# ed-fish/data-efficient-video-transformers

Measured on AMD Instinct MI355X. Metric: clips/sec fwd+bwd, B=8 T=32 3x224x224 bf16, higher is better.
Workload: dtype bf16; 1 GPU; ViViT metric shape (SURVEY 8 'M'; BASELINE configs[2]/[3] transformer): B=8/GPU, T=32, 3x224x224, patch 16, d=512, ...; global_batch=8, parallelism=dp1

## Files before the change

### data-efficient-video-transformers_amd/csrc/layernorm.hip

```cpp
#include "common.h"
#include "ln_reduce.h"

namespace {

constexpr int kLnBlock = 256;
constexpr int kLnBwdBlock = 256;
constexpr int kLnBwdMaxBlocks = 1024;

template <typename TX, typename TY, int VPL>
__global__ __launch_bounds__(kLnBlock) void ln_fwd_kernel(
    const TX* __restrict__ x, const float* __restrict__ gamma, const float* __restrict__ beta,
    TY* __restrict__ y, float* __restrict__ mean, float* __restrict__ rstd, int64_t rows, int64_t n1,
    int d, int64_t xs0, int64_t xs1, int64_t ys0, int64_t ys1, float eps) {
  const int lane = threadIdx.x & 63;
  const int64_t wave = (int64_t)blockIdx.x * (kLnBlock / 64) + (threadIdx.x >> 6);
  const int64_t nwaves = (int64_t)gridDim.x * (kLnBlock / 64);
  const float inv_d = 1.0f / (float)d;

  float g[VPL][8], b[VPL][8];
#pragma unroll
  for (int i = 0; i < VPL; ++i) {
    const int c = (lane + 64 * i) * 8;
    if (c < d) {
      load8<float>(gamma + c, g[i]);
      load8<float>(beta + c, b[i]);
    }
  }

  for (int64_t r = wave; r < rows; r += nwaves) {
    const int64_t i0 = r / n1, i1 = r - i0 * n1;
    const TX* xr = x + i0 * xs0 + i1 * xs1;
    TY* yr = y + i0 * ys0 + i1 * ys1;
    float v[VPL][8];
    float s = 0.f;
#pragma unroll
    for (int i = 0; i < VPL; ++i) {
      const int c = (lane + 64 * i) * 8;
      if (c < d) {
        load8<TX>(xr + c, v[i]);
#pragma unroll
        for (int k = 0; k < 8; ++k) s += v[i][k];
      }
    }
    const float mu = wave_sum_dpp(s) * inv_d;
    float q = 0.f;
#pragma unroll
    for (int i = 0; i < VPL; ++i) {
      const int c = (lane + 64 * i) * 8;
      if (c < d) {
#pragma unroll
        for (int k = 0; k < 8; ++k) {
          v[i][k] -= mu;
          q = fmaf(v[i][k], v[i][k], q);
        }
      }
    }
    const float rs = rsqrtf(wave_sum_dpp(q) * inv_d + eps);
#pragma unroll
    for (int i = 0; i < VPL; ++i) {
      const int c = (lane + 64 * i) * 8;
      if (c < d) {
        float o[8];
#pragma unroll
        for (int k = 0; k < 8; ++k) o[k] = fmaf(v[i][k] * rs, g[i][k], b[i][k]);
        store8<TY>(yr + c, o);
      }
    }
    if (lane == 0) {
      mean[r] = mu;
      rstd[r] = rs;
    }
  }
}

template <typename TDY, typename TX, typename TDX, typename TL, int VPL>
__global__ __launch_bounds__(kLnBwdBlock) void ln_bwd_kernel(
    const TDY* __restrict__ dy, const TX* __restrict__ x, const float* __restrict__ gamma,
    const float* __restrict__ mean, const float* __restrict__ rstd, const TDX* dx_add,
    TDX* dx, TL* __restrict__ dx_lp, float* __restrict__ partial , int64_t rows, int64_t n1, int d,
    int64_t xs0, int64_t xs1, int64_t ys0, int64_t ys1,
    const TDY* __restrict__ dy_first, int64_t dyf_s, const TDX* __restrict__ dx_first, int64_t dxf_s) {
  extern __shared__ __attribute__((aligned(16))) float lds[];
  const int lane = threadIdx.x & 63;
  const int wid = threadIdx.x >> 6;
  const int64_t wave = (int64_t)blockIdx.x * (kLnBwdBlock / 64) + wid;
  const int64_t nwaves = (int64_t)gridDim.x * (kLnBwdBlock / 64);
  const float inv_d = 1.0f / (float)d;

  float g[VPL][8], dg[VPL][8], db[VPL][8];
#pragma unroll
  for (int i = 0; i < VPL; ++i) {
    const int c = (lane + 64 * i) * 8;
    if (c < d) load8<float>(gamma + c, g[i]);
#pragma unroll
    for (int k = 0; k < 8; ++k) { dg[i][k] = 0.f; db[i][k] = 0.f; }
  }

  for (int64_t r = wave; r < rows; r += nwaves) {
    const int64_t i0 = r / n1, i1 = r - i0 * n1;
    const TX* xr = x + i0 * xs0 + i1 * xs1;
    const TDY* dyr = dy + i0 * ys0 + i1 * ys1;
    const int64_t xoff = i0 * xs0 + i1 * xs1;
    TDX* dxr = dx + xoff;
    const float mu = mean[r], rs = rstd[r];
    float xh[VPL][8], gg[VPL][8];
    float s1 = 0.f, s2 = 0.f;
#pragma unroll
    for (int i = 0; i < VPL; ++i) {
      const int c = (lane + 64 * i) * 8;
      if (c < d) {
        float xv[8], dv[8];
        load8<TX>(xr + c, xv);
        load8<TDY>(dyr + c, dv);
        if (dy_first && i1 == 0) {
          float fv[8];
          load8<TDY>(dy_first + i0 * dyf_s + c, fv);
#pragma unroll
          for (int k = 0; k < 8; ++k) dv[k] += fv[k];
        }
#pragma unroll
        for (int k = 0; k < 8; ++k) {
          xh[i][k] = (xv[k] - mu) * rs;
          gg[i][k] = dv[k] * g[i][k];
          s1 += gg[i][k];
          s2 = fmaf(gg[i][k], xh[i][k], s2);
          dg[i][k] = fmaf(dv[k], xh[i][k], dg[i][k]);
          db[i][k] += dv[k];
        }
      }
    }
    const float c1 = wave_sum_dpp(s1) * inv_d;
    const float c2 = wave_sum_dpp(s2) * inv_d;
#pragma unroll
    for (int i = 0; i < VPL; ++i) {
      const int c = (lane + 64 * i) * 8;
      if (c < d) {
        float o[8];
#pragma unroll
        for (int k = 0; k < 8; ++k) o[k] = rs * (gg[i][k] - c1 - xh[i][k] * c2);
        if (dx_add) {
          float a[8];
          load8<TDX>(dx_add + xoff + c, a);
#pragma unroll
          for (int k = 0; k < 8; ++k) o[k] += a[k];
        }
        if (dx_first && i1 == 0) {
          float a[8];
          load8<TDX>(dx_first + i0 * dxf_s + c, a);
#pragma unroll
          for (int k = 0; k < 8; ++k) o[k] += a[k];
        }
        store8<TDX>(dxr + c, o);
        if (dx_lp) store8<TL>(dx_lp + xoff + c, o);
      }
    }
  }

  for (int w = 0; w < kLnBwdBlock / 64; ++w) {
    if (wid == w) {
#pragma unroll
      for (int i = 0; i < VPL; ++i) {
        const int c = (lane + 64 * i) * 8;
        if (c < d) {
#pragma unroll
          for (int k = 0; k < 8; ++k) {
            if (w == 0) { lds[c + k] = dg[i][k]; lds[d + c + k] = db[i][k]; }
            else { lds[c + k] += dg[i][k]; lds[d + c + k] += db[i][k]; }
          }
        }
      }
    }
    __syncthreads();
  }
  float* out = partial + (int64_t)blockIdx.x * 2 * d;
  for (int c = threadIdx.x; c < 2 * d; c += kLnBwdBlock) out[c] = lds[c];
}

int ln_check(const char* name, const void* a, const void* b, int64_t n0, int64_t n1, int64_t d,
             int64_t xs0, int64_t xs1, int64_t ys0, int64_t ys1) {
  DVT_REQUIRE(a && b, "%s: null pointer", name);
  DVT_REQUIRE(n0 >= 0 && n1 >= 1 && d >= 8, "%s: bad sizes", name);
  DVT_REQUIRE(d % 8 == 0, "%s: d = %lld must be a multiple of 8", name, (long long)d);
  if (d > 8 * 64 * 8) DVT_UNSUPPORTED("%s: d = %lld > 4096 not supported", name, (long long)d);
  DVT_REQUIRE(xs0 % 8 == 0 && xs1 % 8 == 0 && ys0 % 8 == 0 && ys1 % 8 == 0,
              "%s: row strides must be multiples of 8 elements", name);
  DVT_REQUIRE(dvt_aligned16(a) && dvt_aligned16(b), "%s: buffers must be 16-byte aligned", name);
  return DVT_OK;
}

}

#define DVT_LN_VPL_SWITCH(vpl, ...)                    \
  switch (vpl) {                                       \
    case 1: { constexpr int VPL = 1; __VA_ARGS__; break; } \
    case 2: { constexpr int VPL = 2; __VA_ARGS__; break; } \
    case 3: { constexpr int VPL = 3; __VA_ARGS__; break; } \
    case 4: { constexpr int VPL = 4; __VA_ARGS__; break; } \
    default: { constexpr int VPL = 8; __VA_ARGS__; break; } \
  }

#define DVT_LN_FWD_LAUNCH(TX, TY)                                                                                          \
  DVT_LN_VPL_SWITCH(vpl, hipLaunchKernelGGL((ln_fwd_kernel<TX, TY, VPL>), dim3((unsigned)blocks), dim3(kLnBlock), 0, st,    \
                                            (const TX*)x, gamma, beta, (TY*)y, mean, rstd, rows, n1, (int)d, xs0, xs1, ys0, \
                                            ys1, eps))

#define DVT_LN_BWD_LAUNCH(TDY, TX, TDX, TL)                                                                                \
  DVT_LN_VPL_SWITCH(vpl, hipLaunchKernelGGL((ln_bwd_kernel<TDY, TX, TDX, TL, VPL>), dim3((unsigned)blocks),                 \
                                            dim3(kLnBwdBlock), lds, st, (const TDY*)q->dy, (const TX*)q->x, q->gamma,       \
                                            q->mean, q->rstd, (const TDX*)q->dx_add, (TDX*)q->dx, (TL*)q->dx_lp, partial,   \
                                            rows, q->n1, (int)q->d, q->xs0, q->xs1, q->ys0, q->ys1, (const TDY*)q->dy_first, \
                                            q->dy_first_stride, (const TDX*)q->dx_first, q->dx_first_stride))

namespace {

constexpr int kLnGroup = 32;
struct LnGroup { dvt_ln_pending e[kLnGroup]; };

__global__ __launch_bounds__(1024) void ln_bwd_reduce_group_kernel(const LnGroup grp) {
  const dvt_ln_pending& q = grp.e[blockIdx.y];
  constexpr int PL = 32;
  __shared__ float red[PL][33];
  const int cl = threadIdx.x & 31, pl = threadIdx.x >> 5;
  const int c = blockIdx.x * 32 + cl;
  const int d = q.d;
  if (blockIdx.x * 32 >= 2 * d) return;
  const int64_t ld = 2 * (int64_t)d;
  float a0 = 0.f, a1 = 0.f, a2 = 0.f, a3 = 0.f;
  if (c < 2 * d) {
    int p = pl;
    for (; p + 3 * PL < q.nparts; p += 4 * PL) {
      a0 += q.partial[(int64_t)p * ld + c];
      a1 += q.partial[(int64_t)(p + PL) * ld + c];
      a2 += q.partial[(int64_t)(p + 2 * PL) * ld + c];
      a3 += q.partial[(int64_t)(p + 3 * PL) * ld + c];
    }
    for (; p < q.nparts; p += PL) a0 += q.partial[(int64_t)p * ld + c];
  }
  red[pl][cl] = (a0 + a1) + (a2 + a3);
  __syncthreads();
  if (pl < 4) {
    float t = 0.f;
#pragma unroll
    for (int i = 0; i < PL / 4; ++i) t += red[pl * (PL / 4) + i][cl];
    red[pl * (PL / 4)][cl] = t;
  }
  __syncthreads();
  if (pl == 0 && c < 2 * d) {
    const float t = (red[0][cl] + red[PL / 4][cl]) + (red[2 * (PL / 4)][cl] + red[3 * (PL / 4)][cl]);
    float* o = c < d ? q.dgamma + c : q.dbeta + (c - d);
    const bool acc = c < d ? (q.accumulate & 1) : (q.accumulate & 2);
    *o = acc ? *o + t : t;
  }
}

}

extern "C" {

int dvt_layernorm_fwd_mixed(const void* x, int x_dtype, const float* gamma, const float* beta, void* y, int y_dtype, float* mean,
                            float* rstd, int64_t n0, int64_t n1, int64_t d, int64_t xs0, int64_t xs1,
                            int64_t ys0, int64_t ys1, float eps, dvt_stream_t stream) {
  int rc = ln_check("dvt_layernorm_fwd", x, y, n0, n1, d, xs0, xs1, ys0, ys1);
  if (rc) return rc;
  DVT_REQUIRE(gamma && beta && mean && rstd, "dvt_layernorm_fwd: null parameter/statistics pointer");
  DVT_REQUIRE(dvt_aligned16(gamma) && dvt_aligned16(beta), "dvt_layernorm_fwd: gamma/beta misaligned");
  const int64_t rows = n0 * n1;
  if (rows == 0) return DVT_OK;
  hipStream_t st = (hipStream_t)stream;
  int64_t blocks = dvt_cdiv(rows, kLnBlock / 64);
  const int64_t cap = (int64_t)dvt_num_cus() * 8;
  if (blocks > cap) blocks = cap;
  const int vpl = (int)dvt_cdiv(d, 8 * 64);
  if (x_dtype == y_dtype) {
    DVT_DISPATCH_DTYPE(x_dtype, T, DVT_LN_FWD_LAUNCH(T, T));
  } else if (x_dtype == DVT_F32 && dvt_is_16bit(y_dtype)) {
    DVT_DISPATCH_16BIT(y_dtype, E, DVT_LN_FWD_LAUNCH(float, E));
  } else if (y_dtype == DVT_F32 && dvt_is_16bit(x_dtype)) {
    DVT_DISPATCH_16BIT(x_dtype, E, DVT_LN_FWD_LAUNCH(E, float));
  } else {
    DVT_UNSUPPORTED("dvt_layernorm_fwd: x dtype %d -> y dtype %d (equal types, or fp32 on one side)", x_dtype, y_dtype);
  }
  DVT_LAUNCH_CHECK("dvt_layernorm_fwd");
  return DVT_OK;
}

int dvt_layernorm_fwd(const void* x, const float* gamma, const float* beta, void* y, float* mean,
                      float* rstd, int64_t n0, int64_t n1, int64_t d, int64_t xs0, int64_t xs1,
                      int64_t ys0, int64_t ys1, float eps, int dtype, dvt_stream_t stream) {
  return dvt_layernorm_fwd_mixed(x, dtype, gamma, beta, y, dtype, mean, rstd, n0, n1, d, xs0, xs1, ys0, ys1, eps, stream);
}

size_t dvt_layernorm_bwd_workspace_bytes(int64_t d) {
  return (size_t)kLnBwdMaxBlocks * 2 * (size_t)(d > 0 ? d : 0) * sizeof(float);
}

size_t dvt_layernorm_bwd_partial_bytes(int64_t rows, int64_t d) {
  int64_t blocks = dvt_cdiv(rows > 0 ? rows : 1, kLnBwdBlock / 64);
  if (blocks > kLnBwdMaxBlocks) blocks = kLnBwdMaxBlocks;
  return (size_t)blocks * 2 * (size_t)(d > 0 ? d : 0) * sizeof(float);
}

int dvt_layernorm_bwd_ex(const dvt_ln_bwd_desc* q, dvt_stream_t stream) {
  DVT_REQUIRE(q, "dvt_layernorm_bwd: null descriptor");
  int rc = ln_check("dvt_layernorm_bwd", q->x, q->dy, q->n0, q->n1, q->d, q->xs0, q->xs1, q->ys0, q->ys1);
  if (rc) return rc;
  DVT_REQUIRE(q->gamma && q->mean && q->rstd && q->dx && q->dgamma && q->dbeta && q->workspace, "dvt_layernorm_bwd: null pointer");
  DVT_REQUIRE(dvt_aligned16(q->dx) && dvt_aligned16(q->gamma) && dvt_aligned16(q->workspace) && dvt_aligned16(q->dx_add) &&
                  dvt_aligned16(q->dy_first) && dvt_aligned16(q->dx_first) && dvt_aligned16(q->dx_lp),
              "dvt_layernorm_bwd: buffers must be 16-byte aligned");
  DVT_REQUIRE(q->dy_first_stride % 8 == 0 && q->dx_first_stride % 8 == 0,
              "dvt_layernorm_bwd: first-row strides must be multiples of 8 elements");
  DVT_REQUIRE(!q->defer_reduce || q->pending, "dvt_layernorm_bwd: defer_reduce needs a pending descriptor to fill");
  const int64_t rows = q->n0 * q->n1;
  DVT_REQUIRE(rows > 0, "dvt_layernorm_bwd: no rows");
  hipStream_t st = (hipStream_t)stream;
  int64_t blocks = dvt_cdiv(rows, kLnBwdBlock / 64);
  if (blocks > kLnBwdMaxBlocks) blocks = kLnBwdMaxBlocks;
  const int64_t d = q->d;
  const int vpl = (int)dvt_cdiv(d, 8 * 64);
  const size_t lds = 2 * (size_t)d * sizeof(float);
  float* partial = (float*)q->workspace;
  const int dyt = q->dy_dtype, xt = q->x_dtype, dxt = q->dx_dtype;
  if (dyt == xt && xt == dxt && !q->dx_lp) {
    DVT_DISPATCH_DTYPE(xt, T, DVT_LN_BWD_LAUNCH(T, T, T, T));
  } else if (dvt_is_16bit(dyt) && xt == DVT_F32 && dxt == DVT_F32 && (!q->dx_lp || q->dx_lp_dtype == dyt)) {
    DVT_DISPATCH_16BIT(dyt, E, DVT_LN_BWD_LAUNCH(E, float, float, E));
  } else if (dyt == DVT_F32 && dvt_is_16bit(xt) && dxt == xt && !q->dx_lp) {
    DVT_DISPATCH_16BIT(xt, E, DVT_LN_BWD_LAUNCH(float, E, E, E));
  } else {
    DVT_UNSUPPORTED("dvt_layernorm_bwd: dtype combination (dy %d, x %d, dx %d, dx_lp %d) not instantiated", dyt, xt, dxt,
                    q->dx_lp ? q->dx_lp_dtype : -1);
  }
  DVT_LAUNCH_CHECK("dvt_layernorm_bwd");
  if (q->defer_reduce) {
    dvt_ln_pending* pn = q->pending;
    pn->partial = partial; pn->nparts = (int)blocks; pn->d = (int)d; pn->dgamma = q->dgamma; pn->dbeta = q->dbeta;
    pn->accumulate = (q->accumulate_gamma ? 1 : 0) | (q->accumulate_beta ? 2 : 0); pn->valid = 1;
    return DVT_OK;
  }
  dvt_ln_partials_reduce(partial, (int)blocks, (int)d, q->dgamma, q->dbeta, q->accumulate_gamma, q->accumulate_beta, st);
  DVT_LAUNCH_CHECK("dvt_layernorm_bwd(reduce)");
  return DVT_OK;
}

int dvt_layernorm_reduce_group(const dvt_ln_pending* list, int count, dvt_stream_t stream) {
  DVT_REQUIRE(count >= 0 && (count == 0 || list), "dvt_layernorm_reduce_group: bad arguments");
  hipStream_t st = (hipStream_t)stream;
  for (int i = 0; i < count;) {
    LnGroup grp{};
    int n = 0, dmax = 0;
    for (; i < count && n < kLnGroup; ++i) {
      if (!list[i].valid) continue;
      DVT_REQUIRE(list[i].partial && list[i].dgamma && list[i].dbeta && list[i].nparts > 0 && list[i].d > 0,
                  "dvt_layernorm_reduce_group: bad entry");
      grp.e[n++] = list[i];
      if (list[i].d > dmax) dmax = list[i].d;
    }
    if (n == 0) continue;
    hipLaunchKernelGGL(ln_bwd_reduce_group_kernel, dim3((unsigned)dvt_cdiv(2 * dmax, 32), (unsigned)n), dim3(1024), 0, st, grp);
    DVT_LAUNCH_CHECK("dvt_layernorm_reduce_group");
  }
  return DVT_OK;
}

int dvt_layernorm_bwd_first(const void* dy, const void* x, const float* gamma, const float* mean,
                            const float* rstd, const void* dx_add, void* dx, float* dgamma, float* dbeta,
                            void* workspace,
                            int64_t n0, int64_t n1, int64_t d, int64_t xs0, int64_t xs1, int64_t ys0,
                            int64_t ys1, const void* dy_first, int64_t dy_first_stride,
                            const void* dx_first, int64_t dx_first_stride, int dtype,
                            int accumulate_gamma, int accumulate_beta, dvt_stream_t stream) {
  dvt_ln_bwd_desc q{};
  q.dy = dy; q.dy_dtype = dtype; q.x = x; q.x_dtype = dtype; q.gamma = gamma; q.mean = mean; q.rstd = rstd;
  q.dx_add = dx_add; q.dx = dx; q.dx_dtype = dtype; q.dgamma = dgamma; q.dbeta = dbeta; q.workspace = workspace;
  q.n0 = n0; q.n1 = n1; q.d = d; q.xs0 = xs0; q.xs1 = xs1; q.ys0 = ys0; q.ys1 = ys1;
  q.dy_first = dy_first; q.dy_first_stride = dy_first_stride; q.dx_first = dx_first; q.dx_first_stride = dx_first_stride;
  q.accumulate_gamma = accumulate_gamma; q.accumulate_beta = accumulate_beta;
  return dvt_layernorm_bwd_ex(&q, stream);
}

int dvt_layernorm_bwd(const void* dy, const void* x, const float* gamma, const float* mean,
                      const float* rstd, const void* dx_add, void* dx, float* dgamma, float* dbeta,
                      void* workspace,
                      int64_t n0, int64_t n1, int64_t d, int64_t xs0, int64_t xs1, int64_t ys0,
                      int64_t ys1, int dtype, int accumulate, dvt_stream_t stream) {
  return dvt_layernorm_bwd_first(dy, x, gamma, mean, rstd, dx_add, dx, dgamma, dbeta, workspace, n0, n1, d, xs0,
                                 xs1, ys0, ys1, nullptr, 0, nullptr, 0, dtype, accumulate, accumulate, stream);
}

}
```

### data-efficient-video-transformers_amd/functional.py

```python
from __future__ import annotations

import contextlib
from collections import namedtuple
from typing import Optional

import torch

from . import _lib as L
from . import ops

Tensor = torch.Tensor


def _wc(w: Optional[Tensor], dtype: torch.dtype) -> Optional[Tensor]:
    if w is None:
        return None
    c = getattr(w, "_dvt_compute", None)
    if c is not None and c.dtype == dtype and w._dvt_sink.owner.compute_valid:
        return c
    w = w.detach()
    if w.dtype == dtype:
        return w.contiguous()
    return ops.cast(w, dtype)


def _sink(p):
    return None if p is None else getattr(p, "_dvt_sink", None)


def _emit_wgrad(sink, dy2: Tensor, x2: Tensor):
    if sink is None:
        return ops.linear_wgrad(dy2, x2)
    ops.linear_wgrad(dy2, x2, out=sink.buf.view(dy2.shape[1], x2.shape[1]), accumulate=not sink.fresh)
    sink.mark_written()
    return None


def _emit_wgrad_bias(sink_w, sink_b, dy2: Tensor, x2: Tensor, has_bias: bool, defer: bool = False):
    N, K = dy2.shape[1], x2.shape[1]
    w_out = sink_w.buf.view(N, K) if sink_w is not None else None
    b_out, b_acc = None, False
    if has_bias:
        if sink_b is not None:
            b_out, b_acc = sink_b.buf.view(-1), not sink_b.fresh
        else:
            b_out = torch.empty((N,), dtype=torch.float32, device=dy2.device)
    r = ops.linear_wgrad(dy2, x2, out=w_out, accumulate=(not sink_w.fresh) if sink_w is not None else False,
                         bias_out=b_out, bias_accumulate=b_acc, defer_reduce=defer)
    dw, pending = r if defer else (r, None)

    def finish():
        if sink_w is not None:
            sink_w.mark_written()
        if has_bias and sink_b is not None:
            sink_b.mark_written()

    dw_ret = None if sink_w is not None else dw
    db_ret = None if (not has_bias or sink_b is not None) else b_out
    if defer:
        return dw_ret, db_ret, pending, finish
    finish()
    return dw_ret, db_ret


def _linear_bwd(sink_w, sink_b, dy2: Tensor, x2: Tensor, w: Tensor, has_bias: bool, *, epilogue: int = L.EPI_NONE,
                aux: Optional[Tensor] = None):
    N, K = dy2.shape[1], x2.shape[1]
    w_out = sink_w.buf.view(N, K) if sink_w is not None else None
    b_out, b_acc = None, False
    if has_bias:
        if sink_b is not None:
            b_out, b_acc = sink_b.buf.view(-1), not sink_b.fresh
        else:
            b_out = torch.empty((N,), dtype=torch.float32, device=dy2.device)
    dw, dx = ops.linear_backward(dy2, x2, w, out=w_out, accumulate=(not sink_w.fresh) if sink_w is not None else False,
                                 bias_out=b_out, bias_accumulate=b_acc, epilogue=epilogue, aux=aux)
    if sink_w is not None:
        sink_w.mark_written()
    if has_bias and sink_b is not None:
        sink_b.mark_written()
    return (None if sink_w is not None else dw), (None if (not has_bias or sink_b is not None) else b_out), dx


def _emit_colsum(sink, dy2: Tensor):
    if sink is None:
        return ops.colsum(dy2)
    ops.colsum(dy2, out=sink.buf.view(-1), accumulate=not sink.fresh)
    sink.mark_written()
    return None


LN_DEFER = True
_ln_pending_sinks = set()


def ln_flush(end_of_step: bool = False):
    ops.layernorm_flush()
    _ln_pending_sinks.clear()
    if end_of_step:
        _lp_hand.clear()


def _ln_bwd(dy, x, g, mean, rstd, sg, sb, **kw):
    if sg is None or sb is None:
        return ops.layernorm_bwd(dy, x, g, mean, rstd, **kw)
    defer = None
    if LN_DEFER:
        if id(sg) in _ln_pending_sinks or id(sb) in _ln_pending_sinks:
            ln_flush()
        if sg.fresh and sb.fresh:
            _ln_pending_sinks.update((id(sg), id(sb)))

            def defer():
                sg.mark_written()
                sb.mark_written()
    r = ops.layernorm_bwd(dy, x, g, mean, rstd, dg=sg.buf.view(-1), db=sb.buf.view(-1),
                          accumulate=not sg.fresh, accumulate_beta=not sb.fresh, defer=defer, **kw)
    if defer is None:
        sg.mark_written()
        sb.mark_written()
    return (r[0], None, None) + tuple(r[3:])


def _emit_into(sink, t: Tensor):
    ops.axpby_f32_(sink.buf.view(-1), t.reshape(-1).contiguous(), 1.0, 0.0 if sink.fresh else 1.0)
    sink.mark_written()


_lp_hand = {}


def lp_clear() -> None:
    _lp_hand.clear()


def _lp_put(t32: Tensor, lp: Tensor) -> None:
    _lp_hand[t32.data_ptr()] = (t32, t32._version, lp)


def _lp_take(t32: Tensor, T: torch.dtype) -> Tensor:
    e = _lp_hand.pop(t32.data_ptr(), None)
    if (e is not None and e[0].shape == t32.shape and e[0].stride() == t32.stride() and e[0].dtype == t32.dtype
            and t32._version == e[1] and e[2].dtype == T):
        return e[2]
    return ops.cast(t32, T)


def _f32(t: Optional[Tensor]) -> Optional[Tensor]:
    if t is None:
        return None
    t = t.detach()
    return t.contiguous() if t.dtype == torch.float32 else ops.cast(t, torch.float32)


def _same_layout(a: Tensor, b: Tensor) -> bool:
    return a.shape == b.shape and all(sa == sb for sa, sb, n in zip(a.stride(), b.stride(), a.shape) if n > 1)


def _as(t: Tensor, dtype: torch.dtype) -> Tensor:
    return t if t.dtype == dtype else ops.cast(t, dtype)


class _Linear(torch.autograd.Function):
    @staticmethod
    def forward(ctx, x, w, b, out_f32):
        shp = x.shape
        x2 = x.reshape(-1, shp[-1])
        if not x2.is_contiguous():
            x2 = x2.contiguous()
        wc = _wc(w, x.dtype)
        M, K = x2.shape
        N = wc.shape[0]
        out_dtype = torch.float32 if out_f32 else x.dtype
        y = ops.gemm(x2, wc, M, N, K, a_kmajor=True, b_kmajor=True, lda=x2.stride(0), ldb=K,
                     out_dtype=out_dtype, bias=_f32(b))
        ctx.save_for_backward(x2, wc)
        ctx.has_bias = b is not None
        ctx.xshape = shp
        ctx.sinks = (_sink(w), _sink(b))
        return y.view(*shp[:-1], N)

    @staticmethod
    def backward(ctx, dy):
        x2, wc = ctx.saved_tensors
        dy2 = _as(dy.reshape(-1, dy.shape[-1]).contiguous(), x2.dtype)
        dx = dw = db = None
        if ctx.needs_input_grad[0]:
            dx = ops.linear_dgrad(dy2, wc).view(ctx.xshape)
        if ctx.needs_input_grad[1]:
            dw, db = _emit_wgrad_bias(ctx.sinks[0], ctx.sinks[1], dy2, x2, ctx.has_bias and ctx.needs_input_grad[2])
        elif ctx.has_bias and ctx.needs_input_grad[2]:
            db = _emit_colsum(ctx.sinks[1], dy2)
        return dx, dw, db, None


def linear(x: Tensor, w: Tensor, b: Optional[Tensor] = None, out_f32: bool = False) -> Tensor:
    return _Linear.apply(x, w, b, out_f32)


class _Act(torch.autograd.Function):
    @staticmethod
    def forward(ctx, x, act):
        ctx.save_for_backward(x)
        ctx.act = act
        return ops.act_fwd(x, act)

    @staticmethod
    def backward(ctx, dy):
        (x,) = ctx.saved_tensors
        return ops.act_bwd(_as(dy, x.dtype), x, ctx.act), None


def gelu(x: Tensor) -> Tensor:
    return _Act.apply(x, ops.ACT_GELU)


def relu(x: Tensor) -> Tensor:
    return _Act.apply(x, ops.ACT_RELU)


class _Add(torch.autograd.Function):
    @staticmethod
    def forward(ctx, a, b):
        return ops.add(a, b)

    @staticmethod
    def backward(ctx, dy):
        return dy, dy


def add(a: Tensor, b: Tensor) -> Tensor:
    return _Add.apply(a, b)


class _Fork(torch.autograd.Function):

    @staticmethod
    def forward(ctx, x):
        return x.view(x.shape), x.view(x.shape)

    @staticmethod
    def backward(ctx, da, db):
        if da is None or db is None:
            return da if db is None else db
        if da.dtype != db.dtype:
            db = _as(db.contiguous(), da.dtype)
        return ops.add(da.contiguous(), db.contiguous())


def fork(x: Tensor):
    if not (torch.is_grad_enabled() and x.requires_grad):
        return x, x
    return _Fork.apply(x)


class _Cast(torch.autograd.Function):

    @staticmethod
    def forward(ctx, x, dtype):
        ctx.src = x.dtype
        return _as(x, dtype)

    @staticmethod
    def backward(ctx, dy):
        return _as(dy.contiguous(), ctx.src), None


def cast(x: Tensor, dtype: torch.dtype) -> Tensor:
    return x if x.dtype == dtype else _Cast.apply(x, dtype)


class _LayerNorm(torch.autograd.Function):
    @staticmethod
    def forward(ctx, x, w, b, eps):
        xc = x.contiguous()
        g, bb = _f32(w), _f32(b)
        y, mean, rstd = ops.layernorm_fwd(xc, g, bb, eps)
        ctx.save_for_backward(xc, g, mean, rstd)
        ctx.sinks = (_sink(w), _sink(b))
        return y

    @staticmethod
    def backward(ctx, dy):
        xc, g, mean, rstd = ctx.saved_tensors
        dx, dg, db = _ln_bwd(_as(dy.contiguous(), xc.dtype), xc, g, mean, rstd, *ctx.sinks)
        return dx, dg, db, None


def layernorm(x: Tensor, w: Tensor, b: Tensor, eps: float = 1e-5) -> Tensor:
    return _LayerNorm.apply(x, w, b, eps)


class _PatchEmbed(torch.autograd.Function):

    @staticmethod
    def forward(ctx, clip, w, b, patch, dtype, tubelet):
        if tubelet == 1:
            patches = ops.patchify(clip, patch, dtype)
        else:
            patches = ops.tubelet_patchify(clip, patch, tubelet, dtype)
        wc = _wc(w, dtype)
        emb = ops.linear_fwd(patches, wc, _f32(b))
        ctx.save_for_backward(patches, wc)
        ctx.clip_shape, ctx.clip_dtype, ctx.patch, ctx.tubelet = tuple(clip.shape), clip.dtype, patch, tubelet
        ctx.sinks = (_sink(w), _sink(b))
        return emb

    @staticmethod
    def backward(ctx, demb):
        patches, wc = ctx.saved_tensors
        demb = demb.contiguous()
        dclip = None
        if ctx.needs_input_grad[0]:
            dpatch = ops.linear_dgrad(demb, wc)
            if ctx.tubelet == 1:
                dclip = ops.patchify_bwd(dpatch, ctx.clip_shape, ctx.patch, ctx.clip_dtype)
            else:
                dclip = ops.tubelet_patchify_bwd(dpatch, ctx.clip_shape, ctx.patch, ctx.tubelet, ctx.clip_dtype)
        dw, db = _emit_wgrad_bias(ctx.sinks[0], ctx.sinks[1], demb, patches, True)
        return dclip, dw, db, None, None, None


def patch_embed(clip: Tensor, w: Tensor, b: Tensor, patch: int, dtype: torch.dtype, tubelet: int = 1) -> Tensor:
    return _PatchEmbed.apply(clip, w, b, patch, dtype, tubelet)


class _Tokens(torch.autograd.Function):
    @staticmethod
    def forward(ctx, emb, cls, pos, S, T, n):
        cls32 = _f32(cls).reshape(-1)
        pos32 = _f32(pos)
        pos32 = pos32.reshape(T, pos32.shape[-2], pos32.shape[-1])
        ctx.T, ctx.pos_rows = T, pos32.shape[1]
        ctx.cls_shape, ctx.pos_shape = tuple(cls.shape), tuple(pos.shape)
        ctx.sinks = (_sink(cls), _sink(pos))
        return ops.tokens_assemble_fwd(emb.contiguous(), cls32, pos32, S, T, n)

    @staticmethod
    def backward(ctx, dout):
        sc, sp = ctx.sinks
        if sc is not None and sp is not None and sc.fresh != sp.fresh:
            demb, dcls, dpos = ops.tokens_assemble_bwd(dout, ctx.T, ctx.pos_rows)
            _emit_into(sc, dcls)
            _emit_into(sp, dpos)
            return demb, None, None, None, None, None
        if sc is not None and sp is not None:
            demb, _, _ = ops.tokens_assemble_bwd(dout, ctx.T, ctx.pos_rows, dcls=sc.buf.view(-1),
                                                 dpos=sp.buf.view(ctx.T, ctx.pos_rows, -1),
                                                 accumulate=not sc.fresh)
            sc.mark_written()
            sp.mark_written()
            return demb, None, None, None, None, None
        demb, dcls, dpos = ops.tokens_assemble_bwd(dout, ctx.T, ctx.pos_rows)
        return demb, dcls.view(ctx.cls_shape), dpos.view(ctx.pos_shape), None, None, None


def tokens_assemble(emb: Tensor, cls: Tensor, pos: Tensor, S: int, T: int, n: int) -> Tensor:
    return _Tokens.apply(emb, cls, pos, S, T, n)


class _ClsNormConcat(torch.autograd.Function):

    @staticmethod
    def forward(ctx, x, w, b, tok, B, T, eps, out_dtype=None):
        S, N, d = x.shape
        xc = x.contiguous()
        g, bb = _f32(w), _f32(b)
        rows = (S, 1, N * d, 0)
        cls_rows, mean, rstd = ops.layernorm_fwd(xc, g, bb, eps, rows=rows, out_dtype=out_dtype)
        tok32 = _f32(tok).reshape(-1) if tok is not None else None
        seq = ops.rows_gather_fwd(cls_rows, d, tok32, B, T, d)
        ctx.save_for_backward(xc, g, mean, rstd)
        ctx.dims = (B, T, S, N, d)
        ctx.seq_dtype = seq.dtype
        ctx.tok_shape = tuple(tok.shape) if tok is not None else None
        ctx.sinks = (_sink(w), _sink(b), _sink(tok))
        return seq

    @staticmethod
    def backward(ctx, dseq):
        xc, g, mean, rstd = ctx.saved_tensors
        B, T, S, N, d = ctx.dims
        gdt = ctx.seq_dtype
        dseq = _as(dseq.contiguous(), gdt)
        drows = torch.empty((S, d), dtype=gdt, device=xc.device)
        sg, sb, st = ctx.sinks
        if st is not None:
            ops.rows_gather_bwd(dseq, drows, d, True, B, T, d, dtok=st.buf.view(-1), accumulate=not st.fresh)
            st.mark_written()
            dtok = None
        else:
            dtok = ops.rows_gather_bwd(dseq, drows, d, ctx.tok_shape is not None, B, T, d)
        dx = ops.zeros(xc.shape, xc.dtype, xc.device) if N > 1 else torch.empty_like(xc)
        _, dg, db = _ln_bwd(drows, xc, g, mean, rstd, sg, sb, rows=(S, 1, N * d, 0), dy_rows=(d, 0), dx=dx)
        if dtok is not None:
            dtok = dtok.view(ctx.tok_shape)
        return dx, dg, db, dtok, None, None, None, None


def cls_norm_concat(x: Tensor, w: Tensor, b: Tensor, tok: Optional[Tensor], B: int, T: int,
                    eps: float = 1e-5, out_dtype: Optional[torch.dtype] = None) -> Tensor:
    return _ClsNormConcat.apply(x, w, b, tok, B, T, eps, out_dtype)


class _RowsSelect(torch.autograd.Function):

    @staticmethod
    def forward(ctx, x):
        B, Ln, d = x.shape
        xc = x.contiguous()
        ctx.shape = (B, Ln, d)
        return ops.rows_gather_fwd(xc, Ln * d, None, B, 1, d).view(B, d)

    @staticmethod
    def backward(ctx, dy):
        B, Ln, d = ctx.shape
        dx = ops.zeros((B, Ln, d), dy.dtype, dy.device)
        ops.rows_gather_bwd(dy.contiguous().view(B, 1, d), dx, Ln * d, False, B, 1, d)
        return dx


def select_first_row(x: Tensor) -> Tensor:
    return _RowsSelect.apply(x)


class _AttentionCore(torch.autograd.Function):

    @staticmethod
    def forward(ctx, q, k, v, scale):
        B, H, Lq, dh = q.shape
        o_mem = torch.empty((B, Lq, H, dh), dtype=q.dtype, device=q.device)
        o = o_mem.permute(0, 2, 1, 3)
        lse = ops.attention_fwd(q, k, v, o, scale)
        ctx.save_for_backward(q, k, v, o, lse)
        ctx.scale = scale
        return o

    @staticmethod
    def backward(ctx, do):
        q, k, v, o, lse = ctx.saved_tensors
        B, H, Lq, dh = q.shape
        Lk = k.shape[2]
        if _same_layout(do, o) and do.dtype == q.dtype:
            do_v = do.as_strided(o.shape, o.stride())
        else:
            do_c = _as(do.permute(0, 2, 1, 3).contiguous(), q.dtype)
            do_v = do_c.permute(0, 2, 1, 3).as_strided(o.shape, o.stride())
        dq = torch.empty_strided(q.shape, q.stride(), dtype=q.dtype, device=q.device)
        dk = torch.empty_strided(k.shape, k.stride(), dtype=k.dtype, device=k.device)
        dv = torch.empty_strided(v.shape, v.stride(), dtype=v.dtype, device=v.device)
        ops.attention_bwd(q, k, v, o, lse, do_v, dq, dk, dv, ctx.scale)
        return dq, dk, dv, None


def attention_core(q: Tensor, k: Tensor, v: Tensor, scale: float) -> Tensor:
    return _AttentionCore.apply(q, k, v, scale)


AttnTap = namedtuple("AttnTap", "kind q k lse heads dh seq_first packed P")
_attn_tap = None


@contextlib.contextmanager
def attention_tap():
    global _attn_tap
    outer, layers = _attn_tap, []
    _attn_tap = layers
    try:
        yield layers
    finally:
        _attn_tap = outer


def _split_qkv(qkv: Tensor, S: int, N: int, heads: int, dh: int, seq_first: bool):
    if seq_first:
        q5 = qkv.view(N, S, 3, heads, dh)
        return tuple(q5[:, :, i].permute(1, 2, 0, 3) for i in range(3))
    q5 = qkv.view(S, N, 3, heads, dh)
    return tuple(q5[:, :, i].permute(0, 2, 1, 3) for i in range(3))


def _heads_view(o_mem: Tensor, seq_first: bool) -> Tensor:
    return o_mem.permute(1, 2, 0, 3) if seq_first else o_mem.permute(0, 2, 1, 3)


class _AttnBlock(torch.autograd.Function):

    @staticmethod
    def forward(ctx, x, ln_w, ln_b, w_qkv, w_out, b_out, heads, prenorm, residual, eps, b_qkv=None,
                seq_first=False, attn_dropout=0.0, cdt=None):
        shp = x.shape
        d = shp[-1]
        if seq_first:
            N, S = shp[0], shp[1]
        else:
            S, N = (shp[0], shp[1]) if x.dim() == 3 else (1, shp[0])
        x2 = x.reshape(-1, d)
        if not x2.is_contiguous():
            x2 = x2.contiguous()
        M = x2.shape[0]
        T = x.dtype if cdt is None else cdt
        ctx.mixed = mixed = T != x.dtype
        if mixed and not (x.dtype == torch.float32 and prenorm and residual and w_out is not None and attn_dropout == 0.0):
            raise ValueError("the fp32 stream form is the pre-norm residual block with an output projection")
        if prenorm:
            g, bb = _f32(ln_w), _f32(ln_b)
            xn, mean, rstd = ops.layernorm_fwd(x2, g, bb, eps, out_dtype=T)
        else:
            g = mean = rstd = None
            xn = x2
        wq = _wc(w_qkv, T)
        inner = wq.shape[0] // 3
        dh = inner // heads
        qkv = ops.linear_fwd(xn, wq, _f32(b_qkv))
        q, k, v = _split_qkv(qkv, S, N, heads, dh, seq_first)
        o_mem = torch.empty((N, S, heads, dh) if seq_first else (S, N, heads, dh), dtype=T, device=x.device)
        drop = None
        if attn_dropout > 0.0:
            drop = (attn_dropout, _rng.tensor(x.device), _rng.take(S * heads * N * N))
        lse = ops.attention_fwd(q, k, v, _heads_view(o_mem, seq_first), dh ** -0.5, drop)
        if _attn_tap is not None:
            _attn_tap.append(AttnTap("dense", q, k, lse, heads, dh, seq_first, qkv, None))
        ctx.drop = drop
        o2 = o_mem.view(M, inner)
        if w_out is not None:
            wo = _wc(w_out, T)
            if residual:
                y = ops.linear_fwd(o2, wo, _f32(b_out), epilogue=L.EPI_RESIDUAL, residual=x2,
                                   out_dtype=torch.float32 if mixed else None)
            else:
                y = ops.linear_fwd(o2, wo, _f32(b_out))
        else:
            wo = None
            y = ops.add(o2, x2) if residual else o2
        ctx.save_for_backward(x2, g, mean, rstd, xn if prenorm else None, wq, wo, qkv, o_mem, lse)
        ctx.cfg = (S, N, heads, dh, inner, prenorm, residual, w_out is not None, b_out is not None,
                   b_qkv is not None, seq_first)
        ctx.xshape = shp
        ctx.sinks = tuple(_sink(t) for t in (ln_w, ln_b, w_qkv, w_out, b_out, b_qkv))
        return y.view(*shp[:-1], y.shape[-1])

    @staticmethod
    def backward(ctx, dy):
        x2, g, mean, rstd, xn, wq, wo, qkv, o_mem, lse = ctx.saved_tensors
        S, N, heads, dh, inner, prenorm, residual, has_out, has_bias, has_qkv_bias, seq_first = ctx.cfg
        M = x2.shape[0]
        T = qkv.dtype
        if xn is None:
            xn = x2
        if ctx.mixed:
            dy32 = dy.reshape(M, -1).contiguous()
            dy2 = _lp_take(dy32, T)
        else:
            dy2 = _as(dy.reshape(M, -1).contiguous(), T)
        dwo = dbo = None
        if has_out:
            dwo, dbo, do2 = _linear_bwd(ctx.sinks[3], ctx.sinks[4], dy2, o_mem.view(M, inner), wo, has_bias)
        else:
            do2 = dy2
        q, k, v = _split_qkv(qkv, S, N, heads, dh, seq_first)
        dqkv = torch.empty_like(qkv)
        dq, dk, dv = _split_qkv(dqkv, S, N, heads, dh, seq_first)
        ops.attention_bwd(q, k, v, _heads_view(o_mem, seq_first), lse,
                          _heads_view(do2.view(o_mem.shape), seq_first), dq, dk, dv, dh ** -0.5, ctx.drop)
        dwq, dbq, dxn = _linear_bwd(ctx.sinks[2], ctx.sinks[5], dqkv, xn, wq, has_qkv_bias)
        dg = db = None
        if ctx.mixed:
            dx, dg, db, dx_lp = _ln_bwd(dxn, x2, g, mean, rstd, ctx.sinks[0], ctx.sinks[1], dx_add=dy32,
                                        dx_dtype=torch.float32, dx_lp=T)
            _lp_put(dx, dx_lp)
        elif prenorm:
            dx, dg, db = _ln_bwd(dxn, x2, g, mean, rstd, ctx.sinks[0], ctx.sinks[1],
                                 dx_add=dy2 if residual else None)
        else:
            dx = ops.add(dxn, dy2) if residual else dxn
        if M >= 4096:
            ln_flush()
        return dx.view(ctx.xshape), dg, db, dwq, dwo, dbo, None, None, None, None, dbq, None, None, None


def attn_block(x, ln_w, ln_b, w_qkv, w_out, b_out, heads, *, prenorm=True, residual=True, eps=1e-5,
               b_qkv=None, seq_first=False, attn_dropout=0.0, cdt=None):
    return _AttnBlock.apply(x, ln_w, ln_b, w_qkv, w_out, b_out, heads, prenorm, residual, eps, b_qkv, seq_first,
                            float(attn_dropout), cdt)


class _AttnBlockCls(torch.autograd.Function):

    @staticmethod
    def forward(ctx, x, ln_w, ln_b, w_qkv, w_out, b_out, heads, eps, cdt=None):
        S, N, d = x.shape
        T = x.dtype if cdt is None else cdt
        ctx.mixed = mixed = T != x.dtype
        x2 = x.reshape(S * N, d)
        if not x2.is_contiguous():
            x2 = x2.contiguous()
        g, bb = _f32(ln_w), _f32(ln_b)
        wqkv = _wc(w_qkv, T)
        inner = wqkv.shape[0] // 3
        dh = inner // heads
        wo = _wc(w_out, T)
        ctx.cfg = (S, N, d, heads, dh, inner, b_out is not None, eps)
        ctx.sinks = tuple(_sink(t) for t in (ln_w, ln_b, w_qkv, w_out, b_out))
        x3 = x2.view(S, N, d)
        ctx.folded = (not mixed) and cls_fold_taken(x3, heads, dh)
        if ctx.folded:
            xn0, mean0, rstd0 = ops.layernorm_fwd(x2, g, bb, eps, rows=(S, 1, N * d, 0))
            q = ops.linear_fwd(xn0, wqkv[:inner])
            R = ops.heads_expand(q, wqkv[inner:2 * inner], heads, dh ** -0.5)
            A, lse, P, mean, rstd = ops.attn_cls_fwd(x3, g, bb, eps, R)
            if _attn_tap is not None:
                _attn_tap.append(AttnTap("folded", None, None, None, heads, dh, False, None, P))
            o = ops.heads_contract(A, wqkv[2 * inner:], 1.0, g, bb)
            y = ops.linear_fwd(o, wo, _f32(b_out), epilogue=L.EPI_RESIDUAL, residual=x3[:, 0])
            ctx.save_for_backward(x2, g, bb, mean0, rstd0, xn0, wqkv, wo, q, o, R, A, lse, P, mean, rstd)
            return y
        xn, mean, rstd = ops.layernorm_fwd(x2, g, bb, eps, out_dtype=T)
        w_q, w_kv = wqkv[:inner], wqkv[inner:]
        kv = ops.linear_fwd(xn, w_kv)
        xn0 = xn.view(S, N, d)[:, 0]
        q = ops.linear_fwd(xn0, w_q)
        kv5 = kv.view(S, N, 2, heads, dh)
        k4, v4 = kv5[:, :, 0].permute(0, 2, 1, 3), kv5[:, :, 1].permute(0, 2, 1, 3)
        o = torch.empty((S, inner), dtype=T, device=x.device)
        lse = ops.attention_fwd(q.view(S, 1, heads, dh).permute(0, 2, 1, 3), k4, v4,
                                o.view(S, 1, heads, dh).permute(0, 2, 1, 3), dh ** -0.5)
        if _attn_tap is not None:
            _attn_tap.append(AttnTap("cls", q.view(S, 1, heads, dh).permute(0, 2, 1, 3), k4, lse, heads, dh, False, kv, None))
        y = ops.linear_fwd(o, wo, _f32(b_out), epilogue=L.EPI_RESIDUAL, residual=x3[:, 0],
                           out_dtype=torch.float32 if mixed else None)
        ctx.save_for_backward(x2, g, mean, rstd, xn, wqkv, wo, q, kv, o, lse)
        return y

    @staticmethod
    def _backward_folded(ctx, dy):
        x2, g, bb, mean0, rstd0, xn0, wqkv, wo, q, o, R, A, lse, P, mean, rstd = ctx.saved_tensors
        S, N, d, heads, dh, inner, has_bias, eps = ctx.cfg
        T = x2.dtype
        s_g, s_b, s_qkv, s_o, s_bo = ctx.sinks
        scale = dh ** -0.5
        dy2 = _as(dy.reshape(S, d).contiguous(), T)
        dwo, dbo, do = _linear_bwd(s_o, s_bo, dy2, o, wo, has_bias)
        if s_qkv is not None:
            buf, acc = s_qkv.buf.view(3 * inner, d), not s_qkv.fresh
            dwqkv = None
        else:
            buf, acc = torch.empty((3 * inner, d), dtype=torch.float32, device=x2.device), False
            dwqkv = buf
        w_q, w_k, w_v = wqkv[:inner], wqkv[inner:2 * inner], wqkv[2 * inner:]
        dM = ops.heads_expand_outer(do, w_v, heads, A, buf[2 * inner:], gamma=g, beta=bb, accumulate=acc)
        if s_g is not None and s_b is not None:
            dx2, G, _, _ = ops.attn_cls_bwd(x2.view(S, N, d), g, bb, eps, R, A, lse, P, mean, rstd, dM, dg=s_g.buf.view(-1),
                                            db=s_b.buf.view(-1), accumulate=not s_g.fresh, accumulate_beta=not s_b.fresh)
            dg, db = s_g.buf.view(-1), s_b.buf.view(-1)
        else:
            dx2, G, dg, db = ops.attn_cls_bwd(x2.view(S, N, d), g, bb, eps, R, A, lse, P, mean, rstd, dM)
        dq = ops.heads_contract_outer(G, g, w_k, q, buf[inner:2 * inner], alpha_out=scale, alpha_dw=scale, accumulate=acc)
        _, dxn0 = ops.linear_backward(dq, xn0, w_q, out=buf[:inner], accumulate=acc)
        if s_qkv is not None:
            s_qkv.mark_written()
        dxf = dx2.view(S * N, d)
        ops.layernorm_bwd(dxn0, x2, g, mean0, rstd0, rows=(S, 1, N * d, 0), dx=dxf, dx_add=dxf, dx_first=dy2,
                          dg=dg, db=db, accumulate=True)
        if s_g is not None and s_b is not None:
            s_g.mark_written()
            s_b.mark_written()
            dg = db = None
        return dx2.view(S, N, d), dg, db, dwqkv, dwo, dbo, None, None, None

    @staticmethod
    def backward(ctx, dy):
        if ctx.folded:
            return _AttnBlockCls._backward_folded(ctx, dy)
        x2, g, mean, rstd, xn, wqkv, wo, q, kv, o, lse = ctx.saved_tensors
        S, N, d, heads, dh, inner, has_bias, _ = ctx.cfg
        T = kv.dtype
        s_g, s_b, s_qkv, s_o, s_bo = ctx.sinks
        dy_s = dy.reshape(S, d).contiguous()
        dy2 = _lp_take(dy_s, T) if ctx.mixed else _as(dy_s, T)
        dwo, dbo, do = _linear_bwd(s_o, s_bo, dy2, o, wo, has_bias)
        kv5 = kv.view(S, N, 2, heads, dh)
        k4, v4 = kv5[:, :, 0].permute(0, 2, 1, 3), kv5[:, :, 1].permute(0, 2, 1, 3)
        dq = torch.empty_like(q)
        dkv = torch.empty_like(kv)
        dkv5 = dkv.view(S, N, 2, heads, dh)
        one = lambda t: t.view(S, 1, heads, dh).permute(0, 2, 1, 3)
        ops.attention_bwd(one(q), k4, v4, one(o), lse, one(do), one(dq),
                          dkv5[:, :, 0].permute(0, 2, 1, 3), dkv5[:, :, 1].permute(0, 2, 1, 3), dh ** -0.5)
        xn0 = xn.view(S, N, d)[:, 0]
        w_q, w_kv = wqkv[:inner], wqkv[inner:]
        if s_qkv is not None:
            buf, acc = s_qkv.buf.view(3 * inner, d), not s_qkv.fresh
            dwqkv = None
        else:
            buf, acc = torch.empty((3 * inner, d), dtype=torch.float32, device=x2.device), False
            dwqkv = buf
        ops.linear_wgrad(dq, xn0, out=buf[:inner], accumulate=acc)
        _, pend = ops.linear_wgrad(dkv, xn, out=buf[inner:], accumulate=acc, defer_reduce=True)
        dxn = ops.linear_dgrad(dkv, w_kv, carry=pend)
        if s_qkv is not None:
            s_qkv.mark_written()
        dxn0 = ops.linear_dgrad(dq, w_q)
        if ctx.mixed:
            dx, dg, db, dx_lp = _ln_bwd(dxn, x2, g, mean, rstd, s_g, s_b, rows=(S, N, N * d, d), dy_first=dxn0,
                                        dx_first=dy_s, dx_dtype=torch.float32, dx_lp=T)
            _lp_put(dx.view(S * N, d), dx_lp.view(S * N, d))
        else:
            dx, dg, db = _ln_bwd(dxn, x2, g, mean, rstd, s_g, s_b, rows=(S, N, N * d, d),
                                 dy_first=dxn0, dx_first=dy2)
        return dx.view(S, N, d), dg, db, dwqkv, dwo, dbo, None, None, None


CLS_FOLD_MIN_ROWS = 4096


def cls_fold_taken(x3: Tensor, heads: int, dh: int) -> bool:
    S, N, _ = x3.shape
    return S * N >= CLS_FOLD_MIN_ROWS and ops.attn_cls_supported(x3, heads, dh)


def attn_block_cls(x, ln_w, ln_b, w_qkv, w_out, b_out, heads, *, eps=1e-5, cdt=None):
    return _AttnBlockCls.apply(x, ln_w, ln_b, w_qkv, w_out, b_out, heads, eps, cdt)


class _CrossAttnBlock(torch.autograd.Function):

    @staticmethod
    def forward(ctx, x, c, lnq_w, lnq_b, lnk_w, lnk_b, w_q, w_kv, w_out, b_out, heads, eps):
        B, Lq, d = x.shape
        Lk = c.shape[1]
        T = x.dtype
        x2 = x.reshape(B * Lq, d).contiguous()
        c2 = _as(c.reshape(B * Lk, c.shape[-1]).contiguous(), T)
        gq, bq, gk, bk = _f32(lnq_w), _f32(lnq_b), _f32(lnk_w), _f32(lnk_b)
        xn, mq, rq = ops.layernorm_fwd(x2, gq, bq, eps)
        cn, mk, rk = ops.layernorm_fwd(c2, gk, bk, eps)
        wq, wkv, wo = _wc(w_q, T), _wc(w_kv, T), _wc(w_out, T)
        inner = wq.shape[0]
        dh = inner // heads
        q = ops.linear_fwd(xn, wq)
        kv = ops.linear_fwd(cn, wkv)
        q4 = q.view(B, Lq, heads, dh).permute(0, 2, 1, 3)
        kv5 = kv.view(B, Lk, 2, heads, dh)
        k4, v4 = kv5[:, :, 0].permute(0, 2, 1, 3), kv5[:, :, 1].permute(0, 2, 1, 3)
        o_mem = torch.empty((B, Lq, heads, dh), dtype=T, device=x.device)
        lse = ops.attention_fwd(q4, k4, v4, o_mem.permute(0, 2, 1, 3), dh ** -0.5)
        y = ops.linear_fwd(o_mem.view(B * Lq, inner), wo, _f32(b_out), epilogue=L.EPI_RESIDUAL, residual=x2)
        ctx.save_for_backward(x2, c2, gq, gk, mq, rq, mk, rk, xn, cn, wq, wkv, wo, q, kv, o_mem, lse)
        ctx.cfg = (B, Lq, Lk, heads, dh, inner, tuple(x.shape), tuple(c.shape), c.dtype)
        ctx.sinks = tuple(_sink(t) for t in (lnq_w, lnq_b, lnk_w, lnk_b, w_q, w_kv, w_out, b_out))
        return y.view(B, Lq, d)

    @staticmethod
    def backward(ctx, dy):
        x2, c2, gq, gk, mq, rq, mk, rk, xn, cn, wq, wkv, wo, q, kv, o_mem, lse = ctx.saved_tensors
        B, Lq, Lk, heads, dh, inner, xshape, cshape, cdt = ctx.cfg
        s = ctx.sinks
        T = x2.dtype
        dy2 = _as(dy.reshape(B * Lq, -1).contiguous(), T)
        do2 = ops.linear_dgrad(dy2, wo)
        dwo, dbo = _emit_wgrad_bias(s[6], s[7], dy2, o_mem.view(B * Lq, inner), True)
        q4 = q.view(B, Lq, heads, dh).permute(0, 2, 1, 3)
        kv5 = kv.view(B, Lk, 2, heads, dh)
        k4, v4 = kv5[:, :, 0].permute(0, 2, 1, 3), kv5[:, :, 1].permute(0, 2, 1, 3)
        dq = torch.empty_like(q)
        dkv = torch.empty_like(kv)
        dkv5 = dkv.view(B, Lk, 2, heads, dh)
        ops.attention_bwd(q4, k4, v4, o_mem.permute(0, 2, 1, 3), lse, do2.view(o_mem.shape).permute(0, 2, 1, 3),
                          dq.view(B, Lq, heads, dh).permute(0, 2, 1, 3), dkv5[:, :, 0].permute(0, 2, 1, 3),
                          dkv5[:, :, 1].permute(0, 2, 1, 3), dh ** -0.5)
        dwq = _emit_wgrad(s[4], dq, xn)
        dwkv = _emit_wgrad(s[5], dkv, cn)
        dx, dgq, dbq = _ln_bwd(ops.linear_dgrad(dq, wq), x2, gq, mq, rq, s[0], s[1], dx_add=dy2)
        dc = dgk = dbk = None
        if ctx.needs_input_grad[1] or ctx.needs_input_grad[4]:
            dc, dgk, dbk = _ln_bwd(ops.linear_dgrad(dkv, wkv), c2, gk, mk, rk, s[2], s[3])
            dc = _as(dc, cdt).view(cshape)
        return dx.view(xshape), dc, dgq, dbq, dgk, dbk, dwq, dwkv, dwo, dbo, None, None


def cross_attn_block(x, c, lnq_w, lnq_b, lnk_w, lnk_b, w_q, w_kv, w_out, b_out, heads, eps=1e-5):
    return _CrossAttnBlock.apply(x, c, lnq_w, lnq_b, lnk_w, lnk_b, w_q, w_kv, w_out, b_out, heads, eps)


class _MlpBlock(torch.autograd.Function):

    @staticmethod
    def forward(ctx, x, ln_w, ln_b, w1, b1, w2, b2, act, prenorm, residual, eps, cdt=None):
        shp = x.shape
        d = shp[-1]
        x2 = x.reshape(-1, d)
        if not x2.is_contiguous():
            x2 = x2.contiguous()
        T = x.dtype if cdt is None else cdt
        ctx.mixed = mixed = T != x.dtype
        if mixed and not (x.dtype == torch.float32 and prenorm and residual):
            raise ValueError("the fp32 stream form is the pre-norm residual block")
        if prenorm:
            g, bb = _f32(ln_w), _f32(ln_b)
            xn, mean, rstd = ops.layernorm_fwd(x2, g, bb, eps, out_dtype=T)
        else:
            g = mean = rstd = None
            xn = x2
        w1c, w2c = _wc(w1, T), _wc(w2, T)
        M = x2.shape[0]
        if act == "gelu":
            u = torch.empty((M, w1c.shape[0]), dtype=T, device=x.device)
            h = ops.linear_fwd(xn, w1c, _f32(b1), epilogue=L.EPI_GELU, aux=u)
        else:
            u = None
            h = ops.linear_fwd(xn, w1c, _f32(b1), epilogue=L.EPI_RELU)
        if residual:
            y = ops.linear_fwd(h, w2c, _f32(b2), epilogue=L.EPI_RESIDUAL, residual=x2,
                               out_dtype=torch.float32 if mixed else None)
        else:
            y = ops.linear_fwd(h, w2c, _f32(b2))
        ctx.save_for_backward(x2, g, mean, rstd, xn if prenorm else None, w1c, w2c, u, h)
        ctx.cfg = (act, prenorm, residual, b1 is not None, b2 is not None)
        ctx.xshape = shp
        ctx.sinks = tuple(_sink(t) for t in (ln_w, ln_b, w1, b1, w2, b2))
        return y.view(shp)

    @staticmethod
    def backward(ctx, dy):
        x2, g, mean, rstd, xn, w1c, w2c, u, h = ctx.saved_tensors
        act, prenorm, residual, has_b1, has_b2 = ctx.cfg
        T = h.dtype
        if xn is None:
            xn = x2
        if ctx.mixed:
            dy32 = dy.reshape(x2.shape).contiguous()
            dy2 = _lp_take(dy32, T)
        else:
            dy2 = _as(dy.reshape(x2.shape).contiguous(), T)
        sk = ctx.sinks
        if act == "gelu":
            dw2, db2, du = _linear_bwd(sk[4], sk[5], dy2, h, w2c, has_b2, epilogue=L.EPI_DGELU, aux=u)
        else:
            dw2, db2, du = _linear_bwd(sk[4], sk[5], dy2, h, w2c, has_b2, epilogue=L.EPI_DRELU, aux=h)
        dw1, db1, dxn = _linear_bwd(sk[2], sk[3], du, xn, w1c, has_b1)
        dg = db = None
        if ctx.mixed:
            dx, dg, db, dx_lp = _ln_bwd(dxn, x2, g, mean, rstd, sk[0], sk[1], dx_add=dy32, dx_dtype=torch.float32, dx_lp=T)
            _lp_put(dx, dx_lp)
        elif prenorm:
            dx, dg, db = _ln_bwd(dxn, x2, g, mean, rstd, sk[0], sk[1], dx_add=dy2 if residual else None)
        else:
            dx = ops.add(dxn, dy2) if residual else dxn
        return dx.view(ctx.xshape), dg, db, dw1, db1, dw2, db2, None, None, None, None, None


def mlp_block(x, ln_w, ln_b, w1, b1, w2, b2, *, act="gelu", prenorm=True, residual=True, eps=1e-5, cdt=None):
    return _MlpBlock.apply(x, ln_w, ln_b, w1, b1, w2, b2, act, prenorm, residual, eps, cdt)


class _BceLogits(torch.autograd.Function):
    @staticmethod
    def forward(ctx, z, target):
        zc = z.contiguous()
        t32 = _f32(target)
        ctx.save_for_backward(zc, t32)
        return ops.bce_logits_fwd(zc, t32).view(())

    @staticmethod
    def backward(ctx, gloss):
        zc, t32 = ctx.saved_tensors
        g = _f32(gloss).reshape(1)
        return ops.bce_logits_bwd(zc, t32, g), None


def bce_with_logits(z: Tensor, target: Tensor) -> Tensor:
    return _BceLogits.apply(z, target)


class _HeadBce(torch.autograd.Function):

    @staticmethod
    def forward(ctx, x, g1, b1, g2, b2, w, c, target, eps1, eps2, lp_dtype):
        x2 = x.contiguous()
        loss, logits, grads = ops.head_bce_fwd(x2, _f32(g1), _f32(b1), eps1, _f32(g2), _f32(b2), eps2, _f32(w), _f32(c),
                                               _f32(target))
        ctx.grads = grads
        ctx.sinks = tuple(_sink(p) for p in (g1, b1, g2, b2, w, c))
        ctx.shapes = tuple(None if p is None else tuple(p.shape) for p in (g1, b1, g2, b2, w, c))
        ctx.x_dtype, ctx.lp_dtype = x.dtype, lp_dtype
        ctx.mark_non_differentiable(logits)
        ctx.set_materialize_grads(False)
# ... 523 lines not shown
        if fork == "alias":
            return (y, x.view(x.shape)) + tail
        return (y, ops.im2col(xc, False, N, Cin, H, W, 1, int(fork), 0, Cin, xc.dtype)) + tail

    @staticmethod
    def backward(ctx, dy, *more):
        if _ln_pending_sinks:
            ln_flush()
        dshort = more[0] if (ctx.fork is not None and more) else None
        if dy is None or (ctx.fork is not None and dshort is None):
            raise RuntimeError("_ConvBnAct.backward: an output of a deferred-BatchNorm layer received no gradient")
        xc, wp, z, y, mean, invstd, g32, col, b32, pidx, rmask = ctx.saved_tensors
        geom, Cout, ld, direct, relu, training, has_res, wshape, dtype = ctx.cfg
        N, Cin, H, W, k, stride, pad, nchw = geom
        Cout_l, Cin_l, padded = ctx.logical
        sw, sg, sb = ctx.sinks
        dy = _as(dy.contiguous(), z.dtype)
        Ho, Wo = ops.conv_out_hw(H, W, k, stride, pad)

        cval = Cout_l if Cout != Cout_l else 0

        def bn_backward(**kw):
            if pidx is not None:
                dz_, dg_, db_ = ops.bn_bwd_pooled(dy, pidx, z, mean, invstd, g32, b32, N, Ho, Wo - ctx.trim, relu, training, **kw)
                return dz_, None, dg_, db_
            return ops.bn_bwd(dy, z, y, mean, invstd, g32, relu, training, has_res, beta=b32, mask=rmask, c_valid=cval, **kw)

        if ctx.link is not None and ctx.link.get("done"):
            dz, dres = dy, None
            dgam, dbet = ctx.link["grads"]
            ctx.link["done"] = False
        elif sg is not None and sb is not None and sg.fresh != sb.fresh:
            dz, dres, dgam, dbet = bn_backward()
            _emit_into(sg, dgam); _emit_into(sb, dbet)
            dgam = dbet = None
        elif sg is not None and sb is not None:
            dz, dres, _, _ = bn_backward(dgamma=sg.buf.view(-1), dbeta=sb.buf.view(-1), accumulate=not sg.fresh)
            sg.mark_written(); sb.mark_written()
            dgam = dbet = None
        else:
            dz, dres, dgam, dbet = bn_backward()
        (kh, kw) = ops._pair(k)
        w4 = (Cout, Cin, kh, kw)
        wg = _wgrad_route(ctx, xc, dz, geom, Cout)
        direct_dw = wg in ("halo", "window", "implicit_bn", "implicit")
        if direct_dw:
            dw_master = sw.buf.view(wshape) if sw is not None else torch.empty(wshape, dtype=torch.float32, device=dz.device)
            acc_w = (not sw.fresh) if sw is not None else False
            if wg == "halo":
                pend = ops.conv3x3_c64_wgrad(xc, dz, N, H, W, dw_master, accumulate=acc_w, defer_reduce=True, Cout=Cout)
            elif wg == "window":
                pend = ops.conv3x1_wgrad(xc, dz, N, H, W, dw_master, accumulate=acc_w, defer_reduce=True, affine=ctx.in_affine)
            else:
                xw = xc
                if wg == "implicit_bn":
                    am, ai, ag, ab, acv, arelu = ctx.in_affine[:6]
                    xw = ops.bn_apply_fwd(xc.contiguous(), am, ai, ag, ab, None, bool(arelu), c_valid=int(acv))
                _, pend = ops.conv2d_implicit_wgrad(xw, dz, N, Cin, H, W, Cout, k, stride, pad, ctx.trim, defer_reduce=True,
                                                    master=dw_master, accumulate=acc_w, logical=(Cout_l, Cin_l))
        elif wg == "implicit_packed":
            dwt, pend = ops.conv2d_implicit_wgrad(xc, dz, N, Cin, H, W, Cout, k, stride, pad, ctx.trim,
                                                  defer_reduce=True)
            unpack, dwp = ops.conv_weight_unpack_grad_t, dwt
        else:
            if col is None:
                col = xc if direct else ops.im2col(xc, nchw, N, Cin, H, W, k, stride, pad, ld, dtype)
            dwp, pend = ops.linear_wgrad(dz, col, defer_reduce=True)
            unpack = ops.conv_weight_unpack_grad
        dx = None
        (sh_, sw_), (ph_, pw_) = ops._pair(stride), ops._pair(pad)
        joined = [dshort is None or not ctx.x_needs]
        if dshort is not None:
            dshort = _as(dshort.contiguous(), dz.dtype)

        def join_alias():
            if joined[0] or ctx.fork != "alias":
                return None
            joined[0] = True
            return dshort.view(N * H * W, Cin)
        wd = None
        pd = (kh - 1 - ph_, kw - 1 - pw_)
        if ctx.x_needs and ctx.implicit and ctx.geom0 is None and sh_ == 1 and sw_ == 1 and min(pd) >= 0:
            if ctx.w_ref is not None:
                wd = _packed_weight(ctx.w_ref, 1, Cout_l, Cin_l, kh, kw, Cout, Cin, 0, dtype)
            else:
                wd = ops.conv_weight_pack_dgrad(ctx.w4, dtype)
        dg, classes = _dgrad_route(ctx, dz, wd, geom, Cout, pd, not joined[0] and ctx.fork == "alias")
        if dg == "halo":
            dx = ops.conv3x3_c64(dz, wd, N, Ho, Wo, residual=join_alias())
        elif dg == "stream":
            dx = ops.conv3x3_stream(dz, wd, N, Ho, Wo, Cout, Cin, residual=join_alias())
        elif dg == "stream3x1_bn":
            lk = ctx.in_affine[6]
            sgm, sbm = lk["sinks"]
            if sgm is not None and sbm is not None and sgm.fresh == sbm.fresh:
                dx, _, _ = ops.conv3x1_stream_bn_bwd(dz, wd, xc, ctx.in_affine[:6], N, Ho, Wo, lk["training"],
                                                     dgamma=sgm.buf.view(-1), dbeta=sbm.buf.view(-1), accumulate=not sgm.fresh)
                sgm.mark_written(); sbm.mark_written()
                lk["grads"] = (None, None)
            else:
                dx, dgm, dbm = ops.conv3x1_stream_bn_bwd(dz, wd, xc, ctx.in_affine[:6], N, Ho, Wo, lk["training"])
                if sgm is not None and sbm is not None:
                    _emit_into(sgm, dgm); _emit_into(sbm, dbm)
                    dgm = dbm = None
                lk["grads"] = (dgm, dbm)
            lk["done"] = True
        elif dg == "stream3x1":
            dx = ops.conv3x1_stream(dz, wd, N, Ho, Wo, Cout, Cin)
        elif dg == "window":
            dx = ops.conv3x1_fwd(dz, wd, N, Ho, Wo)
        elif dg == "implicit":
            dx = ops.conv2d_implicit(dz, wd, N, Cout, Ho, Wo, Cin, k, 1, pd, carry=pend,
                                     residual=join_alias())
        elif dg == "strided":
            full = compact = None
            if not joined[0]:
                if ctx.fork == "alias":
                    full = dshort.view(N * H * W, Cin)
                elif (int(ctx.fork), int(ctx.fork)) == (sh_, sw_):
                    compact = dshort.view(-1, Cin)
                joined[0] = full is not None or compact is not None
            dx = torch.empty((N * H * W, Cin), dtype=dz.dtype, device=dz.device)
            order = sorted(classes, key=lambda c: c[2][0] * c[2][1])
            for i, (a, b, nt, pq, (rh, rw), hq) in enumerate(order):
                wc = _packed_class_weight(ctx.w_ref, Cout_l, Cin_l, kh, kw, Cout, Cin, (sh_, sw_, rh, rw), dtype)
                res, rc = (full, False) if full is not None else ((compact, True) if (compact is not None and a == 0 and b == 0)
                                                                  else (None, False))
                ops.conv2d_implicit(dz, wc, N, Cout, Ho, Wo, Cin, nt, 1, pq, out=dx, out_hw=hq,
                                    out_rows=ops.strided_class_rows(N, H, W, sh_, sw_, a, b, dz.device), residual=res,
                                    residual_compact=rc, carry=pend if i == len(order) - 1 else None)
        elif dg == "frames":
            if ctx.geom0 is not None:
                N0, C0, H0, W0, k0, s0, p0 = ctx.geom0
                (kh0, kw0) = ops._pair(k0)
                wq = _packed_weight(ctx.w_stem, 0, Cout_l, Cin_l, kh0, kw0, Cout, C0, _kpad(kh0 * kw0 * C0, dtype), dtype)
            else:
                (N0, C0, H0, W0, k0, s0, p0), wq = (N, Cin, H, W, k, stride, pad), wp
            Ho0, Wo0 = ops.conv_out_hw(H0, W0, k0, s0, p0)
            dx = ops.zeros(ctx.x_shape, ctx.x_dtype, dz.device).view(N0, C0, H0, W0)
            hw = Ho0 * Wo0
            for f0, cnt in ctx.dx_frames:
                dcol = ops.linear_dgrad(dz[f0 * hw:(f0 + cnt) * hw], wq)
                ops.copy_(dx[f0:f0 + cnt], ops.col2im_nchw(dcol, cnt, C0, H0, W0, k0, s0, p0, ctx.x_dtype))
            dx = dx.view(ctx.x_shape)
        elif dg == "gemm":
            dcol = ops.linear_dgrad(dz, wp, carry=pend)
            if direct:
                dx = dcol
            elif nchw:
                dx = ops.col2im_nchw(dcol, N, Cin, H, W, k, stride, pad, ctx.x_dtype).view(ctx.x_shape)
            elif not joined[0] and Cin % 8 == 0 and ld % 8 == 0:
                joined[0] = True
                if ctx.fork == "alias":
                    dx = ops.col2im(dcol, N, Cin, H, W, k, stride, pad, add=dshort.view(N * H * W, Cin))
                else:
                    dx = ops.col2im(dcol, N, Cin, H, W, k, stride, pad, add=dshort, add_stride=int(ctx.fork))
            else:
                dx = ops.col2im(dcol, N, Cin, H, W, k, stride, pad)
        if not joined[0]:
            dfull = dshort.view(dx.shape) if ctx.fork == "alias" else ops.col2im(dshort, N, Cin, H, W, 1, int(ctx.fork), 0)
            dx = ops.add(dx.contiguous(), dfull.view(dx.shape))
        ops.splitk_reduce_pending(pend)
        into = dict(out=sw.buf, accumulate=not sw.fresh) if sw is not None else {}
        if direct_dw:
            dw = dw_master
        elif ctx.pair is not None:
            kh_o, kw_o, pw_o, kwp = ctx.pair
            dw_pairs = unpack(dwp, w4)
            if sw is not None and Cout == Cout_l:
                dw = ops.conv_weight_pairs_bwd(dw_pairs, Cout, Cin_l, kh_o, kw_o, pw_o, kwp, **into)
            else:
                dwo = ops.conv_weight_pairs_bwd(dw_pairs, Cout, Cin_l, kh_o, kw_o, pw_o, kwp)
                dw = ops.unpad3_f32(dwo, Cout_l, Cin_l, kh_o * kw_o, Cin_l, **into)
        elif padded:
            dw = ops.unpad3_f32(unpack(dwp, w4), Cout_l, Cin_l, kh * kw, Cin, **into)
        else:
            dw = unpack(dwp, w4, **into)
        if sw is not None:
            sw.mark_written()
        dw = None if sw is not None else dw.view(wshape)
        return dx, dw, dgam, dbet, dres, None, None, None, None, None, None, None, None, None, None, None, None, None, None, None


def conv_bn_act(x, conv: torch.nn.Conv2d, bn: torch.nn.BatchNorm2d, geom, *, relu: bool, residual=None,
                dtype=torch.bfloat16, pool: bool = False, fork=None, stride=None):
    N, Cin, H, W, nchw = geom
    assert conv.bias is None and conv.groups == 1
    return conv_bn_act_raw(x, conv.weight, bn, geom, tuple(conv.kernel_size), tuple(conv.stride) if stride is None else stride,
                           tuple(conv.padding), relu=relu, residual=residual, dtype=dtype, pool=pool, fork=fork)


def conv_bn_act_raw(x, weight, bn, geom, k, stride, pad, *, relu: bool, residual=None, dtype=torch.bfloat16,
                    cpad: int = 0, dx_frames=None, pool: bool = False, fork=None, in_affine=None, defer_apply: bool = False):
    N, Cin, H, W, nchw = geom
    training = bn.training or bn.running_mean is None
    momentum = 0.1 if bn.momentum is None else bn.momentum
    joins = fork is not None and torch.is_grad_enabled() and x.requires_grad
    link = {} if defer_apply else None
    outs = _ConvBnAct.apply(x, weight, bn.weight, bn.bias, residual, bn.running_mean, bn.running_var,
                            (N, Cin, H, W, k, stride, pad, nchw), relu, training, momentum, bn.eps, dtype, cpad, dx_frames, pool,
                            fork if joins else None, in_affine, bool(defer_apply), link)
    if defer_apply:
        (mean, invstd), cout_l = outs[-2:], weight.shape[0]
        affine = (mean, invstd, _f32(bn.weight), _f32(bn.bias), cout_l if outs[0].shape[1] != cout_l else 0, relu, link)
    y = outs[0] if (joins or defer_apply) else outs
    if fork is not None:
        y = (y, outs[1] if joins else (x if fork == "alias" else subsample_nhwc(x, N, Cin, H, W, int(fork))))
    return (y, affine) if defer_apply else y

class _Subsample(torch.autograd.Function):

    @staticmethod
    def forward(ctx, x, geom):
        N, Cc, H, W, stride = geom
        ctx.geom = geom
        return ops.im2col(x.contiguous(), False, N, Cc, H, W, 1, stride, 0, Cc, x.dtype)

    @staticmethod
    def backward(ctx, dy):
        N, Cc, H, W, stride = ctx.geom
        return ops.col2im(dy.contiguous(), N, Cc, H, W, 1, stride, 0), None


def subsample_nhwc(x, N, Cc, H, W, stride):
    return _Subsample.apply(x, (N, Cc, H, W, stride))


class _Im2Col(torch.autograd.Function):

    @staticmethod
    def forward(ctx, x, geom):
        N, Cc, H, W, k, stride, pad = geom
        ctx.geom = geom
        (kh, kw) = ops._pair(k)
        return ops.im2col(x.contiguous(), False, N, Cc, H, W, k, stride, pad, kh * kw * Cc, x.dtype)

    @staticmethod
    def backward(ctx, dy):
        N, Cc, H, W, k, stride, pad = ctx.geom
        return ops.col2im(dy.contiguous(), N, Cc, H, W, k, stride, pad), None


def im2col_nhwc(x, N, Cc, H, W, k, stride, pad):
    return _Im2Col.apply(x, (N, Cc, H, W, k, stride, pad))


class _Col2Im(torch.autograd.Function):

    @staticmethod
    def forward(ctx, col, geom):
        N, Cc, H, W, k, stride, pad = geom
        ctx.geom = geom
        return ops.col2im(col.contiguous(), N, Cc, H, W, k, stride, pad)

    @staticmethod
    def backward(ctx, dy):
        N, Cc, H, W, k, stride, pad = ctx.geom
        (kh, kw) = ops._pair(k)
        return ops.im2col(dy.contiguous(), False, N, Cc, H, W, k, stride, pad, kh * kw * Cc, dy.dtype), None


def col2im_nhwc(col, N, Cc, H, W, k, stride, pad):
    return _Col2Im.apply(col, (N, Cc, H, W, k, stride, pad))


class _MaxPool(torch.autograd.Function):
    @staticmethod
    def forward(ctx, x, geom):
        N, Cc, H, W, k, stride, pad = geom
        y, idx = ops.maxpool_fwd(x.contiguous(), N, Cc, H, W, k, stride, pad)
        ctx.save_for_backward(idx)
        ctx.geom = geom
        return y

    @staticmethod
    def backward(ctx, dy):
        (idx,) = ctx.saved_tensors
        N, Cc, H, W, k, stride, pad = ctx.geom
        return ops.maxpool_bwd(dy.contiguous(), idx, N, Cc, H, W, k, stride, pad), None


def maxpool_nhwc(x, N, Cc, H, W, k, stride, pad):
    return _MaxPool.apply(x, (N, Cc, H, W, k, stride, pad))


class _Transpose12(torch.autograd.Function):

    @staticmethod
    def forward(ctx, x):
        return ops.transpose_last2(x)

    @staticmethod
    def backward(ctx, dy):
        return ops.transpose_last2(dy)


def transpose_last2(x):
    return _Transpose12.apply(x)


class _Checkpoint(torch.autograd.Function):

    @staticmethod
    def forward(ctx, fn, x, *params):
        ctx.fn = fn
        ctx.save_for_backward(x)
        ctx.site = _rng.site
        with torch.no_grad():
            return fn(x)

    @staticmethod
    def backward(ctx, dy):
        (x,) = ctx.saved_tensors
        xin = x.detach().requires_grad_(True)
        site_now, _rng.site = _rng.site, ctx.site
        with torch.enable_grad():
            y = ctx.fn(xin)
        _rng.site = site_now
        torch.autograd.backward(y, dy)
        return (None, xin.grad) + (None,) * (len(ctx.needs_input_grad) - 2)


def checkpoint(fn, x: Tensor, params=()) -> Tensor:
    if not torch.is_grad_enabled():
        return fn(x)
    return _Checkpoint.apply(fn, x, *params)


class _L2Normalize(torch.autograd.Function):
    @staticmethod
    def forward(ctx, x, eps):
        y, inv = ops.l2norm_rows_fwd(x.reshape(-1, x.shape[-1]), eps)
        ctx.save_for_backward(y, inv)
        ctx.eps, ctx.shape = eps, tuple(x.shape)
        return y.view(x.shape)

    @staticmethod
    def backward(ctx, dy):
        y, inv = ctx.saved_tensors
        return ops.l2norm_rows_bwd(_as(dy.reshape(y.shape), y.dtype), y, inv, ctx.eps).view(ctx.shape), None


def l2_normalize(x: Tensor, eps: float = 1e-12) -> Tensor:
    return _L2Normalize.apply(x, eps)


class _Gate(torch.autograd.Function):
    @staticmethod
    def forward(ctx, a, b):
        a, b = a.contiguous(), b.contiguous()
        ctx.save_for_backward(a, b)
        return ops.gate_fwd(a, b)

    @staticmethod
    def backward(ctx, dy):
        a, b = ctx.saved_tensors
        return ops.gate_bwd(_as(dy, a.dtype), a, b)


def gate(a: Tensor, b: Tensor) -> Tensor:
    return _Gate.apply(a, b)


class _Contrastive(torch.autograd.Function):

    @staticmethod
    def forward(ctx, reps, temperature):
        r32 = _as(reps.contiguous(), torch.float32)
        zn, inv = ops.l2norm_rows_fwd(r32, 1e-8)
        M, D = zn.shape
        sim = ops.gemm(zn, zn, M, M, D, a_kmajor=True, b_kmajor=True, lda=D, ldb=D, out_dtype=torch.float32)
        loss, lse = ops.contrastive_fwd(sim, temperature)
        ctx.save_for_backward(zn, inv, sim, lse)
        ctx.t, ctx.dtype = temperature, reps.dtype
        return loss

    @staticmethod
    def backward(ctx, gloss):
        zn, inv, sim, lse = ctx.saved_tensors
        M, D = zn.shape
        g = _as(gloss.contiguous().reshape(1), torch.float32)
        dsim = ops.contrastive_bwd(sim, lse, ctx.t, g)
        dzn = ops.gemm(dsim, zn, M, D, M, a_kmajor=True, b_kmajor=False, lda=M, ldb=D, out_dtype=torch.float32)
        ops.gemm(dsim, zn, M, D, M, a_kmajor=False, b_kmajor=False, lda=M, ldb=D, out=dzn, out_dtype=torch.float32,
                 accumulate=True)
        return _as(ops.l2norm_rows_bwd(dzn, zn, inv, 1e-8), ctx.dtype), None


def contrastive_loss(z_i: Tensor, z_j: Tensor, temperature: float) -> Tensor:
    return _Contrastive.apply(concat_rows(z_i, z_j), temperature)


class DropoutRng:

    def __init__(self):
        self.state = None
        self.site = 0
        self.seed = 1130

    def tensor(self, device) -> Tensor:
        if self.state is None or self.state.device != device:
            self.state = torch.tensor([self.seed, 0], dtype=torch.int64, device=device)
        return self.state

    def take(self, n: int) -> int:
        off = self.site
        self.site += (n + 3) // 4
        return off


_rng = DropoutRng()


def manual_seed(seed: int) -> None:
    _rng.seed, _rng.state, _rng.site = int(seed), None, 0


def next_step() -> None:
    if _rng.state is not None and _rng.site:
        ops.rng_advance_(_rng.state, _rng.site)
    _rng.site = 0


class _Dropout(torch.autograd.Function):
    @staticmethod
    def forward(ctx, x, p):
        st = _rng.tensor(x.device)
        ctx.p, ctx.off, ctx.state = p, _rng.take(x.numel()), st
        return ops.dropout(x, p, st, ctx.off)

    @staticmethod
    def backward(ctx, dy):
        return ops.dropout(dy.contiguous(), ctx.p, ctx.state, ctx.off), None


class _DropoutAdd(torch.autograd.Function):

    @staticmethod
    def forward(ctx, x, res, p):
        st = _rng.tensor(x.device)
        ctx.p, ctx.off, ctx.state = p, _rng.take(x.numel()), st
        return ops.dropout_fused(x, p, st, ctx.off, residual=res.contiguous())

    @staticmethod
    def backward(ctx, dy):
        dy = dy.contiguous()
        return ops.dropout(dy, ctx.p, ctx.state, ctx.off), dy, None


class _ReluDropout(torch.autograd.Function):

    @staticmethod
    def forward(ctx, x, p):
        st = _rng.tensor(x.device)
        y = ops.dropout_fused(x, p, st, _rng.take(x.numel()), relu=True)
        ctx.p = p
        ctx.save_for_backward(y)
        return y

    @staticmethod
    def backward(ctx, dy):
        (y,) = ctx.saved_tensors
        return ops.dropout_fused(dy.contiguous(), ctx.p, None, 0, gate=y), None


def dropout_add(x: Tensor, res: Tensor, p: float, training: bool) -> Tensor:
    if not training or p <= 0.0:
        return add(res, x)
    if p >= 1.0:
        raise ValueError("dropout p must be < 1")
    return _DropoutAdd.apply(x, res, float(p))


def relu_dropout(x: Tensor, p: float, training: bool) -> Tensor:
    if not training or p <= 0.0:
        return relu(x)
    if p >= 1.0:
        raise ValueError("dropout p must be < 1")
    return _ReluDropout.apply(x, float(p))


def dropout(x: Tensor, p: float, training: bool) -> Tensor:
    if not training or p <= 0.0:
        return x
    if p >= 1.0:
        raise ValueError("dropout p must be < 1")
    return _Dropout.apply(x, float(p))


class _LstmLayer(torch.autograd.Function):

    @staticmethod
    def forward(ctx, x, w_ih, w_hh, b_ih, b_hh):
        ctx.set_materialize_grads(False)
        B, T, Fdim = x.shape
        x2 = x.reshape(B * T, Fdim)
        if not x2.is_contiguous():
            x2 = x2.contiguous()
        wih, whh = _wc(w_ih, x.dtype), _wc(w_hh, x.dtype)
        G = ops.linear_fwd(x2, wih)
        h_out, h_prev, gates, c, h_last = ops.lstm_seq_fwd(G, whh, _f32(b_ih), _f32(b_hh), B, T, want_last=True)
        ctx.save_for_backward(x2, wih, whh, h_prev, gates, c)
        ctx.xshape = x.shape
        return h_out, h_last

    @staticmethod
    def backward(ctx, dh_seq, dh_last):
        x2, wih, whh, h_prev, gates, c = ctx.saved_tensors
        if dh_seq is None and dh_last is None:
            return None, None, None, None, None
        if dh_seq is not None:
            dh_seq = _as(dh_seq.contiguous(), whh.dtype)
        if dh_last is not None:
            dh_last = _as(dh_last.contiguous(), whh.dtype)
        dG = ops.lstm_seq_bwd(whh, gates, c, dh_seq, dh_last)
        H4 = dG.shape[1]
        db = torch.empty((H4,), dtype=torch.float32, device=dG.device)
        dx = None
        if ctx.needs_input_grad[0]:
            dw_ih, dx2 = ops.linear_backward(dG, x2, wih, bias_out=db)
            dx = dx2.view(ctx.xshape)
        else:
            dw_ih = ops.linear_wgrad(dG, x2, bias_out=db)
        dw_hh = ops.linear_wgrad(dG, h_prev.view(-1, h_prev.shape[-1]))
        db_hh = ops.copy_(torch.empty_like(db), db)
        return dx, dw_ih, dw_hh, db, db_hh


def lstm_layer(x: Tensor, w_ih: Tensor, w_hh: Tensor, b_ih: Optional[Tensor], b_hh: Optional[Tensor]):
    return _LstmLayer.apply(x, w_ih, w_hh, b_ih, b_hh)


class _SigmoidBce(torch.autograd.Function):
    @staticmethod
    def forward(ctx, z, target):
        zc = z.contiguous()
        t32 = _f32(target)
        ctx.save_for_backward(zc, t32)
        return ops.sigmoid_bce_fwd(zc, t32).view(())

    @staticmethod
    def backward(ctx, gloss):
        zc, t32 = ctx.saved_tensors
        return ops.sigmoid_bce_bwd(zc, t32, _f32(gloss).reshape(1)), None


def sigmoid_bce(z: Tensor, target: Tensor) -> Tensor:
    return _SigmoidBce.apply(z, target)


def _conv3d_pack(conv: torch.nn.Conv3d, bn, Cp: int, dtype: torch.dtype, K: int, Cop: Optional[int] = None):
    ts = [conv.weight] + ([bn.weight, bn.bias, bn.running_mean, bn.running_var] if bn is not None else [])
    stamp = tuple((t.data_ptr(), t._version) for t in ts if t is not None) + ((bn.eps,) if bn is not None else ())
    cache = conv.__dict__.setdefault("_dvt_conv3d_cache", {})
    Cout = conv.out_channels
    Cop = Cout if Cop is None else Cop
    key = (dtype, Cp, K) if Cop == Cout else (dtype, Cp, K, Cop)
    hit = cache.get(key)
    if hit is not None and hit[0] == stamp:
        return hit[1]
    wsrc = conv.weight
    if Cop != Cout:
        wsrc = torch.zeros((Cop,) + tuple(conv.weight.shape[1:]), dtype=torch.float32, device=conv.weight.device)
        wsrc[:Cout] = conv.weight.detach()
    w = ops.conv3d_weight_pack(wsrc, Cp, K, dtype)
    scale = shift = None
    if bn is not None:
        scale, shift = ops.bn_fold(bn.weight, bn.bias, bn.running_mean, bn.running_var, bn.eps)
        if Cop != Cout:
            scale = torch.cat((scale, scale.new_zeros(Cop - Cout)))
            shift = torch.cat((shift, shift.new_zeros(Cop - Cout)))
    cache.clear()
    cache[key] = (stamp, (w, scale, shift))
    return w, scale, shift


CONV3D_ROUTES = ("implicit", "l1")


def conv3d_bn_act(x: Tensor, conv: torch.nn.Conv3d, bn, geom, *, relu: bool, residual: Optional[Tensor] = None,
                  dtype: torch.dtype = torch.bfloat16, cout_multiple: int = 1, route: str = "implicit"):
    if torch.is_grad_enabled() and (x.requires_grad or any(p.requires_grad for p in conv.parameters())
                                    or (bn is not None and any(p.requires_grad for p in bn.parameters()))):
        raise RuntimeError("conv3d_bn_act is inference-only (no backward): call it under torch.no_grad() / "
                           "torch.inference_mode()")
    if bn is not None and (bn.training or bn.running_mean is None):
        raise RuntimeError("conv3d_bn_act folds an eval-mode BatchNorm (running statistics): put the module in eval()")
    assert conv.groups == 1 and conv.bias is None and tuple(conv.dilation) == (1, 1, 1)
    if x.dtype != dtype:
        raise TypeError(f"conv3d_bn_act: map is {x.dtype}, compute dtype {dtype}")
    k, s, p = tuple(conv.kernel_size), tuple(conv.stride), tuple(conv.padding)
    Cout = -(-conv.out_channels // cout_multiple) * cout_multiple
    K = ops.conv3d_implicit_k(x, geom, Cout, k, s, p)
    w, scale, shift = _conv3d_pack(conv, bn, x.shape[1], dtype, K, Cout)
    if route == "l1":
        y = ops.conv2p1d_l1(x, w, geom, Cout, k, s, p, scale=scale, shift=shift, residual=residual, relu=relu)
    elif route == "implicit":
        y = ops.conv3d_implicit(x, w, geom, Cout, k, s, p, scale=scale, shift=shift, residual=residual, relu=relu)
    else:
        raise ValueError(f"conv3d_bn_act: route {route!r} not in {CONV3D_ROUTES}")
    return (y,) + ops.conv3d_out(geom, k, s, p)


def _bn_grad_targets(bn_w: Tensor, bn_b: Tensor):
    sg, sb = _sink(bn_w), _sink(bn_b)
    C = bn_w.shape[0]
    if sg is not None and sb is not None and sg.fresh == sb.fresh:
        def finish():
            sg.mark_written()
            sb.mark_written()
            return None, None
        return sg.buf.view(-1), sb.buf.view(-1), not sg.fresh, finish
    dg = torch.empty(C, dtype=torch.float32, device=bn_w.device)
    db = torch.empty(C, dtype=torch.float32, device=bn_w.device)

    def finish_tmp():
        if sg is None and sb is None:
            return dg, db
        for s, t in ((sg, dg), (sb, db)):
            if s is not None:
                _emit_into(s, t)
        return (dg if sg is None else None), (db if sb is None else None)
    return dg, db, False, finish_tmp


def _bn_module_args(bn, training: bool):
    if bn.momentum is None:
        raise NotImplementedError("BatchNorm1d(momentum=None) (cumulative average) has no HIP kernel")
    if not bn.affine:
# ... 190 lines not shown
```

### data-efficient-video-transformers_amd/models/vit.py

```python
from __future__ import annotations

import torch
from torch import nn

from .. import functional as F


class Patchify(nn.Module):

    def __init__(self, patch_size: int, tubelet_size: int = 1):
        super().__init__()
        self.patch_size = patch_size
        self.tubelet_size = tubelet_size

    def forward(self, x):
        from .. import ops
        b, t = x.shape[0], x.shape[1]
        out = ops.tubelet_patchify(x, self.patch_size, self.tubelet_size, x.dtype)
        return out.view(b, t // self.tubelet_size, -1, out.shape[-1])


def inflate_patch_embedding(weight2d, tubelet_size: int, mode: str = "central"):
    if mode not in ("central", "average"):
        raise ValueError(f"inflate_patch_embedding: mode must be 'central' or 'average', got {mode!r}")
    if int(tubelet_size) != tubelet_size or tubelet_size < 1:
        raise ValueError(f"inflate_patch_embedding: tubelet_size must be an integer >= 1, got {tubelet_size!r}")
    if weight2d.dim() != 2:
        raise ValueError(f"inflate_patch_embedding: expected a weight [dim, P*P*C], got shape {tuple(weight2d.shape)}")
    pt = int(tubelet_size)
    d, pd = weight2d.shape
    w = weight2d.detach()
    if mode == "average":
        return (w / pt).repeat(1, pt)
    out = torch.zeros((d, pt * pd), dtype=w.dtype, device=w.device)
    out[:, (pt // 2) * pd:(pt // 2 + 1) * pd] = w
    return out


class GELU(nn.Module):

    def forward(self, x):
        return F.gelu(x)


class PreNorm(nn.Module):

    def __init__(self, dim, fn):
        super().__init__()
        self.norm = nn.LayerNorm(dim)
        self.fn = fn

    def forward(self, x, **kwargs):
        if isinstance(self.fn, (Attention, FeedForward)) and not kwargs:
            return self.fn(x, _norm=self.norm)
        return self.fn(F.layernorm(x, self.norm.weight, self.norm.bias, self.norm.eps), **kwargs)


class FeedForward(nn.Module):

    def __init__(self, dim, hidden_dim, dropout=0.):
        super().__init__()
        self.net = nn.Sequential(
            nn.Linear(dim, hidden_dim),
            GELU(),
            nn.Dropout(dropout),
            nn.Linear(hidden_dim, dim),
            nn.Dropout(dropout),
        )
        self.dropout_p = dropout

    def forward(self, x, _norm=None, _residual=False, _cdt=None):
        l1, l2 = self.net[0], self.net[3]
        if self.training and self.dropout_p > 0.0:
            h = F.layernorm(x, _norm.weight, _norm.bias, _norm.eps) if _norm is not None else x
            h = F.dropout(F.gelu(F.linear(h, l1.weight, l1.bias)), self.dropout_p, True)
            y = F.dropout(F.linear(h, l2.weight, l2.bias), self.dropout_p, True)
            return F.add(x, y) if _residual else y
        return F.mlp_block(x, _norm.weight if _norm is not None else None,
                           _norm.bias if _norm is not None else None,
                           l1.weight, l1.bias, l2.weight, l2.bias, act="gelu",
                           prenorm=_norm is not None, residual=_residual,
                           eps=_norm.eps if _norm is not None else 1e-5, cdt=_cdt)


class Attention(nn.Module):

    def __init__(self, dim, heads=8, dim_head=64, dropout=0.):
        super().__init__()
        inner_dim = dim_head * heads
        project_out = not (heads == 1 and dim_head == dim)
        self.heads = heads
        self.scale = dim_head ** -0.5
        self.to_qkv = nn.Linear(dim, inner_dim * 3, bias=False)
        self.to_out = nn.Sequential(
            nn.Linear(inner_dim, dim),
            nn.Dropout(dropout),
        ) if project_out else nn.Identity()
        self.project_out = project_out
        self.dropout_p = dropout

    def forward(self, x, _norm=None, _residual=False, _cdt=None):
        w_out = self.to_out[0].weight if self.project_out else None
        b_out = self.to_out[0].bias if self.project_out else None
        if self.training and self.dropout_p > 0.0 and self.project_out:
            y = F.attn_block(x, _norm.weight if _norm is not None else None, _norm.bias if _norm is not None else None,
                             self.to_qkv.weight, w_out, b_out, self.heads, prenorm=_norm is not None, residual=False,
                             eps=_norm.eps if _norm is not None else 1e-5)
            y = F.dropout(y, self.dropout_p, True)
            return F.add(x, y) if _residual else y
        return F.attn_block(x, _norm.weight if _norm is not None else None,
                            _norm.bias if _norm is not None else None,
                            self.to_qkv.weight, w_out, b_out, self.heads,
                            prenorm=_norm is not None, residual=_residual,
                            eps=_norm.eps if _norm is not None else 1e-5, cdt=_cdt)


class Transformer(nn.Module):

    def __init__(self, dim, depth, heads, dim_head, mlp_dim, dropout=0.):
        super().__init__()
        self.layers = nn.ModuleList([])
        self.norm = nn.LayerNorm(dim)
        self.checkpoint = False
        for _ in range(depth):
            self.layers.append(nn.ModuleList([
                PreNorm(dim, Attention(dim, heads=heads, dim_head=dim_head, dropout=dropout)),
                PreNorm(dim, FeedForward(dim, mlp_dim, dropout=dropout)),
            ]))

    def stream_f32_ok(self, rows: int, cdt: torch.dtype) -> bool:
        if cdt not in (torch.bfloat16, torch.float16) or len(self.layers) == 0:
            return False
        attn, ff = self.layers[0][0].fn, self.layers[0][1].fn
        if not attn.project_out or (self.training and (attn.dropout_p > 0.0 or ff.dropout_p > 0.0)):
            return False
        d, inner, hidden = attn.to_out[0].weight.shape[0], attn.to_out[0].weight.shape[1], ff.net[0].weight.shape[0]
        from .. import ops
        return ops.gemm_is_launch_bound(rows, d, inner, cdt) and ops.gemm_is_launch_bound(rows, d, hidden, cdt)

    def forward_layers(self, x, cdt=None):
        for attn, ff in self.layers:
            if self.checkpoint and self.training and torch.is_grad_enabled():
                def block(t, attn=attn, ff=ff):
                    t = attn.fn(t, _norm=attn.norm, _residual=True, _cdt=cdt)
                    return ff.fn(t, _norm=ff.norm, _residual=True, _cdt=cdt)
                x = F.checkpoint(block, x, tuple(attn.parameters()) + tuple(ff.parameters()))
            else:
                x = attn.fn(x, _norm=attn.norm, _residual=True, _cdt=cdt)
                x = ff.fn(x, _norm=ff.norm, _residual=True, _cdt=cdt)
        return x

    def cls_prunable(self) -> bool:
        if len(self.layers) == 0:
            return False
        attn = self.layers[-1][0].fn
        dropping = self.training and (attn.dropout_p > 0.0 or self.layers[-1][1].fn.dropout_p > 0.0)
        return attn.project_out and not dropping

    def forward_layers_cls(self, x, cdt=None):
        *head, (attn, ff) = self.layers
        for a, f in head:
            if self.checkpoint and self.training and torch.is_grad_enabled():
                def block(t, a=a, f=f):
                    t = a.fn(t, _norm=a.norm, _residual=True, _cdt=cdt)
                    return f.fn(t, _norm=f.norm, _residual=True, _cdt=cdt)
                x = F.checkpoint(block, x, tuple(a.parameters()) + tuple(f.parameters()))
            else:
                x = a.fn(x, _norm=a.norm, _residual=True, _cdt=cdt)
                x = f.fn(x, _norm=f.norm, _residual=True, _cdt=cdt)

        def last(t):
            an, af = attn.norm, attn.fn
            c = F.attn_block_cls(t, an.weight, an.bias, af.to_qkv.weight, af.to_out[0].weight, af.to_out[0].bias,
                                 af.heads, eps=an.eps, cdt=cdt)
            return ff.fn(c, _norm=ff.norm, _residual=True, _cdt=cdt)

        if self.checkpoint and self.training and torch.is_grad_enabled():
            return F.checkpoint(last, x, tuple(attn.parameters()) + tuple(ff.parameters()))
        return last(x)

    def forward(self, x, cdt=None):
        x = self.forward_layers(x, cdt)
        return F.layernorm(x, self.norm.weight, self.norm.bias, self.norm.eps)


class ViViT(nn.Module):

    def __init__(self, image_size, patch_size, num_classes, num_frames, dim=192, depth=4, heads=3,
                 pool='cls', in_channels=3, dim_head=64, dropout=0., emb_dropout=0., scale_dim=4, *,
                 compute_dtype: torch.dtype = torch.bfloat16, activation_checkpointing: bool = False,
                 tubelet_size: int = 1):
        super().__init__()
        assert pool in {'cls', 'mean'}, 'pool type must be either cls (cls token) or mean (mean pooling)'
        assert image_size % patch_size == 0, 'Image dimensions must be divisible by the patch size.'
        if isinstance(tubelet_size, bool) or not isinstance(tubelet_size, int) or tubelet_size < 1:
            raise ValueError(f"tubelet_size must be an integer >= 1, got {tubelet_size!r}")
        if num_frames % tubelet_size != 0:
            raise ValueError(f"num_frames = {num_frames} is not a multiple of tubelet_size = {tubelet_size}")
        num_patches = (image_size // patch_size) ** 2
        patch_dim = tubelet_size * in_channels * patch_size ** 2
        self.to_patch_embedding = nn.Sequential(
            Patchify(patch_size, tubelet_size),
            nn.Linear(patch_dim, dim),
        )
        self.pos_embedding = nn.Parameter(torch.randn(1, num_frames // tubelet_size, num_patches + 1, dim))
        self.space_token = nn.Parameter(torch.randn(1, 1, dim))
        self.space_transformer = Transformer(dim, depth, heads, dim_head, dim * scale_dim, dropout)
        self.temporal_token = nn.Parameter(torch.randn(1, 1, dim))
        self.temporal_transformer = Transformer(dim, depth, heads, dim_head, dim * scale_dim, dropout)
        self.dropout = nn.Dropout(emb_dropout)
        self.pool = pool
        self.mlp_head = nn.Sequential(
            nn.LayerNorm(dim),
            nn.Linear(dim, num_classes),
        )
        self.patch_size = patch_size
        self.num_patches = num_patches
        self.num_frames = num_frames
        self.tubelet_size = tubelet_size
        self.emb_dropout_p = emb_dropout
        self.compute_dtype = compute_dtype
        self.zone_f32 = True
        self.space_transformer.checkpoint = activation_checkpointing
        self.temporal_transformer.checkpoint = activation_checkpointing

    def forward(self, x):
        pooled, pending = self._trunk(x)
        if pending is not None:
            pooled = F.layernorm(pooled, pending.weight, pending.bias, pending.eps)
        hn, hl = self.mlp_head[0], self.mlp_head[1]
        h = F.layernorm(pooled, hn.weight, hn.bias, hn.eps)
        return F.linear(h, hl.weight, hl.bias, out_f32=True)

    def loss(self, x, target):
        pooled, pending = self._trunk(x)
        hn, hl = self.mlp_head[0], self.mlp_head[1]
        if pooled.is_cuda and F.head_bce_supported(pooled, hl.weight):
            mixed = pooled.dtype == torch.float32 and self.compute_dtype in (torch.bfloat16, torch.float16)
            return F.head_bce(pooled, pending, hn, hl, target, lp_dtype=self.compute_dtype if mixed else None)
        if pending is not None:
            pooled = F.layernorm(pooled, pending.weight, pending.bias, pending.eps)
        logits = F.linear(F.layernorm(pooled, hn.weight, hn.bias, hn.eps), hl.weight, hl.bias, out_f32=True)
        return F.bce_with_logits(logits, target), logits

    def load_frame_checkpoint(self, state_dict, mode: str = "central"):
        if mode not in ("central", "average"):
            raise ValueError(f"load_frame_checkpoint: mode must be 'central' or 'average', got {mode!r}")
        pt = self.tubelet_size
        own = self.state_dict()
        for k in own:
            if k not in state_dict:
                raise ValueError(f"load_frame_checkpoint: key {k!r} is missing from the checkpoint")
        for k in state_dict:
            if k not in own:
                raise ValueError(f"load_frame_checkpoint: unexpected key {k!r} in the checkpoint")
        new = {}
        for k, dst in own.items():
            src = state_dict[k].detach()
            if k == "to_patch_embedding.1.weight":
                if src.dim() != 2 or (src.shape[0], src.shape[1] * pt) != tuple(dst.shape):
                    raise ValueError(f"load_frame_checkpoint: {k!r} has shape {tuple(src.shape)}; a per-frame weight "
                                     f"[{dst.shape[0]}, {dst.shape[1] // pt}] is expected")
                src = inflate_patch_embedding(src, pt, mode)
            elif k == "pos_embedding":
                want = (1, self.num_frames) + tuple(dst.shape[2:])
                if tuple(src.shape) != want:
                    raise ValueError(f"load_frame_checkpoint: {k!r} has shape {tuple(src.shape)}; the per-frame table "
                                     f"{want} is expected")
                if mode == "central":
                    src = src[:, pt // 2::pt]
                else:
                    src = src.reshape(1, self.num_frames // pt, pt, *src.shape[2:]).mean(2)
            elif tuple(src.shape) != tuple(dst.shape):
                raise ValueError(f"load_frame_checkpoint: {k!r} has shape {tuple(src.shape)}, the model's is "
                                 f"{tuple(dst.shape)}")
            new[k] = src
        with torch.no_grad():
            for k, dst in own.items():
                dst.copy_(new[k])

    def _trunk(self, x):
        if x.dim() != 5:
            raise ValueError("ViViT expects a clip tensor [b, t, c, H, W]")
        b, t = x.shape[0], x.shape[1]
        if t != self.num_frames:
            raise ValueError(f"clip has {t} frames but pos_embedding was built for {self.num_frames} "
                             "(vit.py:94,115 broadcast)")
        t //= self.tubelet_size
        T = self.compute_dtype
        F.lp_clear()
        n = (x.shape[3] // self.patch_size) * (x.shape[4] // self.patch_size)
        pe = self.to_patch_embedding[1]
        emb = F.patch_embed(x, pe.weight, pe.bias, self.patch_size, T, tubelet=self.tubelet_size)
        tok = F.tokens_assemble(emb, self.space_token, self.pos_embedding, b * t, t, n)
        tok = F.dropout(tok, self.emb_dropout_p, self.training)
        st, tt = self.space_transformer, self.temporal_transformer
        sn = st.norm
        if st.cls_prunable():
            s = st.forward_layers_cls(tok).view(b * t, 1, -1)
        else:
            s = st.forward_layers(tok)
        zone32 = self.zone_f32 and tt.stream_f32_ok(b * (t + 1), T)
        cdt = T if zone32 else None
        seq = F.cls_norm_concat(s, sn.weight, sn.bias, self.temporal_token, b, t, sn.eps,
                                out_dtype=torch.float32 if zone32 else None)
        if self.pool == 'cls' and tt.cls_prunable():
            return tt.forward_layers_cls(seq, cdt), tt.norm
        z = tt(seq, cdt)
        return (F.mean_rows(z) if self.pool == 'mean' else F.select_first_row(z)), None
```

### data-efficient-video-transformers_amd/ops.py

```python
from __future__ import annotations

import ctypes as C
import re
from typing import NamedTuple, Optional, Tuple

import torch

from . import _lib as L

Tensor = torch.Tensor

_DT = {torch.float32: L.F32, torch.bfloat16: L.BF16, torch.float16: L.F16}
_TORCH_DT = {L.F32: torch.float32, L.BF16: torch.bfloat16, L.F16: torch.float16}


def dt(t: Tensor) -> int:
    try:
        return _DT[t.dtype]
    except KeyError:
        raise TypeError(f"dtype {t.dtype} is not supported by libdvt_hip (float32 / bfloat16)")


def _stream() -> int:
    return torch.cuda.current_stream().cuda_stream
# ... 92 lines not shown
    _need_cuda(x, table)
    assert x.is_contiguous() and table.is_contiguous() and table.dtype == torch.float32
    d = x.shape[-1]
    rows = x.numel() // d
    assert table.shape[-1] == d and table.numel() // d * rows_per_entry >= rows
    out = torch.empty_like(x)
    L.check(L.load().dvt_add_rowtable(x.data_ptr(), table.data_ptr(), out.data_ptr(), rows, d, rows_per_entry,
                                      dt(x), _stream()), "dvt_add_rowtable")
    return out


def copy_(dst: Tensor, src: Tensor) -> Tensor:
    _need_cuda(dst, src)
    assert dst.is_contiguous() and src.is_contiguous() and dst.numel() == src.numel()
    L.check(L.load().dvt_cast(src.data_ptr(), dt(src), dst.data_ptr(), dt(dst), src.numel(), _stream()), "dvt_cast")
    return dst


def copy2d(src: Tensor, dst: Tensor, rows: int, cols: int, src_ld: int, dst_ld: int) -> None:
    _need_cuda(src, dst)
    assert src.dtype == dst.dtype
    L.check(L.load().dvt_copy2d(src.data_ptr(), dst.data_ptr(), rows, cols, src_ld, dst_ld, dt(src), _stream()),
            "dvt_copy2d")


def rows_sum(src: Tensor, row_stride: int, rows: int, cols: int, *, out: Optional[Tensor] = None,
             accumulate: bool = False) -> Tensor:
    _need_cuda(src)
    if out is None:
        assert not accumulate
        out = torch.empty((cols,), dtype=torch.float32, device=src.device)
    L.check(L.load().dvt_rows_sum(src.data_ptr(), row_stride, rows, cols, out.data_ptr(), dt(src), int(accumulate),
                                  _stream()), "dvt_rows_sum")
    return out


def permute_021(x: Tensor) -> Tensor:
    _need_cuda(x)
    x = x.contiguous()
    A, B, Cc = x.shape
    out = torch.empty((B, A, Cc), dtype=x.dtype, device=x.device)
    L.check(L.load().dvt_permute_021(x.data_ptr(), out.data_ptr(), A, B, Cc, dt(x), _stream()), "dvt_permute_021")
    return out


def axpby_f32_(dst: Tensor, src: Tensor, alpha: float = 1.0, beta: float = 1.0) -> Tensor:
    _need_cuda(dst, src)
    assert dst.dtype == torch.float32 and dst.is_contiguous() and src.is_contiguous()
    assert dst.numel() == src.numel()
    L.check(L.load().dvt_axpby_f32(src.data_ptr(), dt(src), alpha, dst.data_ptr(), beta, dst.numel(), _stream()),
            "dvt_axpby_f32")
    return dst


ACT_GELU, ACT_RELU, ACT_SIGMOID = 1, 2, 3


def act_fwd(x: Tensor, act: int) -> Tensor:
    _need_cuda(x)
    x = x.contiguous()
    y = torch.empty_like(x)
    L.check(L.load().dvt_act_fwd(x.data_ptr(), y.data_ptr(), x.numel(), act, dt(x), _stream()), "dvt_act_fwd")
    return y


def act_bwd(dy: Tensor, x: Tensor, act: int) -> Tensor:
    _need_cuda(dy, x)
    dy = dy.contiguous()
    dx = torch.empty_like(x)
    L.check(L.load().dvt_act_bwd(dy.data_ptr(), x.data_ptr(), dx.data_ptr(), x.numel(), act, dt(x), _stream()),
            "dvt_act_bwd")
    return dx


def _tubelet_geometry(shape, patch: int, tubelet: int, what: str):
    if len(shape) < 4:
        raise ValueError(f"{what}: expected a clip [..., t, C, H, W], got shape {tuple(shape)}")
    if int(tubelet) != tubelet or tubelet < 1:
        raise ValueError(f"{what}: tubelet must be an integer >= 1, got {tubelet!r}")
    t, Cc, H, W = (int(s) for s in shape[-4:])
    if t % tubelet:
        raise ValueError(f"{what}: {t} frames per clip are not whole tubelets of {tubelet}")
    frames = 1
    for s in shape[:-3]:
        frames *= int(s)
    return frames, Cc, H, W


def _patch_gather(what: str, src: Tensor, shape, patch: int, tubelet: Optional[int], dtype: torch.dtype) -> Tensor:
    _need_cuda(src)
    if tubelet is None:
        frames, Cc, H, W = _tubelet_geometry((1, *shape), patch, 1, what)
    else:
        frames, Cc, H, W = _tubelet_geometry(shape, patch, tubelet, what)
    pt = () if tubelet is None else (tubelet,)
    src = src.contiguous()
    if what.endswith("_bwd"):
        if src.numel() != frames * Cc * H * W:
            raise ValueError(f"{what}: dout {tuple(src.shape)} does not hold a clip of shape {tuple(shape)}")
        dst = torch.empty(tuple(shape), dtype=dtype, device=src.device)
    else:
        rows = frames // (tubelet or 1) * (H // patch) * (W // patch)
        dst = torch.empty((rows, (tubelet or 1) * patch * patch * Cc), dtype=dtype, device=src.device)
    with _timed(("hbm", what, src.numel()), src.numel() * src.element_size() + dst.numel() * dst.element_size()):
        L.check(getattr(L.load(), "dvt_" + what)(src.data_ptr(), dt(src), dst.data_ptr(), _DT[dtype], frames, Cc, H, W, patch,
                                                 *pt, _stream()), "dvt_" + what)
    return dst


def patchify(x: Tensor, patch: int, out_dtype: torch.dtype) -> Tensor:
    return _patch_gather("patchify", x, x.shape, patch, None, out_dtype)


def patchify_bwd(dout: Tensor, shape, patch: int, dx_dtype: torch.dtype) -> Tensor:
    return _patch_gather("patchify_bwd", dout, shape, patch, None, dx_dtype)


def tubelet_patchify(x: Tensor, patch: int, tubelet: int, out_dtype: torch.dtype) -> Tensor:
    return _patch_gather("tubelet_patchify", x, x.shape, patch, tubelet, out_dtype)


def tubelet_patchify_bwd(dout: Tensor, shape, patch: int, tubelet: int, dx_dtype: torch.dtype) -> Tensor:
    return _patch_gather("tubelet_patchify_bwd", dout, shape, patch, tubelet, dx_dtype)

def tokens_assemble_fwd(emb: Tensor, cls: Tensor, pos: Tensor, S: int, T: int, n: int) -> Tensor:
    _need_cuda(emb, cls, pos)
    d = emb.shape[-1]
    assert emb.is_contiguous() and cls.is_contiguous() and pos.is_contiguous()
    assert cls.dtype == torch.float32 and pos.dtype == torch.float32
    out = torch.empty((S, n + 1, d), dtype=emb.dtype, device=emb.device)
    with _timed(("hbm", "tokens_assemble_fwd", emb.numel()), (emb.numel() + out.numel()) * emb.element_size() + pos.numel() * 4):
        L.check(L.load().dvt_tokens_assemble_fwd(emb.data_ptr(), cls.data_ptr(), pos.data_ptr(), out.data_ptr(), S, T,
                                                 n, d, pos.shape[-2], dt(emb), _stream()), "dvt_tokens_assemble_fwd")
    return out


def tokens_assemble_bwd(dout: Tensor, T: int, pos_rows: int, *, dcls: Optional[Tensor] = None,
                        dpos: Optional[Tensor] = None, accumulate: bool = False) -> Tuple[Tensor, Tensor, Tensor]:
    _need_cuda(dout)
    dout = dout.contiguous()
    S, n1, d = dout.shape
    n = n1 - 1
    demb = torch.empty((S * n, d), dtype=dout.dtype, device=dout.device)
    if dcls is None:
        assert not accumulate
        dcls = torch.empty((d,), dtype=torch.float32, device=dout.device)
    if dpos is None:
        assert not accumulate
        dpos = torch.empty((T, pos_rows, d), dtype=torch.float32, device=dout.device)
    assert dcls.is_contiguous() and dpos.is_contiguous() and dcls.numel() == d and dpos.numel() == T * pos_rows * d
    L.check(L.load().dvt_tokens_assemble_bwd(dout.data_ptr(), demb.data_ptr(), dcls.data_ptr(), dpos.data_ptr(), S,
                                             T, n, d, pos_rows, dt(dout), int(accumulate), _stream()),
            "dvt_tokens_assemble_bwd")
    return demb, dcls, dpos


def rows_gather_fwd(src: Tensor, row_stride: int, tok: Optional[Tensor], B: int, T: int, d: int) -> Tensor:
    _need_cuda(src, tok)
    lead = 0 if tok is None else 1
    out = torch.empty((B, T + lead, d), dtype=src.dtype, device=src.device)
    L.check(L.load().dvt_rows_gather_fwd(src.data_ptr(), row_stride, _p(tok), out.data_ptr(), B, T, d, dt(src),
                                         _stream()), "dvt_rows_gather_fwd")
    return out


def rows_gather_bwd(dout: Tensor, dsrc: Tensor, row_stride: int, want_tok: bool, B: int, T: int,
                    d: int, *, dtok: Optional[Tensor] = None, accumulate: bool = False) -> Optional[Tensor]:
    _need_cuda(dout, dsrc)
    dout = dout.contiguous()
    if want_tok and dtok is None:
        assert not accumulate
        dtok = torch.empty((d,), dtype=torch.float32, device=dout.device)
    if not want_tok:
        dtok = None
    L.check(L.load().dvt_rows_gather_bwd(dout.data_ptr(), dsrc.data_ptr(), row_stride, _p(dtok), B, T, d, dt(dout),
                                         int(accumulate), _stream()), "dvt_rows_gather_bwd")
    return dtok


def mean_rows_fwd(x: Tensor, scale: Optional[float] = None) -> Tensor:
    _need_cuda(x)
    x = x.contiguous()
    B, Ln, d = x.shape
    out = torch.empty((B, d), dtype=x.dtype, device=x.device)
    sc = 1.0 / Ln if scale is None else scale
    L.check(L.load().dvt_mean_rows_fwd(x.data_ptr(), out.data_ptr(), B, Ln, d, sc, dt(x), _stream()),
            "dvt_mean_rows_fwd")
    return out


def mean_rows_bwd(dout: Tensor, Ln: int, scale: Optional[float] = None) -> Tensor:
    _need_cuda(dout)
    dout = dout.contiguous()
    B, d = dout.shape
    dx = torch.empty((B, Ln, d), dtype=dout.dtype, device=dout.device)
    sc = 1.0 / Ln if scale is None else scale
    L.check(L.load().dvt_mean_rows_bwd(dout.data_ptr(), dx.data_ptr(), B, Ln, d, sc, dt(dout), _stream()),
            "dvt_mean_rows_bwd")
    return dx


def layernorm_fwd(x: Tensor, gamma: Tensor, beta: Tensor, eps: float = 1e-5, *, rows=None,
                  out: Optional[Tensor] = None, out_rows=None, out_dtype: Optional[torch.dtype] = None
                  ) -> Tuple[Tensor, Tensor, Tensor]:
    _need_cuda(x, gamma, beta)
    d = x.shape[-1]
    ydt = x.dtype if out_dtype is None else out_dtype
    if rows is None:
        assert x.is_contiguous()
        n0, n1, xs0, xs1 = x.numel() // d, 1, d, 0
        if out is None:
            out = torch.empty(x.shape, dtype=ydt, device=x.device)
        ys0, ys1 = d, 0
    else:
        n0, n1, xs0, xs1 = rows
        if out is None:
            out = torch.empty((n0 * n1, d), dtype=ydt, device=x.device)
        ys0, ys1 = out_rows if out_rows is not None else (n1 * d, d)
    assert out.dtype == ydt
    nrows = n0 * n1
    mean = torch.empty((nrows,), dtype=torch.float32, device=x.device)
    rstd = torch.empty((nrows,), dtype=torch.float32, device=x.device)
    with _timed(("hbm", "layernorm_fwd", nrows), nrows * (d * (x.element_size() + out.element_size()) + 8)):
        L.check(L.load().dvt_layernorm_fwd_mixed(x.data_ptr(), dt(x), gamma.data_ptr(), beta.data_ptr(), out.data_ptr(),
                                                 dt(out), mean.data_ptr(), rstd.data_ptr(), n0, n1, d, xs0, xs1, ys0, ys1,
                                                 eps, _stream()), "dvt_layernorm_fwd")
    return out, mean, rstd


_ln_deferred = []
LN_DEFER_MAX = 24


def layernorm_flush() -> None:
    global _ln_deferred
    if not _ln_deferred:
        return
    todo, _ln_deferred = _ln_deferred, []
    arr = (L.LnPending * len(todo))(*[pn for pn, _ in todo])
    L.check(L.load().dvt_layernorm_reduce_group(arr, len(todo), _stream()), "dvt_layernorm_reduce_group")
    for pn, done in todo:
        pn.valid = 0
        if done is not None:
            done()


def layernorm_bwd(dy: Tensor, x: Tensor, gamma: Tensor, mean: Tensor, rstd: Tensor, *,
                  dx_add: Optional[Tensor] = None, rows=None, dy_rows=None,
                  dx: Optional[Tensor] = None, dg: Optional[Tensor] = None, db: Optional[Tensor] = None,
                  accumulate: bool = False, accumulate_beta: Optional[bool] = None,
                  dy_first: Optional[Tensor] = None, dx_first: Optional[Tensor] = None,
                  dx_dtype: Optional[torch.dtype] = None, dx_lp: Optional[torch.dtype] = None, defer=None):
    _need_cuda(dy, x, gamma, mean, rstd, dx_add, dy_first, dx_first)
    d = x.shape[-1]
    if rows is None:
        assert x.is_contiguous() and dy.is_contiguous()
        n0, n1, xs0, xs1 = x.numel() // d, 1, d, 0
        ys0, ys1 = d, 0
    else:
        n0, n1, xs0, xs1 = rows
        ys0, ys1 = dy_rows if dy_rows is not None else (d * n1, d)
    dxt = x.dtype if dx_dtype is None else dx_dtype
    assert dy_first is None or (dy_first.dim() == 2 and dy_first.shape == (n0, d) and dy_first.stride(1) == 1 and dy_first.dtype == dy.dtype)
    assert dx_first is None or (dx_first.dim() == 2 and dx_first.shape == (n0, d) and dx_first.stride(1) == 1 and dx_first.dtype == dxt)
    if dx is None:
        dx = torch.empty(x.shape, dtype=dxt, device=x.device)
    assert dx.dtype == dxt and (dx_add is None or dx_add.dtype == dxt)
    if dg is None or db is None:
        assert not accumulate and not accumulate_beta and dg is None and db is None
        dg = torch.empty((d,), dtype=torch.float32, device=x.device)
        db = torch.empty((d,), dtype=torch.float32, device=x.device)
    acc_b = accumulate if accumulate_beta is None else accumulate_beta
    lib = L.load()
    q = L.LnBwdDesc()
    q.dy, q.dy_dtype, q.x, q.x_dtype = dy.data_ptr(), dt(dy), x.data_ptr(), dt(x)
    q.gamma, q.mean, q.rstd = gamma.data_ptr(), mean.data_ptr(), rstd.data_ptr()
    q.dx_add, q.dx, q.dx_dtype = _p(dx_add), dx.data_ptr(), _DT[dxt]
    lp = None
    if dx_lp is not None:
        lp = torch.empty(x.shape, dtype=dx_lp, device=x.device)
        q.dx_lp, q.dx_lp_dtype = lp.data_ptr(), _DT[dx_lp]
    q.dgamma, q.dbeta = dg.data_ptr(), db.data_ptr()
    q.n0, q.n1, q.d, q.xs0, q.xs1, q.ys0, q.ys1 = n0, n1, d, xs0, xs1, ys0, ys1
    q.dy_first, q.dy_first_stride = _p(dy_first), dy_first.stride(0) if dy_first is not None else 0
    q.dx_first, q.dx_first_stride = _p(dx_first), dx_first.stride(0) if dx_first is not None else 0
    q.accumulate_gamma, q.accumulate_beta = int(accumulate), int(acc_b)
    pending = None
    if defer:
        ws = torch.empty((lib.dvt_layernorm_bwd_partial_bytes(n0 * n1, d),), dtype=torch.uint8, device=x.device)
        pending = L.LnPending()
        pending._keep = (ws, dg, db)
        q.defer_reduce, q.pending = 1, C.pointer(pending)
    else:
        ws = workspace(lib.dvt_layernorm_bwd_workspace_bytes(d), x.device)
    q.workspace = ws.data_ptr()
    nb = n0 * n1 * (d * (dy.element_size() + x.element_size() + dx.element_size() * (1 + (dx_add is not None))) + 8)
    with _timed(("hbm", "layernorm_bwd", n0 * n1), nb):
        L.check(lib.dvt_layernorm_bwd_ex(C.byref(q), _stream()), "dvt_layernorm_bwd")
    if defer:
        _ln_deferred.append((pending, defer if callable(defer) else None))
        if len(_ln_deferred) >= LN_DEFER_MAX:
            layernorm_flush()
    return (dx, dg, db) if dx_lp is None else (dx, dg, db, lp)


def _gemm_desc(A: Tensor, B: Tensor, M: int, N: int, K: int, *, a_kmajor: bool, b_kmajor: bool, lda: int, ldb: int,
               out: Optional[Tensor] = None, out_dtype: Optional[torch.dtype] = None, epilogue: int = L.EPI_NONE,
               bias: Optional[Tensor] = None, residual: Optional[Tensor] = None, aux: Optional[Tensor] = None,
               accumulate: bool = False, alpha: float = 1.0, split_k: int = 0, colsum_out: Optional[Tensor] = None,
               colsum_accumulate: bool = False, _launch: bool = True):
    if _launch:
        _need_cuda(A, B, bias, residual, aux)
    assert A.dtype == B.dtype
    if out_dtype is None:
        out_dtype = A.dtype
    if out is None:
        assert not accumulate
        out = torch.empty((M, N), dtype=out_dtype, device=A.device)
    assert out.dtype == out_dtype and out.stride(-1) == 1
    if bias is not None:
        assert bias.dtype == torch.float32 and bias.numel() == N
    d = L.GemmDesc()
    if residual is not None and residual.dtype != A.dtype:
        assert residual.dtype == torch.float32 and out_dtype == torch.float32 and epilogue == L.EPI_RESIDUAL
        d.residual_f32 = 1
    d.A, d.B, d.C = A.data_ptr(), B.data_ptr(), out.data_ptr()
    d.M, d.N, d.K = M, N, K
    d.lda, d.ldb, d.ldc = lda, ldb, out.stride(0) if out.dim() == 2 else N
    d.a_kmajor, d.b_kmajor = int(a_kmajor), int(b_kmajor)
    d.in_dtype, d.out_dtype = dt(A), _DT[out_dtype]
    d.epilogue, d.accumulate = epilogue, int(accumulate)
    d.bias = _p(bias)
    d.residual = _p(residual)
    d.ldr = residual.stride(0) if residual is not None else 0
    d.aux = _p(aux)
    d.ldaux = aux.stride(0) if aux is not None else 0
    d.alpha = alpha
    d.split_k = split_k
    if colsum_out is not None:
        assert colsum_out.dtype == torch.float32 and colsum_out.numel() == M and colsum_out.is_contiguous()
    d.colsum_out = _p(colsum_out)
    d.colsum_accumulate = int(colsum_accumulate)
    return d, out


def gemm(A: Tensor, B: Tensor, M: int, N: int, K: int, *, a_kmajor: bool, b_kmajor: bool,
         lda: int, ldb: int, out: Optional[Tensor] = None, out_dtype: Optional[torch.dtype] = None,
         epilogue: int = L.EPI_NONE, bias: Optional[Tensor] = None, residual: Optional[Tensor] = None,
         aux: Optional[Tensor] = None, accumulate: bool = False, alpha: float = 1.0,
         split_k: int = 0, colsum_out: Optional[Tensor] = None, colsum_accumulate: bool = False,
         defer_reduce: bool = False, carry=None):
    d, out = _gemm_desc(A, B, M, N, K, a_kmajor=a_kmajor, b_kmajor=b_kmajor, lda=lda, ldb=ldb, out=out, out_dtype=out_dtype,
                        epilogue=epilogue, bias=bias, residual=residual, aux=aux, accumulate=accumulate, alpha=alpha,
                        split_k=split_k, colsum_out=colsum_out, colsum_accumulate=colsum_accumulate)
    out_dtype = out.dtype
    pending = None
    if defer_reduce:
        pending = L.SplitKPending()
        pending._keep = (out, colsum_out)
        d.defer_reduce = 1
        d.pending = C.pointer(pending)
    if carry is not None:
        d.carry = C.pointer(carry)
    lib = L.load()
    nws = lib.dvt_gemm_workspace_bytes(C.byref(d))
    ws = _deferred_workspace(nws, A.device, pending) if defer_reduce else workspace(nws, A.device)
    d.workspace = _p(ws)
    if defer_reduce:
        pending._keep += (ws,)
    prof = _profiler
    if prof is not None:
        esz, osz = A.element_size(), out.element_size()
        nbytes = esz * (M * K + N * K) + osz * M * N * (2 if accumulate else 1)
        nbytes += esz * M * N * ((residual is not None) + (aux is not None))
        key = ("gemm", int(a_kmajor), int(b_kmajor), M, N, K, epilogue, nbytes)
        prof.begin(key, 2.0 * M * N * K)
        L.check(lib.dvt_gemm(C.byref(d), _stream()), "dvt_gemm")
        prof.end(key)
        return (out, pending) if defer_reduce else out
    L.check(lib.dvt_gemm(C.byref(d), _stream()), "dvt_gemm")
    return (out, pending) if defer_reduce else out


class GemmPlan(NamedTuple):
    kernel: str
    cfg: int = -1
    split: int = 1
    k_per_split: int = 0
    tile_m: int = 0
    reduce: str = "none"
    colsum: str = "none"
    carry: str = "none"
    a_kmajor: bool = True
    b_kmajor: bool = True
    epilogue: int = L.EPI_NONE
    out: str = "in"


def _enum_names(enum: str, prefix: str) -> Tuple[str, ...]:
    names = {v: re.fullmatch(prefix + r"(\w+)", k).group(1).lower() for k, v in L.ENUMS[enum].items()}
    return tuple(names[i] for i in range(len(names)))


GEMM_OUTS = ("in", "f32", "slab")
GEMM_KERNELS = _enum_names("dvt_gemm_kernel", "DVT_GEMM_K_")
GEMM_REDUCES = _enum_names("dvt_gemm_reduce", "DVT_GEMM_R_")
GEMM_COLSUMS = _enum_names("dvt_gemm_colsum", "DVT_GEMM_CS_")
GEMM_CARRIES = _enum_names("dvt_gemm_carry", "DVT_GEMM_CARRY_")


def _plan_tuple(q) -> GemmPlan:
    return GemmPlan(GEMM_KERNELS[q.kernel], q.cfg, q.split, q.k_per_split, q.tile_m, GEMM_REDUCES[q.reduce],
                    GEMM_COLSUMS[q.colsum], GEMM_CARRIES[q.carry], bool(q.a_kmajor), bool(q.b_kmajor), q.epilogue,
                    GEMM_OUTS[q.out_form])


def _plan_desc(A: Tensor, B: Tensor, M: int, N: int, K: int, *, defer_reduce: bool = False, carry=None, **kw):
    d, out = _gemm_desc(A, B, M, N, K, _launch=False, **kw)
    keep = [out]
    if defer_reduce:
        keep.append(L.SplitKPending())
        d.defer_reduce, d.pending = 1, C.pointer(keep[-1])
    if carry is not None:
        d.carry = C.pointer(carry)
    d.workspace = 256 if L.load().dvt_gemm_workspace_bytes(C.byref(d)) > 0 else None
    return d, keep


def gemm_plan(A: Tensor, B: Tensor, M: int, N: int, K: int, **kw) -> GemmPlan:
    d, _keep = _plan_desc(A, B, M, N, K, **kw)
    q = L.GemmPlanInfo()
    L.check(L.load().dvt_gemm_plan(C.byref(d), C.byref(q)), "dvt_gemm_plan")
    return _plan_tuple(q)


def gemm_pair_plan(wgrad: dict, dgrad: dict) -> Tuple[GemmPlan, GemmPlan]:
    wd, _kw = _plan_desc(**wgrad)
    gd, _kg = _plan_desc(**dgrad)
    qw, qg = L.GemmPlanInfo(), L.GemmPlanInfo()
    L.check(L.load().dvt_gemm_pair_plan(C.byref(wd), C.byref(gd), C.byref(qw), C.byref(qg)), "dvt_gemm_pair_plan")
    return _plan_tuple(qw), _plan_tuple(qg)


def gemm_is_launch_bound(M: int, N: int, K: int, dtype: torch.dtype, *, a_kmajor: bool = True, b_kmajor: bool = True) -> bool:
    if dtype not in (torch.bfloat16, torch.float16):
        return False
    d = L.GemmDesc()
    d.A = d.B = d.C = 16
    d.M, d.N, d.K = M, N, K
    d.lda, d.ldb, d.ldc = (K if a_kmajor else M), (K if b_kmajor else N), N
    d.a_kmajor, d.b_kmajor = int(a_kmajor), int(b_kmajor)
    d.in_dtype = d.out_dtype = _DT[dtype]
    d.alpha = 1.0
    return L.load().dvt_gemm_route(C.byref(d)) == 0


def splitk_reduce_pending(pending) -> None:
    if pending is not None and pending.valid:
        L.check(L.load().dvt_splitk_reduce_pending(C.byref(pending), _stream()), "dvt_splitk_reduce_pending")
        pending.valid = 0


def linear_fwd(x: Tensor, w: Tensor, bias: Optional[Tensor] = None, *, epilogue: int = L.EPI_NONE,
               residual: Optional[Tensor] = None, aux: Optional[Tensor] = None,
               out_dtype: Optional[torch.dtype] = None) -> Tensor:
    M, K = x.shape
    N = w.shape[0]
    assert w.shape[1] == K and x.stride(1) == 1 and w.is_contiguous()
    return gemm(x, w, M, N, K, a_kmajor=True, b_kmajor=True, lda=x.stride(0), ldb=K, epilogue=epilogue,
                bias=bias, residual=residual, aux=aux, out_dtype=out_dtype)


def linear_dgrad(dy: Tensor, w: Tensor, *, epilogue: int = L.EPI_NONE, aux: Optional[Tensor] = None,
                 carry=None) -> Tensor:
    M, N = dy.shape
    K = w.shape[1]
    assert w.shape[0] == N and dy.stride(1) == 1 and w.is_contiguous()
    out = gemm(dy, w, M, K, N, a_kmajor=True, b_kmajor=False, lda=dy.stride(0), ldb=K, epilogue=epilogue,
               aux=aux, carry=carry)
    if carry is not None:
        carry.valid = 0
    return out


def linear_wgrad(dy: Tensor, x: Tensor, *, out: Optional[Tensor] = None, accumulate: bool = False,
                 bias_out: Optional[Tensor] = None, bias_accumulate: bool = False, defer_reduce: bool = False):
    M, N = dy.shape
    K = x.shape[1]
    assert x.shape[0] == M and dy.stride(1) == 1 and x.stride(1) == 1
    return gemm(dy, x, N, K, M, a_kmajor=False, b_kmajor=False, lda=dy.stride(0), ldb=x.stride(0), out=out,
                out_dtype=torch.float32, accumulate=accumulate, colsum_out=bias_out,
                colsum_accumulate=bias_accumulate, defer_reduce=defer_reduce)


PAIR_LAUNCH = True


def linear_backward(dy: Tensor, x: Tensor, w: Tensor, *, out: Optional[Tensor] = None, accumulate: bool = False,
                    bias_out: Optional[Tensor] = None, bias_accumulate: bool = False, epilogue: int = L.EPI_NONE,
                    aux: Optional[Tensor] = None) -> Tuple[Tensor, Tensor]:
    M, N = dy.shape
    K = x.shape[1]
    assert x.shape[0] == M and dy.stride(1) == 1 and x.stride(1) == 1 and w.shape == (N, K) and w.is_contiguous()
    wd, out = _gemm_desc(dy, x, N, K, M, a_kmajor=False, b_kmajor=False, lda=dy.stride(0), ldb=x.stride(0), out=out,
                         out_dtype=torch.float32, accumulate=accumulate, colsum_out=bias_out,
                         colsum_accumulate=bias_accumulate)
    gd, _ = _gemm_desc(dy, w, M, K, N, a_kmajor=True, b_kmajor=False, lda=dy.stride(0), ldb=K, out=dy[:, :0].new_empty((0, K)),
                       epilogue=epilogue, aux=aux)
    gd.C, gd.ldc = dy.data_ptr(), K
    lib = L.load()
    if PAIR_LAUNCH and lib.dvt_gemm_pair_fused(C.byref(wd), C.byref(gd)):
        dx = torch.empty((M, K), dtype=dy.dtype, device=dy.device)
        gd.C, gd.ldc = dx.data_ptr(), K
        L.check(lib.dvt_gemm_pair(C.byref(wd), C.byref(gd), _stream()), "dvt_gemm_pair")
        return out, dx
    _, pend = linear_wgrad(dy, x, out=out, accumulate=accumulate, bias_out=bias_out, bias_accumulate=bias_accumulate,
                           defer_reduce=True)
    return out, linear_dgrad(dy, w, epilogue=epilogue, aux=aux, carry=pend)


def colsum(x: Tensor, *, out: Optional[Tensor] = None, accumulate: bool = False) -> Tensor:
    _need_cuda(x)
    M, N = x.shape
    assert x.stride(1) == 1
    if out is None:
        assert not accumulate
        out = torch.empty((N,), dtype=torch.float32, device=x.device)
    assert out.dtype == torch.float32 and out.numel() == N and out.is_contiguous()
    lib = L.load()
    ws = workspace(lib.dvt_colsum_workspace_bytes(M, N), x.device)
    L.check(lib.dvt_colsum(x.data_ptr(), x.stride(0), out.data_ptr(), _p(ws), M, N, dt(x), int(accumulate),
                           _stream()), "dvt_colsum")
    return out


def _attn_desc(q: Tensor, k: Tensor, v: Tensor, o: Tensor, lse: Tensor, scale: float, dropout=None) -> L.AttnDesc:
    for t in (q, k, v, o):
        assert t.dim() == 4 and t.stride(3) == 1, "attention operands must be [B,H,L,dh] views, dh contiguous"
    B, H, Lq, dh = q.shape
    Lk = k.shape[2]
    assert k.shape == (B, H, Lk, dh) and v.shape == (B, H, Lk, dh) and o.shape == (B, H, Lq, dh)
    d = L.AttnDesc()
    d.q, d.k, d.v, d.o, d.lse = q.data_ptr(), k.data_ptr(), v.data_ptr(), o.data_ptr(), lse.data_ptr()
    d.B, d.H, d.Lq, d.Lk, d.dh = B, H, Lq, Lk, dh
    d.q_sb, d.q_sh, d.q_sl = q.stride(0), q.stride(1), q.stride(2)
    d.k_sb, d.k_sh, d.k_sl = k.stride(0), k.stride(1), k.stride(2)
    d.v_sb, d.v_sh, d.v_sl = v.stride(0), v.stride(1), v.stride(2)
    d.o_sb, d.o_sh, d.o_sl = o.stride(0), o.stride(1), o.stride(2)
    d.scale = scale
    d.dtype = dt(q)
    if dropout is not None:
        d.dropout_p, d.rng_state, d.rng_offset = float(dropout[0]), dropout[1].data_ptr(), int(dropout[2])
    return d


def attention_fwd(q: Tensor, k: Tensor, v: Tensor, o: Tensor, scale: float, dropout=None,
                  lse: Optional[Tensor] = None) -> Tensor:
    _need_cuda(q, k, v, o)
    B, H, Lq, _ = q.shape
    if lse is None:
        lse = torch.empty((B, H, Lq), dtype=torch.float32, device=q.device)
    else:
        assert lse.dtype == torch.float32 and lse.is_contiguous() and lse.numel() == B * H * Lq and lse.device == q.device
    d = _attn_desc(q, k, v, o, lse, scale, dropout)
    nb = (2 * q.numel() + k.numel() + v.numel()) * q.element_size()
    with _timed(("hbm", "attention_fwd", q.numel(), 4.0 * q.numel() * k.shape[2]), nb):
        L.check(L.load().dvt_attention_fwd(C.byref(d), _stream()), "dvt_attention_fwd")
    return lse


ATTN_BWD_TWO_PASS = False


def attention_bwd(q: Tensor, k: Tensor, v: Tensor, o: Tensor, lse: Tensor, do: Tensor, dq: Tensor,
                  dk: Tensor, dv: Tensor, scale: float, dropout=None, two_pass: Optional[bool] = None,
                  ws: Optional[Tensor] = None) -> None:
    _need_cuda(q, k, v, o, do, dq, dk, dv)
    for a, b in ((do, o), (dq, q), (dk, k), (dv, v)):
        assert a.shape == b.shape and all(sa == sb for sa, sb, n in zip(a.stride(), b.stride(), a.shape) if n > 1), \
            "gradient views must share the layout of their primal"
    d = _attn_desc(q, k, v, o, lse, scale, dropout)
    d.d_o, d.dq, d.dk, d.dv = do.data_ptr(), dq.data_ptr(), dk.data_ptr(), dv.data_ptr()
    d.bwd_two_pass = int(ATTN_BWD_TWO_PASS if two_pass is None else two_pass)
    lib = L.load()
    need = lib.dvt_attention_bwd_workspace_bytes(C.byref(d))
    if ws is None:
        ws = workspace(need, q.device)
    else:
        assert ws.device == q.device and ws.numel() * ws.element_size() >= need
    d.workspace = _p(ws)
    nb = (4 * q.numel() + 2 * k.numel() + 2 * v.numel()) * q.element_size()
    with _timed(("hbm", "attention_bwd", q.numel(), 10.0 * q.numel() * k.shape[2]), nb):
        L.check(lib.dvt_attention_bwd(C.byref(d), _stream()), "dvt_attention_bwd")


class AttnPlan(NamedTuple):
    family: str
    count: int = 0
    count2: int = 0
    waves: int = 0
    waves2: int = 0
    patch: Optional[bool] = None
    patch2: Optional[bool] = None
    workspace: bool = False
    lds: int = 0
    lds2: int = 0
# ... 2190 lines not shown
```

### include/dvt_hip.h

```cpp
#ifndef DVT_HIP_H
#define DVT_HIP_H

#include <stddef.h>
#include <stdint.h>

#ifdef __cplusplus
extern "C" {
#endif

#define DVT_ABI_VERSION 5

typedef void* dvt_stream_t;

enum dvt_dtype { DVT_F32 = 0, DVT_BF16 = 1, DVT_F16 = 2 };

enum dvt_status {
  DVT_OK = 0,
  DVT_ERR_BAD_ARG = -1,
  DVT_ERR_UNSUPPORTED = -2,
  DVT_ERR_HIP = -3
};

int dvt_version(void);
const char* dvt_last_error(void);
int dvt_device_info(int* cu_count, int* lds_bytes, char* arch, int arch_len);

int dvt_cast(const void* src, int src_dtype, void* dst, int dst_dtype, int64_t n,
             dvt_stream_t stream);
int dvt_add(const void* a, const void* b, void* out, int64_t n, int dtype, dvt_stream_t stream);
int dvt_add_rowtable(const void* x, const float* table, void* out, int64_t rows, int64_t d,
                     int64_t rows_per_entry, int dtype, dvt_stream_t stream);
int dvt_copy2d(const void* src, void* dst, int64_t rows, int64_t cols, int64_t src_ld, int64_t dst_ld,
               int dtype, dvt_stream_t stream);
int dvt_rows_sum(const void* src, int64_t row_stride, int64_t rows, int64_t cols, float* out,
                 int dtype, int accumulate, dvt_stream_t stream);
int dvt_permute_021(const void* src, void* dst, int64_t A, int64_t B, int64_t C, int dtype,
                    dvt_stream_t stream);
int dvt_axpby_f32(const void* src, int src_dtype, float alpha, float* dst, float beta, int64_t n,
                  dvt_stream_t stream);

int dvt_act_fwd(const void* x, void* y, int64_t n, int act, int dtype, dvt_stream_t stream);
int dvt_act_bwd(const void* dy, const void* x, void* dx, int64_t n, int act, int dtype,
                dvt_stream_t stream);

int dvt_device_delay(uint64_t microseconds, dvt_stream_t stream);
int dvt_zero(void* dst, size_t nbytes, dvt_stream_t stream);

int dvt_dropout(const void* x, void* y, int64_t n, float p, const uint64_t* rng_state, uint64_t call_offset, int dtype,
                dvt_stream_t stream);
int dvt_dropout_fused(const void* x, const void* residual, const void* gate, void* y, int64_t n, float p,
                      const uint64_t* rng_state, uint64_t call_offset, int relu, int dtype, dvt_stream_t stream);
int dvt_rng_advance(uint64_t* rng_state, uint64_t delta, dvt_stream_t stream);

int dvt_patchify(const void* x, int x_dtype, void* out, int out_dtype, int64_t frames, int C,
                 int H, int W, int P, dvt_stream_t stream);
int dvt_patchify_bwd(const void* dout, int dout_dtype, void* dx, int dx_dtype, int64_t frames,
                     int C, int H, int W, int P, dvt_stream_t stream);
int dvt_tubelet_patchify(const void* x, int x_dtype, void* out, int out_dtype, int64_t frames, int C, int H, int W, int P,
                         int pt, dvt_stream_t stream);
int dvt_tubelet_patchify_bwd(const void* dout, int dout_dtype, void* dx, int dx_dtype, int64_t frames, int C, int H, int W,
                             int P, int pt, dvt_stream_t stream);

int dvt_tokens_assemble_fwd(const void* emb, const float* cls, const float* pos, void* out,
                            int64_t S, int64_t T, int64_t n, int64_t d, int64_t pos_rows,
                            int dtype, dvt_stream_t stream);
int dvt_tokens_assemble_bwd(const void* dout, void* demb, float* dcls, float* dpos, int64_t S,
                            int64_t T, int64_t n, int64_t d, int64_t pos_rows, int dtype,
                            int accumulate, dvt_stream_t stream);

int dvt_rows_gather_fwd(const void* src, int64_t src_row_stride, const float* tok, void* out,
                        int64_t B, int64_t T, int64_t d, int dtype, dvt_stream_t stream);
int dvt_rows_gather_bwd(const void* dout, void* dsrc, int64_t src_row_stride, float* dtok,
                        int64_t B, int64_t T, int64_t d, int dtype, int accumulate,
                        dvt_stream_t stream);

int dvt_mean_rows_fwd(const void* x, void* out, int64_t B, int64_t L, int64_t d, float scale, int dtype,
                      dvt_stream_t stream);
int dvt_mean_rows_bwd(const void* dout, void* dx, int64_t B, int64_t L, int64_t d, float scale, int dtype,
                      dvt_stream_t stream);

int dvt_layernorm_fwd(const void* x, const float* gamma, const float* beta, void* y, float* mean,
                      float* rstd, int64_t n0, int64_t n1, int64_t d, int64_t xs0, int64_t xs1,
                      int64_t ys0, int64_t ys1, float eps, int dtype, dvt_stream_t stream);
size_t dvt_layernorm_bwd_workspace_bytes(int64_t d);
int dvt_layernorm_bwd(const void* dy, const void* x, const float* gamma, const float* mean,
                      const float* rstd, const void* dx_add, void* dx, float* dgamma,
                      float* dbeta, void* workspace,
                      int64_t n0, int64_t n1, int64_t d, int64_t xs0, int64_t xs1, int64_t ys0,
                      int64_t ys1, int dtype, int accumulate, dvt_stream_t stream);
int dvt_layernorm_bwd_first(const void* dy, const void* x, const float* gamma, const float* mean,
                            const float* rstd, const void* dx_add, void* dx, float* dgamma, float* dbeta,
                            void* workspace,
                            int64_t n0, int64_t n1, int64_t d, int64_t xs0, int64_t xs1, int64_t ys0,
                            int64_t ys1, const void* dy_first, int64_t dy_first_stride,
                            const void* dx_first, int64_t dx_first_stride, int dtype,
                            int accumulate_gamma, int accumulate_beta, dvt_stream_t stream);

typedef struct dvt_ln_pending {
  const float* partial;
  int32_t nparts, d;
  float* dgamma;
  float* dbeta;
  int32_t accumulate;
  int32_t valid;
} dvt_ln_pending;
typedef struct dvt_ln_bwd_desc {
  const void* dy; int32_t dy_dtype;
  const void* x; int32_t x_dtype;
  const float* gamma; const float* mean; const float* rstd;
  const void* dx_add;
  void* dx; int32_t dx_dtype;
  void* dx_lp; int32_t dx_lp_dtype;
  float* dgamma; float* dbeta; void* workspace;
  int64_t n0, n1, d, xs0, xs1, ys0, ys1;
  const void* dy_first; int64_t dy_first_stride;
  const void* dx_first; int64_t dx_first_stride;
  int32_t accumulate_gamma, accumulate_beta;
  int32_t defer_reduce;
  dvt_ln_pending* pending;
} dvt_ln_bwd_desc;
int dvt_layernorm_fwd_mixed(const void* x, int x_dtype, const float* gamma, const float* beta, void* y, int y_dtype, float* mean,
                            float* rstd, int64_t n0, int64_t n1, int64_t d, int64_t xs0, int64_t xs1,
                            int64_t ys0, int64_t ys1, float eps, dvt_stream_t stream);
size_t dvt_layernorm_bwd_partial_bytes(int64_t rows, int64_t d);
int dvt_layernorm_bwd_ex(const dvt_ln_bwd_desc* desc, dvt_stream_t stream);
int dvt_layernorm_reduce_group(const dvt_ln_pending* list, int count, dvt_stream_t stream);

enum dvt_epilogue {
  DVT_EPI_NONE = 0,
  DVT_EPI_GELU = 1,
  DVT_EPI_RELU = 2,
  DVT_EPI_RESIDUAL = 3,
  DVT_EPI_DGELU = 4,
  DVT_EPI_DRELU = 5
};

typedef struct dvt_splitk_pending {
  const float* slab;
  int32_t splits, valid;
  int64_t M, N;
  float* C;
  int64_t ldc;
  int32_t accumulate;
  int32_t cs_accumulate;
  const float* cs_slab;
  float* cs_out;
  int32_t conv_cin, conv_taps;
  int32_t conv_cin_l, conv_cout_l;
} dvt_splitk_pending;

typedef struct dvt_gemm_desc {
  const void* A;
  const void* B;
  void* C;
  int64_t M, N, K;
  int64_t lda, ldb, ldc;
  int32_t a_kmajor, b_kmajor;
  int32_t in_dtype;
  int32_t out_dtype;
  int32_t epilogue;
  int32_t accumulate;
  const float* bias;
  const void* residual;
  int64_t ldr;
  void* aux;
  int64_t ldaux;
  float alpha;
  int32_t split_k;
  void* workspace;
  float* colsum_out;
  int32_t colsum_accumulate;
  int32_t defer_reduce;
  dvt_splitk_pending* pending;
  const dvt_splitk_pending* carry;
  int32_t residual_f32;
} dvt_gemm_desc;

size_t dvt_gemm_workspace_bytes(const dvt_gemm_desc* desc);
int dvt_gemm(const dvt_gemm_desc* desc, dvt_stream_t stream);
int dvt_gemm_route(const dvt_gemm_desc* desc);
enum dvt_gemm_kernel {
  DVT_GEMM_K_NONE = 0,
  DVT_GEMM_K_SMALL = 1,
  DVT_GEMM_K_SMALL_PAIR = 2,
  DVT_GEMM_K_DMA = 3,
  DVT_GEMM_K_DMA224 = 4,
  DVT_GEMM_K_MFMA128 = 5,
  DVT_GEMM_K_GENERIC64 = 6,
  DVT_GEMM_K_TINY_WAVE = 7,
  DVT_GEMM_K_TINY_THREAD = 8
};
enum dvt_gemm_reduce {
  DVT_GEMM_R_NONE = 0,
  DVT_GEMM_R_PLAIN = 1,
  DVT_GEMM_R_EPILOGUE = 2,
  DVT_GEMM_R_DEFERRED = 3
};
enum dvt_gemm_colsum {
  DVT_GEMM_CS_NONE = 0,
  DVT_GEMM_CS_FUSED = 1,
  DVT_GEMM_CS_ALONE = 2
};
enum dvt_gemm_carry {
  DVT_GEMM_CARRY_NONE = 0,
  DVT_GEMM_CARRY_TAIL = 1,
  DVT_GEMM_CARRY_ALONE = 2,
  DVT_GEMM_CARRY_WIDE = 3,
  DVT_GEMM_CARRY_CONV = 4
};
typedef struct dvt_gemm_plan_info {
  int32_t route;
  int32_t kernel;
  int32_t cfg;
  int32_t split;
  int32_t k_per_split;
  int32_t tile_m;
  int32_t reduce;
  int32_t colsum;
  int32_t carry;
  int32_t a_kmajor, b_kmajor, epilogue, out_form;
} dvt_gemm_plan_info;
int dvt_gemm_plan(const dvt_gemm_desc* desc, dvt_gemm_plan_info* info);
int dvt_gemm_pair_plan(const dvt_gemm_desc* wgrad, const dvt_gemm_desc* dgrad, dvt_gemm_plan_info* wgrad_info,
                       dvt_gemm_plan_info* dgrad_info);
int dvt_gemm_pair_fused(const dvt_gemm_desc* wgrad, const dvt_gemm_desc* dgrad);
int dvt_gemm_pair(const dvt_gemm_desc* wgrad, const dvt_gemm_desc* dgrad, dvt_stream_t stream);
int dvt_splitk_reduce_pending(const dvt_splitk_pending* pending, dvt_stream_t stream);

size_t dvt_colsum_workspace_bytes(int64_t M, int64_t N);
int dvt_colsum(const void* x, int64_t ldx, float* out, void* workspace, int64_t M, int64_t N,
               int dtype, int accumulate, dvt_stream_t stream);

typedef struct dvt_attn_desc {
  const void* q;
  const void* k;
  const void* v;
  void* o;
  float* lse;
  const void* d_o;
  void* dq;
  void* dk;
  void* dv;
  int64_t B, H, Lq, Lk, dh;
  int64_t q_sb, q_sh, q_sl;
  int64_t k_sb, k_sh, k_sl;
  int64_t v_sb, v_sh, v_sl;
  int64_t o_sb, o_sh, o_sl;
  float scale;
  int32_t dtype;
  void* workspace;
  float dropout_p;
  const uint64_t* rng_state;
  uint64_t rng_offset;
  int32_t bwd_two_pass;
} dvt_attn_desc;

size_t dvt_attention_bwd_workspace_bytes(const dvt_attn_desc* desc);
int dvt_attention_fwd(const dvt_attn_desc* desc, dvt_stream_t stream);
int dvt_attention_bwd(const dvt_attn_desc* desc, dvt_stream_t stream);
enum dvt_attn_family {
  DVT_ATTN_F_NONE = 0,
  DVT_ATTN_F_Q1 = 1,
  DVT_ATTN_F_RES = 2,
  DVT_ATTN_F_ONLINE = 3,
  DVT_ATTN_F_SMALL = 4,
  DVT_ATTN_F_GENERIC = 5,
  DVT_ATTN_B_Q1 = 6,
  DVT_ATTN_B_FUSED = 7,
  DVT_ATTN_B_PAIR = 8,
  DVT_ATTN_B_SMALL = 9,
  DVT_ATTN_B_GENERIC = 10
};
typedef struct dvt_attn_plan_info {
  int32_t family;
  int32_t count;
  int32_t count2;
  int32_t waves;
  int32_t waves2;
  int32_t patch;
  int32_t patch2;
  int32_t workspace;
  int64_t lds;
  int64_t lds2;
} dvt_attn_plan_info;
int dvt_attention_plan(const dvt_attn_desc* desc, int bwd, dvt_attn_plan_info* info);

typedef struct dvt_attn_cls_desc {
  const void* x;
  int64_t xs0, xs1;
  const float* gamma;
  const float* beta;
  float eps;
  int64_t S, N, d, H;
  int32_t dtype;
  const float* R;
  float* A;
  float* lse;
  float* P;
  float* mean;
  float* rstd;
  const float* dM;
  void* dx;
  float* G;
  float* dgamma;
  float* dbeta;
  int32_t accumulate_gamma, accumulate_beta;
  void* workspace;
} dvt_attn_cls_desc;

int dvt_attn_cls_supported(const dvt_attn_cls_desc* desc);
size_t dvt_attn_cls_bwd_workspace_bytes(const dvt_attn_cls_desc* desc);
int dvt_attn_cls_fwd(const dvt_attn_cls_desc* desc, dvt_stream_t stream);
int dvt_attn_cls_bwd(const dvt_attn_cls_desc* desc, dvt_stream_t stream);
int dvt_heads_expand(const void* in, int64_t ld_in, const void* W, int64_t ldw, float* out, int64_t S, int64_t H,
                     int64_t dh, int64_t d, float alpha, int dtype, dvt_stream_t stream);
int dvt_heads_contract(const float* in, const float* gamma, const float* beta, const void* W, int64_t ldw, void* out,
                       int64_t ld_out, int64_t S, int64_t H, int64_t dh, int64_t d, float alpha, int dtype,
                       dvt_stream_t stream);
int dvt_heads_outer(const void* a, int64_t lda, const float* b, const float* gamma, const float* beta, float* dW,
                    int64_t ldw, int64_t S, int64_t H, int64_t dh, int64_t d, float alpha, int accumulate, int dtype,
                    dvt_stream_t stream);
int dvt_heads_expand_outer(const void* in, int64_t ld_in, const void* W, int64_t ldw, float* out, float alpha_out,
                           const float* v, const float* gamma, const float* beta, float* dW, int64_t ld_dw, float alpha_dw,
                           int accumulate, int64_t S, int64_t H, int64_t dh, int64_t d, int dtype, dvt_stream_t stream);
int dvt_heads_contract_outer(const float* v, const float* gamma, const void* W, int64_t ldw, void* out, int64_t ld_out,
                             float alpha_out, const void* a, int64_t lda, float* dW, int64_t ld_dw, float alpha_dw,
                             int accumulate, int64_t S, int64_t H, int64_t dh, int64_t d, int dtype, dvt_stream_t stream);

size_t dvt_frames_preprocess_workspace_bytes(int64_t frames, int H0, int W0, int resize, int crop);
int dvt_frames_preprocess(const void* src, void* dst, int dst_dtype, int64_t frames, int H0, int W0, int resize,
                          int crop, const float* mean, const float* std, void* workspace, dvt_stream_t stream);
enum dvt_augment_dst { DVT_AUGMENT_U8_HWC = 8 };
size_t dvt_frames_augment_workspace_bytes(int64_t samples, int H0, int W0, int out_h, int out_w);
int dvt_frames_augment(const void* src, int64_t frames, int H0, int W0, const int32_t* table, int64_t samples, void* dst,
                       int dst_dtype, int out_h, int out_w, const float* mean, const float* std, void* workspace,
                       dvt_stream_t stream);
int dvt_frames_erase(void* x, int dtype, int64_t frames, int H, int W, const int32_t* table, const float* value,
                     dvt_stream_t stream);
enum dvt_autoaugment_op { DVT_AA_IDENTITY = 0, DVT_AA_SHEAR_X = 1, DVT_AA_SHEAR_Y = 2, DVT_AA_TRANSLATE_X = 3,
  DVT_AA_TRANSLATE_Y = 4, DVT_AA_ROTATE = 5, DVT_AA_BRIGHTNESS = 6, DVT_AA_COLOR = 7, DVT_AA_CONTRAST = 8,
  DVT_AA_SHARPNESS = 9, DVT_AA_POSTERIZE = 10, DVT_AA_SOLARIZE = 11, DVT_AA_AUTOCONTRAST = 12, DVT_AA_EQUALIZE = 13,
  DVT_AA_INVERT = 14 };
int dvt_frames_autoaugment(const void* src, int64_t samples, int H, int W, const int32_t* table, void* dst, int dst_dtype,
                           const float* mean, const float* std, dvt_stream_t stream);

int dvt_l2norm_rows_fwd(const void* x, void* y, float* inv_norm, int64_t rows, int D, float eps, int dtype,
                        dvt_stream_t stream);
int dvt_l2norm_rows_bwd(const void* dy, const void* y, const float* inv_norm, void* dx, int64_t rows, int D, float eps,
                        int dtype, dvt_stream_t stream);
int dvt_cosine_rows(const void* a, const void* b, float* out, int64_t rows, int D, float eps, int dtype,
                    dvt_stream_t stream);
int dvt_gate_fwd(const void* a, const void* b, void* y, int64_t n, int dtype, dvt_stream_t stream);
int dvt_gate_bwd(const void* dy, const void* a, const void* b, void* da, void* db, int64_t n, int dtype,
                 dvt_stream_t stream);
int dvt_contrastive_fwd(const float* sim, int M, float temperature, float* loss, float* row_lse, float* row_loss,
                        dvt_stream_t stream);
int dvt_contrastive_bwd(const float* sim, const float* row_lse, int M, float temperature, const float* gloss,
                        float* dsim, dvt_stream_t stream);

size_t dvt_f1_samples_workspace_bytes(int64_t N, int T);
int dvt_f1_samples(const float* probs, const unsigned char* labels, int64_t N, int C, const float* thresholds, int T,
                   float* out, void* workspace, dvt_stream_t stream);
size_t dvt_average_precision_workspace_bytes(int64_t N, int C);
int dvt_average_precision(const float* probs, const unsigned char* labels, int64_t N, int C, float* out_samples,
                          float* out_weighted, float* out_per_class, void* workspace, dvt_stream_t stream);
size_t dvt_multilabel_report_workspace_bytes(int64_t N);
int dvt_multilabel_report(const float* probs, const unsigned char* labels, int64_t N, int C, float threshold,
                          int64_t* counts, double* row_sums, void* workspace, dvt_stream_t stream);

int dvt_im2col(const void* x, int x_dtype, int x_nchw, void* out, int out_dtype, int64_t N, int C, int H,
               int W, int kh, int kw, int sh, int sw, int ph, int pw, int64_t ld, dvt_stream_t stream);
int dvt_nchw_to_nhwc_pad(const void* x, int x_dtype, void* y, int y_dtype, int64_t N, int C, int H, int W, int Cpad,
                         dvt_stream_t stream);
int dvt_conv_weight_pairs(const float* w, float* wp, int Cout, int Cin, int kh, int kw, int pw, int kwp, dvt_stream_t stream);
int dvt_conv_weight_pairs_bwd(const float* dwp, float* dw, int Cout, int Cin, int kh, int kw, int pw, int kwp, int accumulate,
                              dvt_stream_t stream);
int dvt_col2im(const void* dcol, void* dx, int64_t N, int C, int H, int W, int kh, int kw, int sh, int sw,
               int ph, int pw, int64_t ld, const void* add, int add_stride, int dtype, dvt_stream_t stream);
int dvt_col2im_nchw(const void* dcol, int dtype, void* dx, int dx_dtype, int64_t N, int C, int H, int W, int kh,
                    int kw, int sh, int sw, int ph, int pw, int64_t ld, dvt_stream_t stream);
int dvt_pad3_f32(const float* src, float* dst, int A, int B, int K, int Ap, int Bp, dvt_stream_t stream);
int dvt_unpad3_f32(const float* src, float* dst, int A, int B, int K, int Bp, int accumulate, dvt_stream_t stream);
int dvt_conv_weight_pack_dgrad(const float* w, void* dst, int dst_dtype, int Cout, int Cin, int kh, int kw,
                               dvt_stream_t stream);
typedef struct dvt_pack_entry {
  const float* src;
  void* dst;
  int32_t cout_l, cin_l, kh, kw, cout_p, cin_p, ld, kind, dtype;
  int32_t cls_sh, cls_sw, cls_rh, cls_rw;
} dvt_pack_entry;
int dvt_conv_weight_pack_group(const dvt_pack_entry* entries, int count, dvt_stream_t stream);
typedef struct dvt_conv_desc {
  const void* x;
  const void* w;
  void* y;
  int64_t N;
  int32_t H, W, C, Cout, kh, kw, sh, sw, ph, pw;
  int32_t dtype;
  void* workspace;
  float* stats_partial;
  int32_t trim_w;
  int32_t defer_reduce;
  dvt_splitk_pending* pending;
  const dvt_splitk_pending* carry;
  const void* residual;
  int32_t wgrad_master_layout, wgrad_accumulate;
  int32_t wgrad_cout_l, wgrad_cin_l;
  int32_t out_h, out_w;
  const int32_t* out_rows;
  int32_t residual_compact;
} dvt_conv_desc;
int dvt_conv3x3_c64_supported(int64_t N, int H, int W, int dtype);
int dvt_conv3x3_c64_wgrad_supported(int64_t N, int H, int W, int dtype);
size_t dvt_conv3x3_c64_wgrad_workspace_bytes(int64_t N, int H, int W);
int dvt_conv3x3_c64_wgrad(const void* x, const void* dz, float* dw, void* workspace, int64_t N, int H, int W, int accumulate,
                          int defer_reduce, dvt_splitk_pending* pending, int dtype, dvt_stream_t stream);
int dvt_conv3x3_c64_wgrad_wide(const void* x, const void* dz, float* dw, void* workspace, int64_t N, int H, int W, int Cout,
                               int accumulate, int defer_reduce, dvt_splitk_pending* pending, int dtype, dvt_stream_t stream);
int dvt_conv3x3_c64_wgrad_plan(int64_t N, int H, int W, int Cout, int dtype, int max_launches, int* c0, int* width, int* mb,
                               int* rows);
typedef struct dvt_bn_affine {
  const float* mean;
  const float* invstd;
  const float* gamma;
  const float* beta;
  int32_t c_valid;
  int32_t relu;
} dvt_bn_affine;
int dvt_conv3x1_fwd_supported(int64_t N, int T, int L, int Cin, int Cout, int dtype);
// ... 357 lines not shown
```

Before: 1409 clips/s.

## Fuse token assembly with first block's LayerNorm in forward and backward

Adds seam kernels that build the token tensor (cls + patch embeddings + positional) and apply the first transformer block's LayerNorm in one pass, with a matching backward that fuses the LN backward, dpos accumulation across the batch and demb/dcls output. The LN row math is factored into a shared header for reuse. The fusion is meant to remove separate assemble and LN kernel launches and an HBM round trip of the token tensor. The fused path is used only when embedding dropout is off and the shape is supported. The backward loops over the batch serially per position row, which may limit parallelism.

Result: no change. 1417 clips/s (median of 6 runs) (+0.6%).

```diff
diff --git a/data-efficient-video-transformers_amd/csrc/layernorm.hip b/data-efficient-video-transformers_amd/csrc/layernorm.hip
--- a/data-efficient-video-transformers_amd/csrc/layernorm.hip
+++ b/data-efficient-video-transformers_amd/csrc/layernorm.hip
@@ -1,5 +1,6 @@
 #include "common.h"
 #include "ln_reduce.h"
+#include "ln_row.h"
 
 namespace {
 
@@ -32,37 +33,19 @@
     const TX* xr = x + i0 * xs0 + i1 * xs1;
     TY* yr = y + i0 * ys0 + i1 * ys1;
     float v[VPL][8];
-    float s = 0.f;
 #pragma unroll
     for (int i = 0; i < VPL; ++i) {
       const int c = (lane + 64 * i) * 8;
-      if (c < d) {
-        load8<TX>(xr + c, v[i]);
-#pragma unroll
-        for (int k = 0; k < 8; ++k) s += v[i][k];
-      }
-    }
-    const float mu = wave_sum_dpp(s) * inv_d;
-    float q = 0.f;
-#pragma unroll
-    for (int i = 0; i < VPL; ++i) {
-      const int c = (lane + 64 * i) * 8;
-      if (c < d) {
-#pragma unroll
-        for (int k = 0; k < 8; ++k) {
-          v[i][k] -= mu;
-          q = fmaf(v[i][k], v[i][k], q);
-        }
-      }
-    }
-    const float rs = rsqrtf(wave_sum_dpp(q) * inv_d + eps);
+      if (c < d) load8<TX>(xr + c, v[i]);
+    }
+    float mu, rs;
+    ln_row_stats<VPL>(v, d, lane, inv_d, eps, mu, rs);
 #pragma unroll
     for (int i = 0; i < VPL; ++i) {
       const int c = (lane + 64 * i) * 8;
       if (c < d) {
         float o[8];
-#pragma unroll
-        for (int k = 0; k < 8; ++k) o[k] = fmaf(v[i][k] * rs, g[i][k], b[i][k]);
+        ln_row_affine(v[i], rs, g[i], b[i], o);
         store8<TY>(yr + c, o);
       }
     }
@@ -118,15 +101,7 @@
 #pragma unroll
           for (int k = 0; k < 8; ++k) dv[k] += fv[k];
         }
-#pragma unroll
-        for (int k = 0; k < 8; ++k) {
-          xh[i][k] = (xv[k] - mu) * rs;
-          gg[i][k] = dv[k] * g[i][k];
-          s1 += gg[i][k];
-          s2 = fmaf(gg[i][k], xh[i][k], s2);
-          dg[i][k] = fmaf(dv[k], xh[i][k], dg[i][k]);
-          db[i][k] += dv[k];
-        }
+        ln_row_bwd_acc(xv, dv, g[i], mu, rs, xh[i], gg[i], dg[i], db[i], s1, s2);
       }
     }
     const float c1 = wave_sum_dpp(s1) * inv_d;
@@ -136,8 +111,7 @@
       const int c = (lane + 64 * i) * 8;
       if (c < d) {
         float o[8];
-#pragma unroll
-        for (int k = 0; k < 8; ++k) o[k] = rs * (gg[i][k] - c1 - xh[i][k] * c2);
+        LN_ROW_BWD_DX(o, gg[i], xh[i], rs, c1, c2);
         if (dx_add) {
           float a[8];
           load8<TDX>(dx_add + xoff + c, a);
@@ -156,24 +130,7 @@
     }
   }
 
-  for (int w = 0; w < kLnBwdBlock / 64; ++w) {
-    if (wid == w) {
-#pragma unroll
-      for (int i = 0; i < VPL; ++i) {
-        const int c = (lane + 64 * i) * 8;
-        if (c < d) {
-#pragma unroll
-          for (int k = 0; k < 8; ++k) {
-            if (w == 0) { lds[c + k] = dg[i][k]; lds[d + c + k] = db[i][k]; }
-            else { lds[c + k] += dg[i][k]; lds[d + c + k] += db[i][k]; }
-          }
-        }
-      }
-    }
-    __syncthreads();
-  }
-  float* out = partial + (int64_t)blockIdx.x * 2 * d;
-  for (int c = threadIdx.x; c < 2 * d; c += kLnBwdBlock) out[c] = lds[c];
+  ln_block_partials<VPL, kLnBwdBlock>(dg, db, lds, d, lane, wid, partial + (int64_t)blockIdx.x * 2 * d);
 }
 
 int ln_check(const char* name, const void* a, const void* b, int64_t n0, int64_t n1, int64_t d,
@@ -189,15 +146,6 @@
 }
 
 }
-
-#define DVT_LN_VPL_SWITCH(vpl, ...)                    \
-  switch (vpl) {                                       \
-    case 1: { constexpr int VPL = 1; __VA_ARGS__; break; } \
-    case 2: { constexpr int VPL = 2; __VA_ARGS__; break; } \
-    case 3: { constexpr int VPL = 3; __VA_ARGS__; break; } \
-    case 4: { constexpr int VPL = 4; __VA_ARGS__; break; } \
-    default: { constexpr int VPL = 8; __VA_ARGS__; break; } \
-  }
 
 #define DVT_LN_FWD_LAUNCH(TX, TY)                                                                                          \
   DVT_LN_VPL_SWITCH(vpl, hipLaunchKernelGGL((ln_fwd_kernel<TX, TY, VPL>), dim3((unsigned)blocks), dim3(kLnBlock), 0, st,    \
diff --git a/data-efficient-video-transformers_amd/csrc/ln_row.h b/data-efficient-video-transformers_amd/csrc/ln_row.h
--- /dev/null
+++ b/data-efficient-video-transformers_amd/csrc/ln_row.h
@@ -0,0 +1,84 @@
+#pragma once
+#include "common.h"
+
+template <int VPL>
+__device__ __forceinline__ void ln_row_stats(float (&v)[VPL][8], int d, int lane, float inv_d, float eps, float& mu,
+                                             float& rs) {
+  float s = 0.f;
+#pragma unroll
+  for (int i = 0; i < VPL; ++i) {
+    const int c = (lane + 64 * i) * 8;
+    if (c < d) {
+#pragma unroll
+      for (int k = 0; k < 8; ++k) s += v[i][k];
+    }
+  }
+  mu = wave_sum_dpp(s) * inv_d;
+  float q = 0.f;
+#pragma unroll
+  for (int i = 0; i < VPL; ++i) {
+    const int c = (lane + 64 * i) * 8;
+    if (c < d) {
+#pragma unroll
+      for (int k = 0; k < 8; ++k) {
+        v[i][k] -= mu;
+        q = fmaf(v[i][k], v[i][k], q);
+      }
+    }
+  }
+  rs = rsqrtf(wave_sum_dpp(q) * inv_d + eps);
+}
+
+__device__ __forceinline__ void ln_row_affine(const float (&vc)[8], float rs, const float (&g)[8], const float (&b)[8],
+                                              float (&o)[8]) {
+#pragma unroll
+  for (int k = 0; k < 8; ++k) o[k] = fmaf(vc[k] * rs, g[k], b[k]);
+}
+
+__device__ __forceinline__ void ln_row_bwd_acc(const float (&xv)[8], const float (&dv)[8], const float (&g)[8], float mu,
+                                               float rs, float (&xh)[8], float (&gg)[8], float (&dg)[8], float (&db)[8],
+                                               float& s1, float& s2) {
+#pragma unroll
+  for (int k = 0; k < 8; ++k) {
+    xh[k] = (xv[k] - mu) * rs;
+    gg[k] = dv[k] * g[k];
+    s1 += gg[k];
+    s2 = fmaf(gg[k], xh[k], s2);
+    dg[k] = fmaf(dv[k], xh[k], dg[k]);
+    db[k] += dv[k];
+  }
+}
+
+#define LN_ROW_BWD_DX(o, gg, xh, rs, c1, c2) \
+  _Pragma("unroll") for (int k = 0; k < 8; ++k) (o)[k] = (rs) * ((gg)[k] - (c1) - (xh)[k] * (c2))
+
+template <int VPL, int BLOCK>
+__device__ __forceinline__ void ln_block_partials(const float (&dg)[VPL][8], const float (&db)[VPL][8], float* lds, int d,
+                                                  int lane, int wid, float* __restrict__ out) {
+  for (int w = 0; w < BLOCK / 64; ++w) {
+    if (wid == w) {
+#pragma unroll
+      for (int i = 0; i < VPL; ++i) {
+        const int c = (lane + 64 * i) * 8;
+        if (c < d) {
+#pragma unroll
+          for (int k = 0; k < 8; ++k) {
+            if (w == 0) { lds[c + k] = dg[i][k]; lds[d + c + k] = db[i][k]; }
+            else { lds[c + k] += dg[i][k]; lds[d + c + k] += db[i][k]; }
+          }
+        }
+      }
+    }
+    __syncthreads();
+  }
+  for (int c = threadIdx.x; c < 2 * d; c += BLOCK) out[c] = lds[c];
+}
+
+#define DVT_LN_VPL_SWITCH(vpl, ...)                    \
+  switch (vpl) {                                       \
+    case 1: { constexpr int VPL = 1; __VA_ARGS__; break; } \
+    case 2: { constexpr int VPL = 2; __VA_ARGS__; break; } \
+    case 3: { constexpr int VPL = 3; __VA_ARGS__; break; } \
+    case 4: { constexpr int VPL = 4; __VA_ARGS__; break; } \
+    default: { constexpr int VPL = 8; __VA_ARGS__; break; } \
+  }
diff --git a/data-efficient-video-transformers_amd/csrc/seams.hip b/data-efficient-video-transformers_amd/csrc/seams.hip
--- /dev/null
+++ b/data-efficient-video-transformers_amd/csrc/seams.hip
@@ -0,0 +1,241 @@
+#include "common.h"
+#include "ln_row.h"
+
+namespace {
+
+constexpr int kSeamBlock = 256;
+constexpr int kSeamMaxBlocks = 1024;
+constexpr int kSeamBwdMaxD = 8 * 64;
+
+template <typename T>
+__device__ __forceinline__ void round8(float (&v)[8]) {
+#pragma unroll
+  for (int k = 0; k < 8; ++k) v[k] = to_f32<T>(from_f32<T>(v[k]));
+}
+
+template <typename T, int VPL>
+__global__ __launch_bounds__(kSeamBlock) void seam_tokens_ln_fwd_kernel(
+    const T* __restrict__ emb, const float* __restrict__ cls, const float* __restrict__ pos,
+    const float* __restrict__ gamma, const float* __restrict__ beta, T* __restrict__ x0, T* __restrict__ xn,
+    float* __restrict__ mean, float* __restrict__ rstd, int64_t S, int64_t Tn, int64_t n, int d, int64_t pos_rows,
+    float eps) {
+  const int lane = threadIdx.x & 63;
+  const int64_t wave = (int64_t)blockIdx.x * (kSeamBlock / 64) + (threadIdx.x >> 6);
+  const int64_t nwaves = (int64_t)gridDim.x * (kSeamBlock / 64);
+  const float inv_d = 1.0f / (float)d;
+  const int64_t rows = S * (n + 1);
+
+  float g[VPL][8], b[VPL][8];
+#pragma unroll
+  for (int i = 0; i < VPL; ++i) {
+    const int c = (lane + 64 * i) * 8;
+    if (c < d) {
+      load8<float>(gamma + c, g[i]);
+      load8<float>(beta + c, b[i]);
+    }
+  }
+
+  for (int64_t r = wave; r < rows; r += nwaves) {
+    const int64_t s = r / (n + 1), j = r - s * (n + 1);
+    const float* pr = pos + ((s % Tn) * pos_rows + j) * d;
+    float v[VPL][8];
+#pragma unroll
+    for (int i = 0; i < VPL; ++i) {
+      const int c = (lane + 64 * i) * 8;
+      if (c < d) {
+        float p[8];
+        load8<float>(pr + c, p);
+        if (j == 0) load8<float>(cls + c, v[i]);
+        else load8<T>(emb + (s * n + (j - 1)) * d + c, v[i]);
+#pragma unroll
+        for (int k = 0; k < 8; ++k) v[i][k] += p[k];
+        store8<T>(x0 + r * d + c, v[i]);
+        round8<T>(v[i]);
+      }
+    }
+    float mu, rs;
+    ln_row_stats<VPL>(v, d, lane, inv_d, eps, mu, rs);
+#pragma unroll
+    for (int i = 0; i < VPL; ++i) {
+      const int c = (lane + 64 * i) * 8;
+      if (c < d) {
+        float o[8];
+        ln_row_affine(v[i], rs, g[i], b[i], o);
+        store8<T>(xn + r * d + c, o);
+      }
+    }
+    if (lane == 0) {
+      mean[r] = mu;
+      rstd[r] = rs;
+    }
+  }
+}
+
+template <typename T, int VPL>
+__global__ __launch_bounds__(kSeamBlock) void seam_ln_tokens_bwd_kernel(
+    const T* __restrict__ dxn, const T* __restrict__ x0, const float* __restrict__ gamma, const float* __restrict__ mean,
+    const float* __restrict__ rstd, const T* dy, T* __restrict__ demb, float* __restrict__ dpos, T* __restrict__ dcls_rows,
+    float* __restrict__ partial , int64_t S, int64_t Tn, int64_t n, int d, int64_t pos_rows,
+    int accumulate) {
+  extern __shared__ __attribute__((aligned(16))) float lds[];
+  const int lane = threadIdx.x & 63;
+  const int wid = threadIdx.x >> 6;
+  const int64_t wave = (int64_t)blockIdx.x * (kSeamBlock / 64) + wid;
+  const int64_t nwaves = (int64_t)gridDim.x * (kSeamBlock / 64);
+  const float inv_d = 1.0f / (float)d;
+  const int64_t B = S / Tn;
+  const int64_t items = Tn * pos_rows;
+
+  float g[VPL][8], dg[VPL][8], db[VPL][8];
+#pragma unroll
+  for (int i = 0; i < VPL; ++i) {
+    const int c = (lane + 64 * i) * 8;
+    if (c < d) load8<float>(gamma + c, g[i]);
+#pragma unroll
+    for (int k = 0; k < 8; ++k) { dg[i][k] = 0.f; db[i][k] = 0.f; }
+  }
+
+  for (int64_t it = wave; it < items; it += nwaves) {
+    const int64_t t = it / pos_rows, j = it - t * pos_rows;
+    float acc[VPL][8];
+#pragma unroll
+    for (int i = 0; i < VPL; ++i)
+#pragma unroll
+      for (int k = 0; k < 8; ++k) acc[i][k] = 0.f;
+    if (j <= n) {
+      for (int64_t bb = 0; bb < B; ++bb) {
+        const int64_t s = bb * Tn + t;
+        const int64_t r = s * (n + 1) + j;
+        const int64_t xoff = r * d;
+        const float mu = mean[r], rs = rstd[r];
+        float xh[VPL][8], gg[VPL][8];
+        float s1 = 0.f, s2 = 0.f;
+#pragma unroll
+        for (int i = 0; i < VPL; ++i) {
+          const int c = (lane + 64 * i) * 8;
+          if (c < d) {
+            float xv[8], dv[8];
+            load8<T>(x0 + xoff + c, xv);
+            load8<T>(dxn + xoff + c, dv);
+            ln_row_bwd_acc(xv, dv, g[i], mu, rs, xh[i], gg[i], dg[i], db[i], s1, s2);
+          }
+        }
+        const float c1 = wave_sum_dpp(s1) * inv_d;
+        const float c2 = wave_sum_dpp(s2) * inv_d;
+        T* out = j == 0 ? dcls_rows + s * d : demb + (s * n + (j - 1)) * d;
+#pragma unroll
+        for (int i = 0; i < VPL; ++i) {
+          const int c = (lane + 64 * i) * 8;
+          if (c < d) {
+            float o[8];
+            LN_ROW_BWD_DX(o, gg[i], xh[i], rs, c1, c2);
+            if (dy) {
+              float a[8];
+              load8<T>(dy + xoff + c, a);
+#pragma unroll
+              for (int k = 0; k < 8; ++k) o[k] += a[k];
+            }
+            store8<T>(out + c, o);
+            round8<T>(o);
+#pragma unroll
+            for (int k = 0; k < 8; ++k) acc[i][k] += o[k];
+          }
+        }
+      }
+    }
+#pragma unroll
+    for (int i = 0; i < VPL; ++i) {
+      const int c = (lane + 64 * i) * 8;
+      if (c < d) {
+        float* o = dpos + it * d + c;
+        if (accumulate) {
+          float p[8];
+          load8<float>(o, p);
+#pragma unroll
+          for (int k = 0; k < 8; ++k) acc[i][k] += p[k];
+        }
+        store8<float>(o, acc[i]);
+      }
+    }
+  }
+  ln_block_partials<VPL, kSeamBlock>(dg, db, lds, d, lane, wid, partial + (int64_t)blockIdx.x * 2 * d);
+}
+
+int64_t seam_bwd_blocks(int64_t T, int64_t pos_rows) {
+  int64_t blocks = dvt_cdiv(T * pos_rows > 0 ? T * pos_rows : 1, kSeamBlock / 64);
+  return blocks > kSeamMaxBlocks ? kSeamMaxBlocks : blocks;
+}
+
+int seam_check(const char* name, int64_t S, int64_t T, int64_t n, int64_t d, int64_t pos_rows) {
+  DVT_REQUIRE(S > 0 && T > 0 && n >= 0 && S % T == 0, "%s: bad sizes", name);
+  DVT_REQUIRE(d >= 8 && d % 8 == 0, "%s: d = %lld must be a positive multiple of 8", name, (long long)d);
+  if (d > 8 * 64 * 8) DVT_UNSUPPORTED("%s: d = %lld > 4096 not supported", name, (long long)d);
+  DVT_REQUIRE(pos_rows >= n + 1, "%s: positional table has %lld rows < n+1 = %lld", name, (long long)pos_rows,
+              (long long)(n + 1));
+  return DVT_OK;
+}
+
+}
+
+extern "C" {
+
+int dvt_seam_tokens_ln_fwd(const void* emb, const float* cls, const float* pos, const float* gamma, const float* beta,
+                           void* x0, void* xn, float* mean, float* rstd, int64_t S, int64_t T, int64_t n, int64_t d,
+                           int64_t pos_rows, float eps, int dtype, dvt_stream_t stream) {
+  int rc = seam_check("dvt_seam_tokens_ln_fwd", S, T, n, d, pos_rows);
+  if (rc) return rc;
+  DVT_REQUIRE((emb || n == 0) && cls && pos && gamma && beta && x0 && xn && mean && rstd, "dvt_seam_tokens_ln_fwd: null pointer");
+  DVT_REQUIRE(dvt_aligned16(emb) && dvt_aligned16(cls) && dvt_aligned16(pos) && dvt_aligned16(gamma) && dvt_aligned16(beta) &&
+                  dvt_aligned16(x0) && dvt_aligned16(xn),
+              "dvt_seam_tokens_ln_fwd: buffers must be 16-byte aligned");
+  hipStream_t st = (hipStream_t)stream;
+  const int64_t rows = S * (n + 1);
+  int64_t blocks = dvt_cdiv(rows, kSeamBlock / 64);
+  const int64_t cap = (int64_t)dvt_num_cus() * 8;
+  if (blocks > cap) blocks = cap;
+  const int vpl = (int)dvt_cdiv(d, 8 * 64);
+  DVT_DISPATCH_DTYPE(dtype, Tt,
+                     DVT_LN_VPL_SWITCH(vpl, hipLaunchKernelGGL((seam_tokens_ln_fwd_kernel<Tt, VPL>), dim3((unsigned)blocks),
+                                                               dim3(kSeamBlock), 0, st, (const Tt*)emb, cls, pos, gamma, beta,
+                                                               (Tt*)x0, (Tt*)xn, mean, rstd, S, T, n, (int)d, pos_rows, eps)));
+  DVT_LAUNCH_CHECK("dvt_seam_tokens_ln_fwd");
+  return DVT_OK;
+}
+
+size_t dvt_seam_ln_tokens_bwd_partial_bytes(int64_t T, int64_t pos_rows, int64_t d) {
+  return (size_t)seam_bwd_blocks(T, pos_rows) * 2 * (size_t)(d > 0 ? d : 0) * sizeof(float);
+}
+
+int dvt_seam_ln_tokens_bwd(const void* dxn, const void* x0, const float* gamma, const float* mean, const float* rstd,
+                           const void* dy, void* demb, float* dpos, void* dcls_rows, float* dgamma, float* dbeta,
+                           void* workspace, int64_t S, int64_t T, int64_t n, int64_t d, int64_t pos_rows, int dtype,
+                           int accumulate_pos, int accumulate_gamma, int accumulate_beta, dvt_ln_pending* pending,
+                           dvt_stream_t stream) {
+  int rc = seam_check("dvt_seam_ln_tokens_bwd", S, T, n, d, pos_rows);
+  if (rc) return rc;
+  DVT_REQUIRE(dxn && x0 && gamma && mean && rstd && (demb || n == 0) && dpos && dcls_rows && dgamma && dbeta && workspace,
+              "dvt_seam_ln_tokens_bwd: null pointer");
+  DVT_REQUIRE(dvt_aligned16(dxn) && dvt_aligned16(x0) && dvt_aligned16(gamma) && dvt_aligned16(dy) && dvt_aligned16(demb) &&
+                  dvt_aligned16(dpos) && dvt_aligned16(dcls_rows) && dvt_aligned16(workspace),
+              "dvt_seam_ln_tokens_bwd: buffers must be 16-byte aligned");
+  if (d > kSeamBwdMaxD) DVT_UNSUPPORTED("dvt_seam_ln_tokens_bwd: d = %lld > %d not supported", (long long)d, kSeamBwdMaxD);
+  hipStream_t st = (hipStream_t)stream;
+  const int64_t blocks = seam_bwd_blocks(T, pos_rows);
+  const size_t lds = 2 * (size_t)d * sizeof(float);
+  float* partial = (float*)workspace;
+  DVT_DISPATCH_DTYPE(dtype, Tt,
+                     hipLaunchKernelGGL((seam_ln_tokens_bwd_kernel<Tt, 1>), dim3((unsigned)blocks), dim3(kSeamBlock), lds, st,
+                                        (const Tt*)dxn, (const Tt*)x0, gamma, mean, rstd, (const Tt*)dy, (Tt*)demb, dpos,
+                                        (Tt*)dcls_rows, partial, S, T, n, (int)d, pos_rows, accumulate_pos));
+  DVT_LAUNCH_CHECK("dvt_seam_ln_tokens_bwd");
+  dvt_ln_pending pn{};
+  pn.partial = partial; pn.nparts = (int)blocks; pn.d = (int)d; pn.dgamma = dgamma; pn.dbeta = dbeta;
+  pn.accumulate = (accumulate_gamma ? 1 : 0) | (accumulate_beta ? 2 : 0); pn.valid = 1;
+  if (pending) {
+    *pending = pn;
+    return DVT_OK;
+  }
+  return dvt_layernorm_reduce_group(&pn, 1, stream);
+}
+
+}
diff --git a/data-efficient-video-transformers_amd/functional.py b/data-efficient-video-transformers_amd/functional.py
--- a/data-efficient-video-transformers_amd/functional.py
+++ b/data-efficient-video-transformers_amd/functional.py
@@ -101,9 +101,11 @@
         _lp_hand.clear()
 
 
-def _ln_bwd(dy, x, g, mean, rstd, sg, sb, **kw):
+def _ln_bwd(dy, x, g, mean, rstd, sg, sb, op=None, **kw):
+    if op is None:
+        op = ops.layernorm_bwd
     if sg is None or sb is None:
-        return ops.layernorm_bwd(dy, x, g, mean, rstd, **kw)
+        return op(dy, x, g, mean, rstd, **kw)
     defer = None
     if LN_DEFER:
         if id(sg) in _ln_pending_sinks or id(sb) in _ln_pending_sinks:
@@ -114,8 +116,8 @@
             def defer():
                 sg.mark_written()
                 sb.mark_written()
-    r = ops.layernorm_bwd(dy, x, g, mean, rstd, dg=sg.buf.view(-1), db=sb.buf.view(-1),
-                          accumulate=not sg.fresh, accumulate_beta=not sb.fresh, defer=defer, **kw)
+    r = op(dy, x, g, mean, rstd, dg=sg.buf.view(-1), db=sb.buf.view(-1),
+           accumulate=not sg.fresh, accumulate_beta=not sb.fresh, defer=defer, **kw)
     if defer is None:
         sg.mark_written()
         sb.mark_written()
@@ -338,25 +340,85 @@
 
     @staticmethod
     def backward(ctx, dout):
-        sc, sp = ctx.sinks
+        return _tokens_bwd(ctx, dout) + (None, None, None)
+
+
+def _tokens_bwd(ctx, dout):
+    sc, sp = ctx.sinks[:2]
+    if sc is not None and sp is not None and sc.fresh != sp.fresh:
+        demb, dcls, dpos = ops.tokens_assemble_bwd(dout, ctx.T, ctx.pos_rows)
+        _emit_into(sc, dcls)
+        _emit_into(sp, dpos)
+        return demb, None, None
+    if sc is not None and sp is not None:
+        demb, _, _ = ops.tokens_assemble_bwd(dout, ctx.T, ctx.pos_rows, dcls=sc.buf.view(-1),
+                                             dpos=sp.buf.view(ctx.T, ctx.pos_rows, -1),
+                                             accumulate=not sc.fresh)
+        sc.mark_written()
+        sp.mark_written()
+        return demb, None, None
+    demb, dcls, dpos = ops.tokens_assemble_bwd(dout, ctx.T, ctx.pos_rows)
+    return demb, dcls.view(ctx.cls_shape), dpos.view(ctx.pos_shape)
+
+
+def tokens_assemble(emb: Tensor, cls: Tensor, pos: Tensor, S: int, T: int, n: int) -> Tensor:
+    return _Tokens.apply(emb, cls, pos, S, T, n)
+
+
+class _TokensLn(torch.autograd.Function):
+
+    @staticmethod
+    def forward(ctx, emb, cls, pos, ln_w, ln_b, S, T, n, eps):
+        cls32 = _f32(cls).reshape(-1)
+        pos32 = _f32(pos)
+        pos32 = pos32.reshape(T, pos32.shape[-2], pos32.shape[-1])
+        g, bb = _f32(ln_w), _f32(ln_b)
+        x0, xn, mean, rstd = ops.seam_tokens_ln_fwd(emb.contiguous(), cls32, pos32, g, bb, S, T, n, eps)
+        ctx.T, ctx.pos_rows = T, pos32.shape[1]
+        ctx.cls_shape, ctx.pos_shape = tuple(cls.shape), tuple(pos.shape)
+        ctx.sinks = (_sink(cls), _sink(pos), _sink(ln_w), _sink(ln_b))
+        ctx.save_for_backward(x0, g, mean, rstd)
+        ctx.mark_non_differentiable(mean, rstd)
+        ctx.set_materialize_grads(False)
+        return x0, xn, mean, rstd
+
+    @staticmethod
+    def backward(ctx, dx0, dxn, _dmean, _drstd):
+        x0, g, mean, rstd = ctx.saved_tensors
+        sc, sp, sg, sb = ctx.sinks
+        dxn = _as(dxn.contiguous(), x0.dtype) if dxn is not None else ops.zeros(x0.shape, x0.dtype, x0.device)
+        dx0 = _as(dx0.contiguous(), x0.dtype) if dx0 is not None else None
         if sc is not None and sp is not None and sc.fresh != sp.fresh:
-            demb, dcls, dpos = ops.tokens_assemble_bwd(dout, ctx.T, ctx.pos_rows)
-            _emit_into(sc, dcls)
-            _emit_into(sp, dpos)
-            return demb, None, None, None, None, None
-        if sc is not None and sp is not None:
-            demb, _, _ = ops.tokens_assemble_bwd(dout, ctx.T, ctx.pos_rows, dcls=sc.buf.view(-1),
-                                                 dpos=sp.buf.view(ctx.T, ctx.pos_rows, -1),
-                                                 accumulate=not sc.fresh)
+            dout, dg, db = _ln_bwd(dxn, x0, g, mean, rstd, sg, sb, dx_add=dx0)
+            return _tokens_bwd(ctx, dout) + (dg, db, None, None, None, None)
+        both = sc is not None and sp is not None
+        demb, dg, db, dpos, dcls_rows = _ln_bwd(
+            dxn, x0, g, mean, rstd, sg, sb, op=ops.seam_ln_tokens_bwd, T=ctx.T, pos_rows=ctx.pos_rows, dx_add=dx0,
+            dpos=sp.buf.view(ctx.T, ctx.pos_rows, -1) if both else None, accumulate_pos=both and not sp.fresh)
+        S, d = dcls_rows.shape
+        if x0.shape[0] * x0.shape[1] >= 4096:
+            ln_flush()
+        if both:
+            ops.rows_sum(dcls_rows, d, S, d, out=sc.buf.view(-1), accumulate=not sc.fresh)
             sc.mark_written()
             sp.mark_written()
-            return demb, None, None, None, None, None
-        demb, dcls, dpos = ops.tokens_assemble_bwd(dout, ctx.T, ctx.pos_rows)
-        return demb, dcls.view(ctx.cls_shape), dpos.view(ctx.pos_shape), None, None, None
-
-
-def tokens_assemble(emb: Tensor, cls: Tensor, pos: Tensor, S: int, T: int, n: int) -> Tensor:
-    return _Tokens.apply(emb, cls, pos, S, T, n)
+            return demb, None, None, dg, db, None, None, None, None
+        dcls = ops.rows_sum(dcls_rows, d, S, d)
+        return demb, dcls.view(ctx.cls_shape), dpos.view(ctx.pos_shape), dg, db, None, None, None, None
+
+
+def tokens_ln_supported(emb: Tensor) -> bool:
+    d = emb.shape[-1]
+    return (emb.is_cuda and emb.dtype in (torch.float32, torch.bfloat16, torch.float16) and d % 8 == 0
+            and 8 <= d <= ops.SEAM_BWD_FUSED_MAX_D)
+
+
+def tokens_ln(emb: Tensor, cls: Tensor, pos: Tensor, ln_w: Tensor, ln_b: Tensor, S: int, T: int, n: int, eps: float = 1e-5):
+    if not tokens_ln_supported(emb):
+        raise ValueError("tokens_ln: needs a HIP device, a 16- or 32-bit float type and d a multiple of 8 up to %d; use "
+                         "tokens_assemble and the block's own norm" % ops.SEAM_BWD_FUSED_MAX_D)
+    x0, xn, mean, rstd = _TokensLn.apply(emb, cls, pos, ln_w, ln_b, S, T, n, eps)
+    return x0, (xn, mean, rstd)
 
 
 class _ClsNormConcat(torch.autograd.Function):
@@ -488,7 +550,7 @@
 
     @staticmethod
     def forward(ctx, x, ln_w, ln_b, w_qkv, w_out, b_out, heads, prenorm, residual, eps, b_qkv=None,
-                seq_first=False, attn_dropout=0.0, cdt=None):
+                seq_first=False, attn_dropout=0.0, cdt=None, xn_pre=None, mean_pre=None, rstd_pre=None):
         shp = x.shape
         d = shp[-1]
         if seq_first:
@@ -503,7 +565,15 @@
         ctx.mixed = mixed = T != x.dtype
         if mixed and not (x.dtype == torch.float32 and prenorm and residual and w_out is not None and attn_dropout == 0.0):
             raise ValueError("the fp32 stream form is the pre-norm residual block with an output projection")
-        if prenorm:
+        ctx.pre = xn_pre is not None
+        if ctx.pre:
+            if not (prenorm and residual and not mixed and ln_w is None and ln_b is None):
+                raise ValueError("pre= is for the pre-norm residual block whose norm ran with the launch that made x")
+            g = mean = rstd = None
+            xn = xn_pre.reshape(-1, d)
+            if not (xn.is_contiguous() and xn.shape == x2.shape and xn.dtype == T):
+                raise ValueError("pre=: xn must be a contiguous map of x's shape and type")
+        elif prenorm:
             g, bb = _f32(ln_w), _f32(ln_b)
             xn, mean, rstd = ops.layernorm_fwd(x2, g, bb, eps, out_dtype=T)
         else:
@@ -564,8 +634,10 @@
         ops.attention_bwd(q, k, v, _heads_view(o_mem, seq_first), lse,
                           _heads_view(do2.view(o_mem.shape), seq_first), dq, dk, dv, dh ** -0.5, ctx.drop)
         dwq, dbq, dxn = _linear_bwd(ctx.sinks[2], ctx.sinks[5], dqkv, xn, wq, has_qkv_bias)
-        dg = db = None
-        if ctx.mixed:
+        dg = db = dpre = None
+        if ctx.pre:
+            dx, dpre = dy2, dxn.view(ctx.xshape)
+        elif ctx.mixed:
             dx, dg, db, dx_lp = _ln_bwd(dxn, x2, g, mean, rstd, ctx.sinks[0], ctx.sinks[1], dx_add=dy32,
                                         dx_dtype=torch.float32, dx_lp=T)
             _lp_put(dx, dx_lp)
@@ -574,15 +646,16 @@
                                  dx_add=dy2 if residual else None)
         else:
             dx = ops.add(dxn, dy2) if residual else dxn
-        if M >= 4096:
+        if M >= 4096 and not ctx.pre:
             ln_flush()
-        return dx.view(ctx.xshape), dg, db, dwq, dwo, dbo, None, None, None, None, dbq, None, None, None
+        return (dx.view(ctx.xshape), dg, db, dwq, dwo, dbo, None, None, None, None, dbq, None, None, None,
+                dpre, None, None)
 
 
 def attn_block(x, ln_w, ln_b, w_qkv, w_out, b_out, heads, *, prenorm=True, residual=True, eps=1e-5,
-               b_qkv=None, seq_first=False, attn_dropout=0.0, cdt=None):
+               b_qkv=None, seq_first=False, attn_dropout=0.0, cdt=None, pre=None):
     return _AttnBlock.apply(x, ln_w, ln_b, w_qkv, w_out, b_out, heads, prenorm, residual, eps, b_qkv, seq_first,
-                            float(attn_dropout), cdt)
+                            float(attn_dropout), cdt, *(pre if pre is not None else (None, None, None)))
 
 
 class _AttnBlockCls(torch.autograd.Function):
@@ -1712,29 +1785,28 @@
 class _Checkpoint(torch.autograd.Function):
 
     @staticmethod
-    def forward(ctx, fn, x, *params):
-        ctx.fn = fn
-        ctx.save_for_backward(x)
+    def forward(ctx, fn, nx, *args):
+        ctx.fn, ctx.nx = fn, nx
+        ctx.save_for_backward(*args[:nx])
         ctx.site = _rng.site
         with torch.no_grad():
-            return fn(x)
-
-    @staticmethod
-    def backward(ctx, dy):
-        (x,) = ctx.saved_tensors
-        xin = x.detach().requires_grad_(True)
+            return fn(*args[:nx])
+
+    @staticmethod
+    def backward(ctx, dy):
+        ins = [t.detach().requires_grad_(i == 0 or ctx.needs_input_grad[2 + i]) for i, t in enumerate(ctx.saved_tensors)]
         site_now, _rng.site = _rng.site, ctx.site
         with torch.enable_grad():
-            y = ctx.fn(xin)
+            y = ctx.fn(*ins)
         _rng.site = site_now
         torch.autograd.backward(y, dy)
-        return (None, xin.grad) + (None,) * (len(ctx.needs_input_grad) - 2)
-
-
-def checkpoint(fn, x: Tensor, params=()) -> Tensor:
+        return (None, None) + tuple(t.grad for t in ins) + (None,) * (len(ctx.needs_input_grad) - 2 - ctx.nx)
+
+
+def checkpoint(fn, x: Tensor, params=(), extra=()) -> Tensor:
     if not torch.is_grad_enabled():
-        return fn(x)
-    return _Checkpoint.apply(fn, x, *params)
+        return fn(x, *extra)
+    return _Checkpoint.apply(fn, 1 + len(extra), x, *extra, *params)
 
 
 class _L2Normalize(torch.autograd.Function):
diff --git a/data-efficient-video-transformers_amd/models/vit.py b/data-efficient-video-transformers_amd/models/vit.py
--- a/data-efficient-video-transformers_amd/models/vit.py
+++ b/data-efficient-video-transformers_amd/models/vit.py
@@ -99,9 +99,12 @@
         self.project_out = project_out
         self.dropout_p = dropout
 
-    def forward(self, x, _norm=None, _residual=False, _cdt=None):
+    def forward(self, x, _norm=None, _residual=False, _cdt=None, _pre=None):
         w_out = self.to_out[0].weight if self.project_out else None
         b_out = self.to_out[0].bias if self.project_out else None
+        if _pre is not None:
+            return F.attn_block(x, None, None, self.to_qkv.weight, w_out, b_out, self.heads, prenorm=True,
+                                residual=_residual, eps=_norm.eps, pre=_pre)
         if self.training and self.dropout_p > 0.0 and self.project_out:
             y = F.attn_block(x, _norm.weight if _norm is not None else None, _norm.bias if _norm is not None else None,
                              self.to_qkv.weight, w_out, b_out, self.heads, prenorm=_norm is not None, residual=False,
@@ -138,16 +141,27 @@
         from .. import ops
         return ops.gemm_is_launch_bound(rows, d, inner, cdt) and ops.gemm_is_launch_bound(rows, d, hidden, cdt)
 
-    def forward_layers(self, x, cdt=None):
+    def entry_norm(self, prunable: bool):
+        if len(self.layers) < (2 if prunable else 1):
+            return None
+        attn = self.layers[0][0]
+        if not attn.fn.project_out or (self.training and attn.fn.dropout_p > 0.0):
+            return None
+        if F._attn_tap is not None:
+            return None
+        return attn.norm
+
+    def forward_layers(self, x, cdt=None, pre=None):
         for attn, ff in self.layers:
             if self.checkpoint and self.training and torch.is_grad_enabled():
-                def block(t, attn=attn, ff=ff):
-                    t = attn.fn(t, _norm=attn.norm, _residual=True, _cdt=cdt)
+                def block(t, *p, attn=attn, ff=ff):
+                    t = attn.fn(t, _norm=attn.norm, _residual=True, _cdt=cdt, _pre=p or None)
                     return ff.fn(t, _norm=ff.norm, _residual=True, _cdt=cdt)
-                x = F.checkpoint(block, x, tuple(attn.parameters()) + tuple(ff.parameters()))
+                x = F.checkpoint(block, x, tuple(attn.parameters()) + tuple(ff.parameters()), extra=pre or ())
             else:
-                x = attn.fn(x, _norm=attn.norm, _residual=True, _cdt=cdt)
+                x = attn.fn(x, _norm=attn.norm, _residual=True, _cdt=cdt, _pre=pre)
                 x = ff.fn(x, _norm=ff.norm, _residual=True, _cdt=cdt)
+            pre = None
         return x
 
     def cls_prunable(self) -> bool:
@@ -157,17 +171,18 @@
         dropping = self.training and (attn.dropout_p > 0.0 or self.layers[-1][1].fn.dropout_p > 0.0)
         return attn.project_out and not dropping
 
-    def forward_layers_cls(self, x, cdt=None):
+    def forward_layers_cls(self, x, cdt=None, pre=None):
         *head, (attn, ff) = self.layers
         for a, f in head:
             if self.checkpoint and self.training and torch.is_grad_enabled():
-                def block(t, a=a, f=f):
-                    t = a.fn(t, _norm=a.norm, _residual=True, _cdt=cdt)
+                def block(t, *p, a=a, f=f):
+                    t = a.fn(t, _norm=a.norm, _residual=True, _cdt=cdt, _pre=p or None)
                     return f.fn(t, _norm=f.norm, _residual=True, _cdt=cdt)
-                x = F.checkpoint(block, x, tuple(a.parameters()) + tuple(f.parameters()))
+                x = F.checkpoint(block, x, tuple(a.parameters()) + tuple(f.parameters()), extra=pre or ())
             else:
-                x = a.fn(x, _norm=a.norm, _residual=True, _cdt=cdt)
+                x = a.fn(x, _norm=a.norm, _residual=True, _cdt=cdt, _pre=pre)
                 x = f.fn(x, _norm=f.norm, _residual=True, _cdt=cdt)
+            pre = None
 
         def last(t):
             an, af = attn.norm, attn.fn
@@ -292,14 +307,20 @@
         n = (x.shape[3] // self.patch_size) * (x.shape[4] // self.patch_size)
         pe = self.to_patch_embedding[1]
         emb = F.patch_embed(x, pe.weight, pe.bias, self.patch_size, T, tubelet=self.tubelet_size)
-        tok = F.tokens_assemble(emb, self.space_token, self.pos_embedding, b * t, t, n)
-        tok = F.dropout(tok, self.emb_dropout_p, self.training)
         st, tt = self.space_transformer, self.temporal_transformer
         sn = st.norm
-        if st.cls_prunable():
-            s = st.forward_layers_cls(tok).view(b * t, 1, -1)
+        prunable = st.cls_prunable()
+        en = None if (self.training and self.emb_dropout_p > 0.0) or not F.tokens_ln_supported(emb) else st.entry_norm(prunable)
+        pre = None
+        if en is not None:
+            tok, pre = F.tokens_ln(emb, self.space_token, self.pos_embedding, en.weight, en.bias, b * t, t, n, en.eps)
         else:
-            s = st.forward_layers(tok)
+            tok = F.tokens_assemble(emb, self.space_token, self.pos_embedding, b * t, t, n)
+            tok = F.dropout(tok, self.emb_dropout_p, self.training)
+        if prunable:
+            s = st.forward_layers_cls(tok, pre=pre).view(b * t, 1, -1)
+        else:
+            s = st.forward_layers(tok, pre=pre)
         zone32 = self.zone_f32 and tt.stream_f32_ok(b * (t + 1), T)
         cdt = T if zone32 else None
         seq = F.cls_norm_concat(s, sn.weight, sn.bias, self.temporal_token, b, t, sn.eps,
diff --git a/data-efficient-video-transformers_amd/ops.py b/data-efficient-video-transformers_amd/ops.py
--- a/data-efficient-video-transformers_amd/ops.py
+++ b/data-efficient-video-transformers_amd/ops.py
@@ -418,6 +418,84 @@
         if len(_ln_deferred) >= LN_DEFER_MAX:
             layernorm_flush()
     return (dx, dg, db) if dx_lp is None else (dx, dg, db, lp)
+
+
+SEAM_MAX_D = 4096
+SEAM_BWD_FUSED_MAX_D = 512
+
+
+def seam_tokens_ln_fwd(emb: Tensor, cls: Tensor, pos: Tensor, gamma: Tensor, beta: Tensor, S: int, T: int, n: int,
+                       eps: float = 1e-5) -> Tuple[Tensor, Tensor, Tensor, Tensor]:
+    _need_cuda(emb, cls, pos, gamma, beta)
+    d = emb.shape[-1]
+    assert emb.is_contiguous() and cls.is_contiguous() and pos.is_contiguous() and gamma.is_contiguous() and beta.is_contiguous()
+    assert all(t.dtype == torch.float32 for t in (cls, pos, gamma, beta))
+    assert emb.numel() == S * n * d and pos.dim() == 3 and pos.shape[0] == T and pos.shape[2] == d and cls.numel() == d
+    x0 = torch.empty((S, n + 1, d), dtype=emb.dtype, device=emb.device)
+    xn = torch.empty_like(x0)
+    rows = S * (n + 1)
+    mean = torch.empty((rows,), dtype=torch.float32, device=emb.device)
+    rstd = torch.empty((rows,), dtype=torch.float32, device=emb.device)
+    nb = (emb.numel() + 2 * x0.numel()) * emb.element_size() + pos.numel() * 4 + rows * 8
+    with _timed(("hbm", "seam_tokens_ln_fwd", rows), nb):
+        L.check(L.load().dvt_seam_tokens_ln_fwd(emb.data_ptr(), cls.data_ptr(), pos.data_ptr(), gamma.data_ptr(),
+                                                beta.data_ptr(), x0.data_ptr(), xn.data_ptr(), mean.data_ptr(),
+                                                rstd.data_ptr(), S, T, n, d, pos.shape[1], eps, dt(emb), _stream()),
+                "dvt_seam_tokens_ln_fwd")
+    return x0, xn, mean, rstd
+
+
+def seam_ln_tokens_bwd(dxn: Tensor, x0: Tensor, gamma: Tensor, mean: Tensor, rstd: Tensor, *, T: int, pos_rows: int,
+                       dx_add: Optional[Tensor] = None, dpos: Optional[Tensor] = None, accumulate_pos: bool = False,
+                       dg: Optional[Tensor] = None, db: Optional[Tensor] = None, accumulate: bool = False,
+                       accumulate_beta: Optional[bool] = None, defer=None):
+    _need_cuda(dxn, x0, gamma, mean, rstd, dx_add, dpos, dg, db)
+    S, n1, d = x0.shape
+    n = n1 - 1
+    assert x0.is_contiguous() and dxn.is_contiguous() and dxn.shape == x0.shape and dxn.dtype == x0.dtype
+    assert dx_add is None or (dx_add.is_contiguous() and dx_add.shape == x0.shape and dx_add.dtype == x0.dtype)
+    assert S % T == 0 and pos_rows >= n1 and mean.numel() == S * n1 and rstd.numel() == S * n1
+    demb = torch.empty((S * n, d), dtype=x0.dtype, device=x0.device)
+    dcls_rows = torch.empty((S, d), dtype=x0.dtype, device=x0.device)
+    if dpos is None:
+        assert not accumulate_pos
+        dpos = torch.empty((T, pos_rows, d), dtype=torch.float32, device=x0.device)
+    assert dpos.is_contiguous() and dpos.dtype == torch.float32 and dpos.numel() == T * pos_rows * d
+    if dg is None or db is None:
+        assert not accumulate and not accumulate_beta and dg is None and db is None
+        dg = torch.empty((d,), dtype=torch.float32, device=x0.device)
+        db = torch.empty((d,), dtype=torch.float32, device=x0.device)
+    acc_b = accumulate if accumulate_beta is None else accumulate_beta
+    lib = L.load()
+    if d > SEAM_BWD_FUSED_MAX_D:
+        dx0, dg, db = layernorm_bwd(dxn, x0, gamma, mean, rstd, dx_add=dx_add, dg=dg, db=db, accumulate=accumulate,
+                                    accumulate_beta=acc_b, defer=defer)
+        L.check(lib.dvt_tokens_assemble_bwd(dx0.data_ptr(), _p(demb) if n > 0 else None, None, dpos.data_ptr(), S, T, n, d,
+                                            pos_rows, dt(x0), int(accumulate_pos), _stream()), "dvt_tokens_assemble_bwd")
+        copy2d(dx0, dcls_rows, S, d, n1 * d, d)
+        return demb, dg, db, dpos, dcls_rows
+    nbytes = lib.dvt_seam_ln_tokens_bwd_partial_bytes(T, pos_rows, d)
+    pending = None
+    if defer:
+        ws = torch.empty((nbytes,), dtype=torch.uint8, device=x0.device)
+        pending = L.LnPending()
+        pending._keep = (ws, dg, db)
+    else:
+        ws = workspace(nbytes, x0.device)
+    es = x0.element_size()
+    nb = S * n1 * (d * es * (2 + (dx_add is not None)) + 8) + demb.numel() * es + dpos.numel() * 4 * (1 + accumulate_pos)
+    with _timed(("hbm", "seam_ln_tokens_bwd", S * n1), nb):
+        L.check(lib.dvt_seam_ln_tokens_bwd(dxn.data_ptr(), x0.data_ptr(), gamma.data_ptr(), mean.data_ptr(), rstd.data_ptr(),
+                                           _p(dx_add), _p(demb) if n > 0 else None, dpos.data_ptr(), dcls_rows.data_ptr(),
+                                           dg.data_ptr(), db.data_ptr(), ws.data_ptr(), S, T, n, d, pos_rows, dt(x0),
+                                           int(accumulate_pos), int(accumulate), int(acc_b),
+                                           C.pointer(pending) if pending is not None else None, _stream()),
+                "dvt_seam_ln_tokens_bwd")
+    if defer:
+        _ln_deferred.append((pending, defer if callable(defer) else None))
+        if len(_ln_deferred) >= LN_DEFER_MAX:
+            layernorm_flush()
+    return demb, dg, db, dpos, dcls_rows
 
 
 def _gemm_desc(A: Tensor, B: Tensor, M: int, N: int, K: int, *, a_kmajor: bool, b_kmajor: bool, lda: int, ldb: int,
diff --git a/include/dvt_hip.h b/include/dvt_hip.h
--- a/include/dvt_hip.h
+++ b/include/dvt_hip.h
@@ -125,6 +125,16 @@
 size_t dvt_layernorm_bwd_partial_bytes(int64_t rows, int64_t d);
 int dvt_layernorm_bwd_ex(const dvt_ln_bwd_desc* desc, dvt_stream_t stream);
 int dvt_layernorm_reduce_group(const dvt_ln_pending* list, int count, dvt_stream_t stream);
+
+int dvt_seam_tokens_ln_fwd(const void* emb, const float* cls, const float* pos, const float* gamma, const float* beta,
+                           void* x0, void* xn, float* mean, float* rstd, int64_t S, int64_t T, int64_t n, int64_t d,
+                           int64_t pos_rows, float eps, int dtype, dvt_stream_t stream);
+size_t dvt_seam_ln_tokens_bwd_partial_bytes(int64_t T, int64_t pos_rows, int64_t d);
+int dvt_seam_ln_tokens_bwd(const void* dxn, const void* x0, const float* gamma, const float* mean, const float* rstd,
+                           const void* dy, void* demb, float* dpos, void* dcls_rows, float* dgamma, float* dbeta,
+                           void* workspace, int64_t S, int64_t T, int64_t n, int64_t d, int64_t pos_rows, int dtype,
+                           int accumulate_pos, int accumulate_gamma, int accumulate_beta, dvt_ln_pending* pending,
+                           dvt_stream_t stream);
 
 enum dvt_epilogue {
   DVT_EPI_NONE = 0,
```
